# Benjamin-Lee/circkit

Measured on NVIDIA B200. Metric: canonicalize+uniq records/sec, higher is better.
Workload: dtype u8

## Files before the change

circkit_b200/_native.py:

```python
from __future__ import annotations

import ctypes as C
import os

HERE = os.path.dirname(os.path.abspath(__file__))
LIB_PATH = os.environ.get("CIRCKIT_B200_LIB") or os.path.join(HERE, "libcirckit_b200.so")

CK_OK = 0
CK_ERR_CUDA, CK_ERR_ARG, CK_ERR_STATE, CK_ERR_TOO_LONG, CK_ERR_TABLE_FULL = -1, -2, -3, -4, -5
CK_F_NORMALIZE, CK_F_NO_BYTES, CK_F_ALIGNED_OUT, CK_F_PACKED_IN, CK_F_SURVIVORS, CK_F_SINGLE_COPY = 1, 2, 4, 8, 16, 32
CK_PEER_HANDLE_BYTES = 64
CK_MONO_SENSITIVE, CK_MONO_FIRST_ONLY, CK_MONO_KEEP_ALL, CK_MONO_NONE = 1, 2, 4, 0xFFFFFFFF
CK_CMD_CANONICALIZE, CK_CMD_UNIQ, CK_CMD_MONOMERIZE = 1, 2, 3
CK_F_CANONICAL_BODY = 64
CK_DEFLATE_MAX_BYTES, CK_DEFLATE_DICT_BYTES = 64 << 20, 32768
CK_CLASS_2BIT_LE_512, CK_CLASS_2BIT_LE_2048, CK_CLASS_2BIT_LE_65536, CK_CLASS_2BIT_LE_425984 = 1, 2, 4, 8
CK_CLASS_2BIT_LE_4096, CK_CLASS_2BIT_LE_8192 = 1 << 10, 1 << 11


class CkConfig(C.Structure):
    _fields_ = [("device", C.c_int32), ("max_batch_bytes", C.c_uint64),
                ("max_batch_records", C.c_uint32), ("table_capacity", C.c_uint64)]


class CkPackedBatch(C.Structure):
    _fields_ = [("packed2", C.c_void_p), ("offsets", C.c_void_p), ("lens", C.c_void_p), ("lane", C.c_void_p),
                ("lane_bytes", C.c_void_p), ("lane_offsets", C.c_void_p), ("lane_bytes_total", C.c_uint64),
                ("n_records", C.c_uint32)]


class CkMonoOptions(C.Structure):
    _fields_ = [("seed_len", C.c_uint32), ("flags", C.c_uint32), ("overlap_dist", C.c_uint64),
                ("overlap_min_identity", C.c_double), ("min_length", C.c_uint64), ("max_length", C.c_uint64),
                ("min_overlap", C.c_uint64), ("min_overlap_percent", C.c_double)]


class NativeLibraryMissing(RuntimeError):
    pass


_vp, _u64, _u32, _i, _sz = C.c_void_p, C.c_uint64, C.c_uint32, C.c_int, C.c_size_t

SIGNATURES = {
    "ck_init": (_i, [C.POINTER(CkConfig), C.POINTER(_vp)]),
    "ck_destroy": (None, [_vp]),
    "ck_last_error": (C.c_char_p, [_vp]),
    "ck_alloc_pinned": (_vp, [_vp, _sz]),
    "ck_free_pinned": (None, [_vp, _vp]),
    "ck_canon_submit": (_i, [_vp, _i, _vp, _vp, _u32, _u32]),
    "ck_canon_wait": (_i, [_vp, _i, _vp, _vp, _vp, _vp, _vp]),
    "ck_uniq_submit": (_i, [_vp, _i, _vp, _vp, _u32, _u32, _u64]),
    "ck_uniq_wait": (_i, [_vp, _i, _vp, _vp, _vp, _vp]),
    "ck_uniq_wait_survivors": (_i, [_vp, _i, C.POINTER(_u32), _vp, _vp, _vp, _vp, _vp, _vp]),
    "ck_uniq_reset": (_i, [_vp]),
    "ck_uniq_grow": (_i, [_vp, _u64]),
    "ck_uniq_table_info": (_i, [_vp, C.POINTER(_u64), C.POINTER(_u64), C.POINTER(_u64)]),
    "ck_peer_export": (_i, [_vp, _u32, _u32, _u32, _vp]),
    "ck_peer_attach": (_i, [_vp, _vp]),
    "ck_dev_peer_first_index": (_i, [_vp, _vp, _vp, _u32, _u64, _vp, _u64, _vp]),
    "ck_pack2_words": (_u64, [_u64, _u32]),
    "ck_pack2_host": (_i, [_vp, _vp, _u32, _u32, _u32, _vp, _vp, _vp, _vp, _u64, _vp, C.POINTER(_u64)]),
    "ck_canon_submit_packed": (_i, [_vp, _i, C.POINTER(CkPackedBatch), _u32]),
    "ck_uniq_submit_packed": (_i, [_vp, _i, C.POINTER(CkPackedBatch), _u32, _u64]),
    "ck_lmsr_index": (_i, [_vp, _vp, _sz, C.POINTER(_sz)]),
    "ck_lmsr": (_i, [_vp, _vp, _sz, _vp]),
    "ck_canonicalize": (_i, [_vp, _vp, _sz, _vp]),
    "ck_lmsr_index_batch": (_i, [_vp, _vp, _vp, _u32, _vp]),
    "ck_dev_workspace_bytes": (_u64, [_u32, _u64]),
    "ck_out_arena_bytes": (_u64, [_u64, _u32]),
    "ck_dev_canon_packed2": (_i, [_vp, _vp, _vp, _vp, _u32, _u32, _u32, _vp, _vp, _vp, _vp, _vp, _u64]),
    "ck_dev_canon_bytes": (_i, [_vp, _vp, _vp, _vp, _u32, _u64, _u32, _u32, _vp, _vp, _vp, _vp, _vp, _vp, _u64]),
    "ck_dev_check": (_i, [_vp, _vp, _vp]),
    "ck_dev_table_bytes": (_u64, [_u64]),
    "ck_dev_table_clear": (_i, [_vp, _vp, _vp, _u64]),
    "ck_dev_table_insert": (_i, [_vp, _vp, _vp, _u64, _vp, _vp, _u64, _u32, _vp]),
    "ck_dev_table_first": (_i, [_vp, _vp, _vp, _u64, _vp, _u32, _vp]),
    "ck_dev_owner_partition": (_i, [_vp, _vp, _vp, _u32, _u64, _u32, _vp, _vp, _vp, _vp]),
    "ck_dev_table_insert_pairs": (_i, [_vp, _vp, _vp, _u64, _vp, _u32, _vp]),
    "ck_dev_owner_partition_padded": (_i, [_vp, _vp, _vp, _u32, _u64, _u32, _u32, _vp, _vp, _vp]),
    "ck_dev_owner_scatter_peers": (_i, [_vp, _vp, _vp, _u32, _u64, _u32, _u32, _u32, _vp, _vp, _vp]),
    "ck_dev_table_first_peers": (_i, [_vp, _vp, _vp, _u64, _vp, _u32, _u32, _u32, _vp]),
    "ck_dev_gather_first": (_i, [_vp, _vp, _vp, _vp, _u32, _vp]),
    "ck_dev_monomerize": (_i, [_vp, _vp, _vp, _vp, _vp, _u32, _u32, _u64, C.c_double, _u32, _vp]),
    "ck_dev_normalize": (_i, [_vp, _vp, _vp, _vp, _u32, _vp, _vp]),
    "ck_mono_submit": (_i, [_vp, _i, _vp, _vp, _u32, _u32, C.POINTER(CkMonoOptions)]),
    "ck_mono_wait": (_i, [_vp, _i, C.POINTER(_u32), _vp, _vp, _vp, _vp, _vp, _vp]),
    "ck_fasta_out_bytes": (_u64, [_u64, _u32]),
    "ck_fasta_submit": (_i, [_vp, _i, _vp, _u64, _u32, _u32, _u64, C.POINTER(CkMonoOptions), C.POINTER(_u32)]),
    "ck_fasta_wait": (_i, [_vp, _i, _vp, C.POINTER(_u64), C.POINTER(_u32), _vp, _vp, _vp, _vp, _vp]),
    "ck_deflate_bound": (_u64, [_u64]),
    "ck_deflate_submit": (_i, [_vp, _i, _vp, _u64, _vp, _u32, _u32]),
    "ck_deflate_wait": (_i, [_vp, _i, _vp, C.POINTER(_u64), C.POINTER(_u32)]),
    "ck_launch_count": (_u64, [_vp]),
    "ck_kernel_timing": (_i, [_vp, _i]),
    "ck_kernel_times": (_i, [_vp, _vp, _vp, _u32]),
    "ck_synth_offsets": (_i, [_vp, _vp, _u64, _u64, _u32, _u32, _u32, _u32, _u32, _vp, C.POINTER(_u64)]),
    "ck_synth_packed2": (_i, [_vp, _vp, _u64, _u64, _u32, _vp, _u32, _u32, _vp, _u32]),
    "ck_dev_unpack2": (_i, [_vp, _vp, _vp, _vp, _u32, _vp, _u32]),
    "ck_packed2_words": (_u64, [_u64, _u32, _u32]),
}

_lib = None


def lib() -> C.CDLL:
    global _lib
    if _lib is None:
        if not os.path.exists(LIB_PATH):
            raise NativeLibraryMissing(
                f"{LIB_PATH} not found: build it with `python -m circkit_b200.build` "
                "(nvcc, sm_100a).  circkit_b200 has no CPU fallback.")
        L = C.CDLL(LIB_PATH)
        for name, (res, args) in SIGNATURES.items():
            f = getattr(L, name)
            f.restype, f.argtypes = res, args
        _lib = L
    return _lib
```

circkit_b200/csrc/ck_kernels.cuh:

```cuda
#pragma once
#include "ck_hash.cuh"

namespace ck {

enum : int {
    CLS_W2S = 0,
    CLS_W2M = 1,
    CLS_C2A = 2,
    CLS_C2B = 3,
    CLS_W4 = 4,
    CLS_C4 = 5,
    CLS_W8 = 6,
    CLS_C8 = 7,
    CLS_HUGE = 8,
    CLS_EMPTY = 9,
    CLS_W2L = 10,
    CLS_W2X = 11,
    CLS_COUNT = 12
};
__host__ __device__ constexpr u32 cls_max_n(int c)
{
    return c == CLS_W2S ? 512u : c == CLS_W2M ? 2048u : c == CLS_W2L ? 4096u : c == CLS_W2X ? 8192u : c == CLS_C2A ? 65536u
         : c == CLS_C2B ? 425984u : c == CLS_W4 ? 2048u : c == CLS_C4 ? 212992u : c == CLS_W8 ? 1024u : c == CLS_C8 ? 106496u
         : c == CLS_EMPTY ? 0u : 0xffffffffu;
}
__host__ __device__ constexpr u32 cls_min_n(int c)
{
    return c == CLS_W2M ? cls_max_n(CLS_W2S) + 1 : c == CLS_W2L ? cls_max_n(CLS_W2M) + 1 : c == CLS_W2X ? cls_max_n(CLS_W2L) + 1
         : c == CLS_C2A ? cls_max_n(CLS_W2X) + 1 : c == CLS_C2B ? cls_max_n(CLS_C2A) + 1 : c == CLS_C4 ? cls_max_n(CLS_W4) + 1
         : c == CLS_C8 ? cls_max_n(CLS_W8) + 1 : c == CLS_EMPTY ? 0u : 1u;
}

__host__ __device__ constexpr u32 cls_rank(int c)
{
    return c == CLS_W2S ? 0u : c == CLS_W2M ? 1u : c == CLS_W2L ? 2u : c == CLS_W2X ? 3u : c == CLS_C2A ? 4u : c == CLS_C2B ? 5u
         : c == CLS_W4 ? 6u : c == CLS_C4 ? 7u : c == CLS_W8 ? 8u : c == CLS_C8 ? 9u : c == CLS_HUGE ? 10u : 11u;
}
__host__ __device__ constexpr int cls_of_rank(u32 r)
{
    return r == 0 ? CLS_W2S : r == 1 ? CLS_W2M : r == 2 ? CLS_W2L : r == 3 ? CLS_W2X : r == 4 ? CLS_C2A : r == 5 ? CLS_C2B
         : r == 6 ? CLS_W4 : r == 7 ? CLS_C4 : r == 8 ? CLS_W8 : r == 9 ? CLS_C8 : r == 10 ? CLS_HUGE : CLS_EMPTY;
}

struct TableSlot { u64 key; u64 first; };
#define CK_EMPTY_KEY 0xffffffffffffffffULL
__device__ __forceinline__ u64 table_home(u64 key, u64 nslots) { return __umul64hi((key ^ (key >> 29)) * 0x9E3779B97F4A7C15ULL, nslots); }
__device__ __forceinline__ u64 table_insert_one(TableSlot *slots, u64 nslots, u64 *side_first, u32 *overflow, u64 key, u64 idx)
{
    if (key == CK_EMPTY_KEY) { atomicMin(side_first, idx); return ~0ULL; }
    u64 s = table_home(key, nslots);
    for (u64 probes = 0; probes < nslots; probes++) {
        const u64 prev = atomicCAS(&slots[s].key, CK_EMPTY_KEY, key);
        if (prev == CK_EMPTY_KEY || prev == key) { atomicMin(&slots[s].first, idx); return s; }
        s = s + 1 == nslots ? 0 : s + 1;
    }
    *overflow = 1;
    return ~0ULL - 1;
}

struct CanonArgs {
    const u64 *packed2;
    u32 p2_dbl;
    const u8 *bytes;
    const u64 *offsets;
    const u32 *lens;
    const u32 *list;
    const u32 *count;
    u32 n_direct;
    u8 *out;
    u32 *out_start;
    u8 *out_strand;
    u64 *out_hash;
    u32 *scratch;
    u64 scratch_stride;
    u32 smem_units;
    u32 *xglobal;
    u32 mode;
    u32 min_n, max_n;
    u32 *retry;
    u32 *retry_counts;
    const u8 *lane_bits;
};

__device__ __forceinline__ void store_chunk(u8 *dst, int t0, u32 n, u64 lo, u64 hi)
{
    if (t0 >= 0 && (u32)t0 + 16u <= n) {
        *reinterpret_cast<uint4 *>(dst + t0) = make_uint4((u32)lo, (u32)(lo >> 32), (u32)hi, (u32)(hi >> 32));
        return;
    }
    const u32 kb = t0 < 0 ? (u32)(-t0) : 0u;
    const u32 ke = t0 < 0 ? min(16u, n + kb) : min(16u, n - (u32)t0);
    u8 *p = dst + t0;
#define CK_PIECE(k) (((k) & 8u ? hi : lo) >> (8u * ((k) & 7u)))
    u32 k = kb;
    if ((k & 1u) && k + 1 <= ke) { p[k] = (u8)CK_PIECE(k); k += 1; }
    if ((k & 2u) && k + 2 <= ke) { *reinterpret_cast<u16 *>(p + k) = (u16)CK_PIECE(k); k += 2; }
    if ((k & 4u) && k + 4 <= ke) { *reinterpret_cast<u32 *>(p + k) = (u32)CK_PIECE(k); k += 4; }
    if ((k & 8u) && k + 8 <= ke) { *reinterpret_cast<u64 *>(p + k) = hi; k += 8; }
    if (k + 8 <= ke) { *reinterpret_cast<u64 *>(p + k) = CK_PIECE(k); k += 8; }
    if (k + 4 <= ke) { *reinterpret_cast<u32 *>(p + k) = (u32)CK_PIECE(k); k += 4; }
    if (k + 2 <= ke) { *reinterpret_cast<u16 *>(p + k) = (u16)CK_PIECE(k); k += 2; }
    if (k + 1 <= ke) { p[k] = (u8)CK_PIECE(k); }
#undef CK_PIECE
}

template <int BITS, typename G>
__device__ __forceinline__ void emit_ascii(const u32 *X, u32 n, u32 start, u8 *dst)
{
    const u32 rank = G::rank(), gs = G::size();
    const u32 a = (u32)(reinterpret_cast<uintptr_t>(dst) & 15u);
    const u32 nchunks = (n + a + 15u) >> 4;
    for (u32 c = rank; c < nchunks; c += gs) {
        const int t0 = (int)(16u * c) - (int)a;
        int ti = t0;
        if (ti < 0) { ti += (int)n; if (ti < 0) { ti %= (int)n; if (ti < 0) ti += (int)n; } }
        const u32 tt = (u32)ti;
        u32 t8 = tt + 8; if (t8 >= n) { t8 -= n; if (t8 >= n) t8 %= n; }
        const u64 lo = ascii8<BITS>(X, n, start, tt), hi = ascii8<BITS>(X, n, start, t8);
        store_chunk(dst, t0, n, lo, hi);
    }
}

template <int BITS, typename G>
__device__ __forceinline__ void do_record(const CanonArgs &a, u32 rec, u32 *Xf, u32 *Xr, u32 *scr, u64 *hbuf, u32 *red)
{
    const u64 off = a.offsets[rec];
    const u32 n = a.lens ? a.lens[rec] : (u32)(a.offsets[rec + 1] - off);
    if (a.list == nullptr && (n < a.min_n || n > a.max_n)) return;
    if (a.lane_bits) { const u32 lb = a.lane_bits[rec]; if ((lb == 3u ? 4u : lb) != (u32)BITS) return; }
    RecordIn in;
    in.packed2 = a.packed2 ? a.packed2 + p2_word(off, rec, a.p2_dbl) : nullptr;
    in.bytes = a.bytes ? a.bytes + off : nullptr;
    in.n = n;
    stage_record<BITS, G>(in, Xf, Xr);
    RecordOut o = canonical_start<BITS, G>(Xf, Xr, n, scr, red, (a.mode & 1u) != 0);
    const u32 *X = o.strand ? Xr : Xf;
    if (a.out) emit_ascii<BITS, G>(X, n, o.start, a.out + ((a.mode & 2u) ? out_byte(off, rec) : off));
    u64 h = 0;
    if (a.out_hash) h = xxh3_canonical<BITS, G>(X, n, o.start, hbuf, red);
    if (G::rank() == 0) {
        if (a.out_start) a.out_start[rec] = o.strand ? (n - 1 - o.start) : o.start;
        if (a.out_strand) a.out_strand[rec] = (u8)o.strand;
        if (a.out_hash) a.out_hash[rec] = h;
    }
    G::sync();
}

template <int BITS>
__global__ void __launch_bounds__(256) k_canon_warp(CanonArgs a)
{
    extern __shared__ u32 smem[];
    typedef Grp<false> G;
    if (BITS != 2) stab_load();
    const u32 wid = threadIdx.x >> 5, wpb = blockDim.x >> 5;
    u32 *Xf = smem + (size_t)wid * 2 * a.smem_units, *Xr = Xf + a.smem_units;
    const u32 gw = blockIdx.x * wpb + wid, nw = gridDim.x * wpb;
    u32 *scr = a.scratch + (size_t)gw * a.scratch_stride;
    const u32 count = a.list ? *a.count : a.n_direct;
    if (a.list) a.list += a.count[16];
    for (u32 e = gw; e < count; e += nw) {
        const u32 rec = a.list ? a.list[e] : e;
        do_record<BITS, G>(a, rec, Xf, Xr, scr, nullptr, nullptr);
    }
}

template <int BITS, bool XGLOBAL>
__global__ void __launch_bounds__(1024) k_canon_cta(CanonArgs a)
{
    extern __shared__ u32 smem[];
    __shared__ u32 red[40];
    __shared__ u64 hbuf[32 * 8];
    typedef Grp<true> G;
    if (BITS != 2) stab_load();
    u32 *Xf = XGLOBAL ? a.xglobal + (size_t)blockIdx.x * 2 * a.smem_units : smem;
    u32 *Xr = Xf + a.smem_units;
    u32 *scr = a.scratch + (size_t)blockIdx.x * a.scratch_stride;
    const u32 count = a.list ? *a.count : a.n_direct;
    if (a.list) a.list += a.count[16];
    for (u32 e = blockIdx.x; e < count; e += gridDim.x) {
        const u32 rec = a.list ? a.list[e] : e;
        do_record<BITS, G>(a, rec, Xf, Xr, scr, hbuf, red);
    }
}

__global__ void k_canon_empty(CanonArgs a)
{
    const u32 count = a.list ? *a.count : a.n_direct;
    if (a.list) a.list += a.count[16];
    for (u32 e = blockIdx.x * blockDim.x + threadIdx.x; e < count; e += gridDim.x * blockDim.x) {
        const u32 rec = a.list ? a.list[e] : e;
        if (a.list == nullptr && a.offsets[rec + 1] != a.offsets[rec]) continue;
        if (a.out_start) a.out_start[rec] = 0;
        if (a.out_strand) a.out_strand[rec] = 1;
        if (a.out_hash) a.out_hash[rec] = xxh64_avalanche(sec64(56) ^ sec64(64));
    }
}

struct PrepareArgs {
    const u8 *raw; const u64 *offsets; u32 n_records; u32 flags;
    u64 *packed2; u8 *bytes; u32 *lens; u8 *lane;
};
__device__ __forceinline__ u32 code2_of(u32 b) { return ((b >> 1) & 3u) ^ ((b >> 2) & 1u); }

__device__ __forceinline__ uint4 prep_load16(const uint4 *w, u32 sh, bool second, bool first = true)
{
    uint4 a = make_uint4(0, 0, 0, 0), b = make_uint4(0, 0, 0, 0);
    if (first) a = __ldg(w);
    if (second) b = __ldg(w + 1);
    const u32 bs = 8u * (sh & 3u);
// ... 52 lines not shown
#pragma unroll
        for (int i = 0; i < 4; i++) {
            const u32 t = ((mm[i] & 0x7f7f7f7fu) + 0x7f7f7f7fu) | mm[i];
            nz |= ((((t >> 7) & 0x01010101u) * 0x01020408u) >> 24) << (4 * i);
        }
        keep = valid & nz;
    }
}

template <int K> __device__ __forceinline__ void prep_store_byte(u8 *g, u32 w, u32 mask)
{
    asm volatile("{ .reg .pred q; .reg .b32 t; and.b32 t, %2, %3; setp.ne.u32 q, t, 0; @q st.global.u8 [%0+%4], %1; }"
                 :: "l"(g), "r"(w >> (8 * (K & 3))), "r"(mask), "n"(1 << K), "n"(K) : "memory");
}
__device__ __forceinline__ void prep_store_bytes(u8 *g, const u32 (&w)[4], u32 mask)
{
    prep_store_byte<0>(g, w[0], mask); prep_store_byte<1>(g, w[0], mask); prep_store_byte<2>(g, w[0], mask); prep_store_byte<3>(g, w[0], mask);
    prep_store_byte<4>(g, w[1], mask); prep_store_byte<5>(g, w[1], mask); prep_store_byte<6>(g, w[1], mask); prep_store_byte<7>(g, w[1], mask);
    prep_store_byte<8>(g, w[2], mask); prep_store_byte<9>(g, w[2], mask); prep_store_byte<10>(g, w[2], mask); prep_store_byte<11>(g, w[2], mask);
    prep_store_byte<12>(g, w[3], mask); prep_store_byte<13>(g, w[3], mask); prep_store_byte<14>(g, w[3], mask); prep_store_byte<15>(g, w[3], mask);
}

#define CK_PREP_STAGE 560u

__global__ void __launch_bounds__(256) k_prepare(PrepareArgs a)
{
    __shared__ u16 tab[256];
    __shared__ __align__(16) u8 stage_all[8][CK_PREP_STAGE];
    const bool norm = a.flags & 1u;
    for (u32 b = threadIdx.x; b < 256; b += blockDim.x) {
        const u32 m = norm ? (u32)c_tab.norm[b] : b;
        const bool keep = norm ? m != 0 : true;
        const bool acgt = (m == 'A') | (m == 'C') | (m == 'G') | (m == 'T');
        u32 e = 0;
        if (keep) e = m | 0x100u | (acgt ? 0u : 0x200u) | ((!acgt && c_tab.code4[m] == 0xffu) ? 0x400u : 0u);
        tab[b] = (u16)e;
    }
    __syncthreads();
    const u32 lane = lane_id();
    u8 *stage = stage_all[threadIdx.x >> 5];
    const u32 gw = (blockIdx.x * blockDim.x + threadIdx.x) >> 5, nw = (gridDim.x * blockDim.x) >> 5;
    for (u32 rec = gw; rec < a.n_records; rec += nw) {
        const u64 off = a.offsets[rec];
        const u32 rawlen = (u32)(a.offsets[rec + 1] - off);
        const u8 *src = a.raw + off;
        u8 *dstb = a.bytes + off;
        const u32 A = (u32)((size_t)dstb & 15u);
        u8 *gbase = dstb - A;
        const u8 *srcA = src - A;
        const u32 shA = (u32)((size_t)srcA & 15u);
        const uint4 *srcA16 = reinterpret_cast<const uint4 *>(srcA - shA);
        const u32 spanA = A + rawlen;
        u32 fl = 0, cnt = 0;
        uint4 m1 = make_uint4(0, 0, 0, 0);
        for (u32 base = 0; base < spanA && rawlen; base += 512) {
            const u32 p = base + 16 * lane;
            if (p < spanA) {
                const u32 lo = p < A ? A - p : 0u, hi = min(16u, spanA - p);
                const uint4 *w0 = srcA16 + (p >> 4);
                const uint4 q = prep_load16(w0, shA, p + 16 < spanA + shA, p + 16 > A + shA);
                u32 f, keep;
                prep_lookup(tab, q, lo, hi, m1, f, keep);
                fl |= f; cnt += __popc(keep);
            }
        }
        cnt = __reduce_add_sync(CK_FULL, cnt);
        fl = __reduce_or_sync(CK_FULL, fl);
        const u32 lanebits = (fl & 0x400u) ? 8u : (fl & 0x200u) ? 4u : 2u;
        if (lane == 0) { a.lens[rec] = cnt; if (a.lane) a.lane[rec] = (u8)lanebits; }
        const bool pack2 = lanebits == 2 && !(a.flags & 2u);
        if (rawlen == 0) continue;
        const u32 sh = (u32)((size_t)src & 15u);
        const uint4 *src16 = reinterpret_cast<const uint4 *>(src - sh);
        const u32 span = sh + rawlen;
        u32 *dst32 = reinterpret_cast<u32 *>(a.packed2 + p2_word(off, rec, (a.flags >> 2) & 1u));
        if (cnt == rawlen && pack2) {
            for (u32 base = 0; base < rawlen; base += 512) {
                const u32 p = base + 16 * lane;
                if (p < rawlen) {
                    const u32 v = min(16u, rawlen - p);
                    u32 unit = prep_pack16(prep_load16(src16 + (p >> 4), sh, p + 16 < span));
                    if (v < 16) unit &= ~(0xffffffffu >> (2 * v));
                    dst32[p >> 4] = unit;
                }
            }
            continue;
        }
        if (cnt == rawlen && spanA <= 512) {
            const u32 p = 16 * lane;
            if (p < spanA) {
                const u32 lo = p < A ? A - p : 0u, hi = min(16u, spanA - p);
                if (hi - lo == 16) *reinterpret_cast<uint4 *>(gbase + p) = m1;
                else {
                    const u32 valid = (hi >= 16 ? 0xffffu : ((1u << hi) - 1u)) & ~((1u << lo) - 1u);
                    const u32 w[4] = {m1.x, m1.y, m1.z, m1.w};
                    u8 *g = gbase + p;
                    u32 vb = valid;
#pragma unroll
                    for (int i = 0; i < 4; i++)
                        if (((valid >> (4 * i)) & 15u) == 15u) { *reinterpret_cast<u32 *>(g + 4 * i) = w[i]; vb &= ~(15u << (4 * i)); }
                    prep_store_bytes(g, w, vb);
                }
            }
            continue;
        }
        u32 S = pack2 ? 0u : A;
        u32 done = 0;
        for (u32 base = 0; base < rawlen; base += 512) {
            const u32 p = base + 16 * lane;
            uint4 m = make_uint4(0, 0, 0, 0);
            u32 mask = 0;
            if (p < rawlen) {
                u32 f;
                prep_lookup(tab, prep_load16(src16 + (p >> 4), sh, p + 16 < span), 0u, min(16u, rawlen - p), m, f, mask);
            }
            const u32 kc = __popc(mask);
            u32 incl = kc;
#pragma unroll
            for (int d = 1; d < 32; d <<= 1) { const u32 t = __shfl_up_sync(CK_FULL, incl, d); if (lane >= (u32)d) incl += t; }
            const u32 T = __shfl_sync(CK_FULL, incl, 31);
            u32 idx = S + incl - kc;
            __syncwarp();
#pragma unroll
            for (int k = 0; k < 16; k++)
                if ((mask >> k) & 1u) stage[idx++] = (u8)prep_byte(m, k);
            __syncwarp();
            const u32 fill = S + T;
            if (pack2) {
                const u32 U = fill >> 4;
                for (u32 j = lane; j < U; j += 32) dst32[done + j] = prep_pack16(*reinterpret_cast<const uint4 *>(stage + 16 * j));
                const u32 r = fill & 15u;
                u8 c = 0;
                if (lane < r) c = stage[16 * U + lane];
                __syncwarp();
                if (lane < r) stage[lane] = c;
                done += U; S = r;
            } else {
                u8 *g = dstb + done - S;
                for (u32 w = lane; 16 * w < fill; w += 32) {
                    const u32 lo = max(16 * w, S), hi = min(16 * w + 16, fill);
                    if (hi - lo == 16) *reinterpret_cast<uint4 *>(g + 16 * w) = *reinterpret_cast<const uint4 *>(stage + 16 * w);
                    else for (u32 i = lo; i < hi; i++) g[i] = stage[i];
                }
                done += T; S = (u32)((size_t)(dstb + done) & 15u);
            }
        }
        __syncwarp();
        if (pack2 && S && lane == 0)
            dst32[done] = prep_pack16(*reinterpret_cast<const uint4 *>(stage)) & ~(0xffffffffu >> (2 * S));
        __syncwarp();
    }
}

struct ClassifyArgs {
    const u64 *offsets; const u32 *lens; const u8 *lane;
    u32 n_records;
    u32 *keys, *vals;
    u32 *counts;
    u32 direct_mask;
    u32 window_shift;
    u32 top_bit;
};
__global__ void __launch_bounds__(256) k_classify(ClassifyArgs a)
{
    __shared__ u32 cnt[16];
    if (threadIdx.x < 16) cnt[threadIdx.x] = 0;
    __syncthreads();
    const u32 nthreads = gridDim.x * blockDim.x;
    const u32 rounds = (a.n_records + nthreads - 1) / nthreads;
    for (u32 r = 0; r < rounds; r++) {
        const u32 i = r * nthreads + blockIdx.x * blockDim.x + threadIdx.x;
        int cls = -1;
        u32 n = 0;
        if (i < a.n_records) {
            n = a.lens ? a.lens[i] : (u32)(a.offsets[i + 1] - a.offsets[i]);
            const u32 bits = a.lane ? a.lane[i] : 2u;
            if (n == 0) cls = CLS_EMPTY;
            else if (bits == 2) cls = n <= cls_max_n(CLS_W2S) ? CLS_W2S : n <= cls_max_n(CLS_W2M) ? CLS_W2M
                                    : n <= cls_max_n(CLS_W2L) ? CLS_W2L : n <= cls_max_n(CLS_W2X) ? CLS_W2X
                                    : n <= cls_max_n(CLS_C2A) ? CLS_C2A : n <= cls_max_n(CLS_C2B) ? CLS_C2B : CLS_HUGE;
            else if (bits == 4 || bits == 3) cls = n <= cls_max_n(CLS_W4) ? CLS_W4 : n <= cls_max_n(CLS_C4) ? CLS_C4 : CLS_HUGE;
            else cls = n <= cls_max_n(CLS_W8) ? CLS_W8 : n <= cls_max_n(CLS_C8) ? CLS_C8 : CLS_HUGE;
        }
        if (a.direct_mask) {
            const u32 m = __ballot_sync(CK_FULL, cls >= 0 && !((a.direct_mask >> cls) & 1u));
            if (m && lane_id() == (u32)(__ffs(m) - 1)) atomicAdd(cnt + CLS_HUGE, __popc(m));
            continue;
        }
        if (cls >= 0) {
            const u32 msb = 31u - __clz(n | 1u);
            const u32 bin = (msb << 5) | ((((n << (31u - msb)) >> 29) & 3u) << 3);
            u32 key = (cls_rank(cls) << 10) | bin;
            if (a.window_shift < 32u) {
                const bool lane_cls = cls == CLS_W2S || cls == CLS_W2M || cls == CLS_W2L || cls == CLS_W2X;
                const u32 q = (msb << 2) | (((n << (31u - msb)) >> 29) & 3u);
                key = lane_cls ? (((i >> a.window_shift) << 5) | (q > 28u ? q - 28u : 0u)) : (key | (1u << a.top_bit));
            }
            a.keys[i] = key; a.vals[i] = i;
        }
        u32 todo = __ballot_sync(CK_FULL, cls >= 0);
        while (todo) {
            const int c = __shfl_sync(CK_FULL, cls, __ffs(todo) - 1);
            const u32 m = __ballot_sync(CK_FULL, cls == c);
            if (lane_id() == (u32)(__ffs(m) - 1)) atomicAdd(cnt + c, __popc(m));
            todo &= ~m;
        }
    }
    __syncthreads();
    if (threadIdx.x < 16 && cnt[threadIdx.x]) atomicAdd(a.counts + threadIdx.x, cnt[threadIdx.x]);
}
__global__ void k_list_starts(u32 *counts)
{
    if (threadIdx.x == 0) {
        u32 s = 0;
        for (u32 r = 0; r < (u32)CLS_COUNT; r++) {
            const int c = cls_of_rank(r);
            counts[16 + c] = s; counts[48 + c] = s;
            s += counts[c];
        }
        counts[12] = counts[CLS_W2S] + counts[CLS_W2M] + counts[CLS_W2L] + counts[CLS_W2X];
        counts[28] = counts[16 + CLS_W2S];
        counts[13] = counts[CLS_C2A] + counts[CLS_C2B];
        counts[29] = counts[16 + CLS_C2A];
    }
}

__device__ __forceinline__ u32 p2_last_unit(u32 n) { return max((2u * n + 143u) >> 4, (n >> 4) + 5u); }
__device__ __forceinline__ void extend_one(u64 *packed2, const u64 *offsets, const u32 *lens, u32 i, const u64 *dense, u32 dbl, u32 lane)
{
    const u64 off = offsets[i];
    const u32 n = lens ? lens[i] : (u32)(offsets[i + 1] - off);
    if (n == 0) return;
    u32 *U = reinterpret_cast<u32 *>(packed2 + p2_word(off, i, dbl));
    const u32 *S = dense ? reinterpret_cast<const u32 *>(dense + (off >> 5) + i) : U;
    const u32 jn = n >> 4, last = dbl ? p2_last_unit(n) : jn + 4;
    if (n >= 80) {
        for (u32 j = (dense ? 0u : jn) + lane; j <= last; j += 32) {
            const u32 r = (16u * j) % n;
            const u32 q = r >> 4, sh = 2u * (r & 15u);
            u32 w = __funnelshift_l(__ldcg(S + q + 1), __ldcg(S + q), sh);
            if (r + 16u > n) {
                const u32 k = n - r;
                w = (w & ~(0xffffffffu >> (2u * k))) | (__ldcg(S) >> (2u * k));
            }
            U[j] = w;
        }
    } else {
        for (u32 j = (dense ? 0u : jn) + lane; j <= last; j += 32) {
            u32 v = 0;
            for (u32 b = 0; b < 16; b++) {
                const u32 t = (16 * j + b) % n;
                v = (v << 2) | ((__ldcg(S + (t >> 4)) >> (30 - 2 * (t & 15))) & 3u);
            }
            __syncwarp(__activemask());
            U[j] = v;
        }
    }
    __syncwarp();
}
__global__ void __launch_bounds__(256) k_extend_packed2(u64 *packed2, const u64 *offsets, const u32 *lens, const u8 *lane_bits, u32 n_records,
                                                        const u64 *dense, u32 dbl)
{
    const u32 lane = lane_id();
    const u32 gw = (blockIdx.x * blockDim.x + threadIdx.x) >> 5, nw = (gridDim.x * blockDim.x) >> 5;
    if (n_records < 65536u) {
        for (u32 i = gw; i < n_records; i += nw) {
            if (lane_bits && lane_bits[i] != 2) continue;
            extend_one(packed2, offsets, lens, i, dense, dbl, lane);
        }
        return;
    }
    for (u32 i0 = 32u * gw; i0 < n_records; i0 += 32u * nw) {
        const u32 ii = i0 + lane;
        u32 m = __ballot_sync(CK_FULL, ii < n_records && (!lane_bits || lane_bits[ii] == 2));
        while (m) {
            const u32 i = i0 + (u32)__ffs(m) - 1u;
            m &= m - 1u;
            extend_one(packed2, offsets, lens, i, dense, dbl, lane);
        }
    }
}

__global__ void __launch_bounds__(256) k_scatter_lane_bytes(const u8 *lane_bytes, const u64 *lane_offsets, const u64 *offsets, const u32 *lens,
                                                            const u8 *lane_bits, u32 n_records, u8 *bytes)
{
    const u32 lane = lane_id();
    const u32 gw = (blockIdx.x * blockDim.x + threadIdx.x) >> 5, nw = (gridDim.x * blockDim.x) >> 5;
    for (u32 i = gw; i < n_records; i += nw) {
        if (lane_bits[i] == 2) continue;
        const u8 *src = lane_bytes + lane_offsets[i];
        u8 *dst = bytes + offsets[i];
        const u32 n = lens[i];
        for (u32 k = lane; k < n; k += 32) dst[k] = src[k];
    }
}

struct TableArgs {
    TableSlot *slots; u64 nslots;
    u64 *side_first;
    const u64 *hash; const u64 *index;
    u32 stride;
    u64 base_index; u32 n;
    u64 *slot_of;
    u64 *first_out;
    u32 *overflow;
    u64 *keys;
};
__global__ void __launch_bounds__(256) k_table_insert(TableArgs a)
{
    const u32 i = blockIdx.x * blockDim.x + threadIdx.x;
    if (i >= a.n) return;
    const u64 key = a.hash[(size_t)i * a.stride];
    const u64 idx = a.index ? a.index[(size_t)i * a.stride] : a.base_index + i;
    if (idx == ~0ULL) { a.slot_of[i] = ~0ULL - 1; return; }
    if (key == CK_EMPTY_KEY) { atomicMin(a.side_first, idx); a.slot_of[i] = ~0ULL; return; }
    u64 s = table_home(key, a.nslots);
    for (u64 probes = 0; probes < a.nslots; probes++) {
        u64 prev = atomicCAS(&a.slots[s].key, CK_EMPTY_KEY, key);
        if (prev == CK_EMPTY_KEY || prev == key) {
            atomicMin(&a.slots[s].first, idx);
            a.slot_of[i] = s;
            if (a.keys && prev == CK_EMPTY_KEY) {
                const u32 m = __activemask();
                if ((threadIdx.x & 31) == (u32)(__ffs(m) - 1)) atomicAdd(a.keys, (u64)__popc(m));
            }
            return;
        }
        s = s + 1 == a.nslots ? 0 : s + 1;
    }
    *a.overflow = 1; a.slot_of[i] = ~0ULL - 1;
}
__global__ void __launch_bounds__(256) k_table_first(TableArgs a)
{
    const u32 i = blockIdx.x * blockDim.x + threadIdx.x;
    if (i >= a.n) return;
    const u64 s = a.slot_of[i];
    a.first_out[i] = s == ~0ULL ? *a.side_first : (s == ~0ULL - 1 ? ~0ULL : a.slots[s].first);
}
__global__ void k_table_clear(TableSlot *slots, u64 n, u64 *side_first)
{
    for (u64 i = blockIdx.x * (u64)blockDim.x + threadIdx.x; i < n; i += (u64)gridDim.x * blockDim.x) {
        slots[i].key = CK_EMPTY_KEY; slots[i].first = ~0ULL;
    }
    if (blockIdx.x == 0 && threadIdx.x == 0) *side_first = ~0ULL;
}
__global__ void __launch_bounds__(256) k_table_rehash(const TableSlot *old, u64 old_slots, TableSlot *slots, u64 nslots)
{
    for (u64 i = blockIdx.x * (u64)blockDim.x + threadIdx.x; i < old_slots; i += (u64)gridDim.x * blockDim.x) {
        const TableSlot e = old[i];
        if (e.key == CK_EMPTY_KEY) continue;
        u64 s = table_home(e.key, nslots);
        while (atomicCAS(&slots[s].key, CK_EMPTY_KEY, e.key) != CK_EMPTY_KEY) s = s + 1 == nslots ? 0 : s + 1;
        slots[s].first = e.first;
    }
}

__global__ void __launch_bounds__(256) k_survivor_flags(const u64 *first, u64 base_index, u32 n, u8 *flags)
{
    const u32 i = blockIdx.x * blockDim.x + threadIdx.x;
    if (i < n) flags[i] = first[i] == base_index + i;
}
__global__ void __launch_bounds__(256) k_survivor_lens(const u32 *sel, const u32 *n_sel, const u32 *lens, u32 n, u64 *len16)
{
    const u32 k = blockIdx.x * blockDim.x + threadIdx.x;
    if (k > n) return;
    len16[k] = k < *n_sel ? (u64)((lens[sel[k]] + 15u) & ~15u) : 0ull;
}
__global__ void __launch_bounds__(256) k_gather_survivors(const u32 *sel, const u32 *n_sel, const u32 *lens, const u64 *offsets, const u8 *out,
                                                          u32 aligned, const u64 *compact_off, u8 *compact)
{
    const u32 lane = lane_id();
    const u32 gw = (blockIdx.x * blockDim.x + threadIdx.x) >> 5, nw = (gridDim.x * blockDim.x) >> 5;
    const u32 ns = *n_sel;
    for (u32 k = gw; k < ns; k += nw) {
        const u32 rec = sel[k], n = lens[rec];
        const u64 off = offsets[rec];
        const u8 *src = out + (aligned ? out_byte(off, rec) : off);
        u8 *dst = compact + compact_off[k];
        if (aligned) {
            for (u32 c = lane; 16u * c < n; c += 32) reinterpret_cast<uint4 *>(dst)[c] = reinterpret_cast<const uint4 *>(src)[c];
        } else {
            for (u32 b = lane; b < n; b += 32) dst[b] = src[b];
        }
    }
}

struct OwnerArgs {
    const u64 *hash; u32 n; u32 world; u64 base_index;
    u32 *counts;
    u64 *send_pairs; u32 *pos;
};
__device__ __forceinline__ u32 owner_of_hash(u64 h, u32 world) { return __umulhi((u32)(h >> 32), world); }
__global__ void __launch_bounds__(256) k_owner_count(OwnerArgs a)
{
    __shared__ u32 cnt[32];
    if (threadIdx.x < 32) cnt[threadIdx.x] = 0;
    __syncthreads();
    for (u32 i = blockIdx.x * blockDim.x + threadIdx.x; i < a.n; i += gridDim.x * blockDim.x)
        atomicAdd(cnt + owner_of_hash(a.hash[i], a.world), 1u);
    __syncthreads();
    if (threadIdx.x < a.world && cnt[threadIdx.x]) atomicAdd(a.counts + threadIdx.x, cnt[threadIdx.x]);
}
__global__ void __launch_bounds__(256) k_owner_scatter(OwnerArgs a)
{
    __shared__ u32 cnt[32], basep[32];
    const u32 per = (a.n + gridDim.x - 1) / gridDim.x;
    const u32 lo = min(a.n, blockIdx.x * per), hi = min(a.n, lo + per);
    if (threadIdx.x < 32) cnt[threadIdx.x] = 0;
    __syncthreads();
    for (u32 i = lo + threadIdx.x; i < hi; i += blockDim.x) atomicAdd(cnt + owner_of_hash(a.hash[i], a.world), 1u);
    __syncthreads();
    if (threadIdx.x < a.world) {
        u32 start = 0;
        for (u32 o = 0; o < threadIdx.x; o++) start += a.counts[o];
        basep[threadIdx.x] = start + atomicAdd(a.counts + a.world + threadIdx.x, cnt[threadIdx.x]);
        cnt[threadIdx.x] = 0;
    }
    __syncthreads();
    for (u32 i = lo + threadIdx.x; i < hi; i += blockDim.x) {
        const u64 h = a.hash[i];
        const u32 o = owner_of_hash(h, a.world);
        const u32 p = basep[o] + atomicAdd(cnt + o, 1u);
        reinterpret_cast<ulonglong2 *>(a.send_pairs)[p] = make_ulonglong2(h, a.base_index + i);
        a.pos[i] = p;
    }
}


struct OwnerPadArgs {
    const u64 *hash; u32 n; u32 world; u64 base_index; u32 cap;
    u32 *cursors;
    u64 *send_pairs; u32 *pos;
};
__global__ void __launch_bounds__(256) k_owner_scatter_padded(OwnerPadArgs a)
{
    __shared__ u32 cnt[32], basep[32];
    const u32 per = (a.n + gridDim.x - 1) / gridDim.x;
    const u32 lo = min(a.n, blockIdx.x * per), hi = min(a.n, lo + per);
    if (threadIdx.x < 32) cnt[threadIdx.x] = 0;
    __syncthreads();
    for (u32 i = lo + threadIdx.x; i < hi; i += blockDim.x) atomicAdd(cnt + owner_of_hash(a.hash[i], a.world), 1u);
    __syncthreads();
    if (threadIdx.x < a.world) {
        basep[threadIdx.x] = cnt[threadIdx.x] ? atomicAdd(a.cursors + threadIdx.x, cnt[threadIdx.x]) : 0u;
        if (basep[threadIdx.x] + cnt[threadIdx.x] > a.cap) a.cursors[a.world] = 1u;
        cnt[threadIdx.x] = 0;
    }
    __syncthreads();
    for (u32 i = lo + threadIdx.x; i < hi; i += blockDim.x) {
        const u64 h = a.hash[i];
        const u32 o = owner_of_hash(h, a.world);
        const u32 k = basep[o] + atomicAdd(cnt + o, 1u);
        u32 p = 0xffffffffu;
        if (k < a.cap) {
            p = o * a.cap + k;
            reinterpret_cast<ulonglong2 *>(a.send_pairs)[p] = make_ulonglong2(h, a.base_index + i);
        }
        a.pos[i] = p;
    }
}
__global__ void __launch_bounds__(256) k_owner_pad(OwnerPadArgs a)
{
    const u32 o = blockIdx.y;
    const u32 used = min(a.cursors[o], a.cap);
    for (u32 k = used + blockIdx.x * blockDim.x + threadIdx.x; k < a.cap; k += gridDim.x * blockDim.x)
        reinterpret_cast<ulonglong2 *>(a.send_pairs)[(size_t)o * a.cap + k] = make_ulonglong2(0ULL, ~0ULL);
}

struct PeerPtrs { u64 *p[32]; };
struct OwnerPeerArgs {
    const u64 *hash; u32 n; u32 world; u32 rank; u64 base_index; u32 cap;
    u32 *cursors;
    u32 *pos;
    PeerPtrs recv;
};
#define CK_SCAT_TILE 2048u
__global__ void __launch_bounds__(256) k_owner_scatter_peers(OwnerPeerArgs a)
{
    __shared__ ulonglong2 stage[CK_SCAT_TILE];
    __shared__ u8 own[CK_SCAT_TILE];
    __shared__ u32 cnt[32], start[33], basep[32], fill[32];
    const u32 per = (a.n + gridDim.x - 1) / gridDim.x;
    const u32 lo = min(a.n, blockIdx.x * per), hi = min(a.n, lo + per);
    for (u32 tile = lo; tile < hi; tile += CK_SCAT_TILE) {
        const u32 tn = min(hi - tile, CK_SCAT_TILE);
        if (threadIdx.x < 32) { cnt[threadIdx.x] = 0; fill[threadIdx.x] = 0; }
        __syncthreads();
        u64 hreg[CK_SCAT_TILE / 256];
        u32 oreg[CK_SCAT_TILE / 256];
#pragma unroll
        for (u32 k = 0; k < CK_SCAT_TILE / 256; k++) {
            const u32 j = threadIdx.x + 256u * k;
            if (j < tn) {
                hreg[k] = a.hash[tile + j];
                oreg[k] = owner_of_hash(hreg[k], a.world);
                atomicAdd(cnt + oreg[k], 1u);
            }
        }
        __syncthreads();
        if (threadIdx.x == 0) {
            u32 acc = 0;
            for (u32 o = 0; o < a.world; o++) { start[o] = acc; acc += cnt[o]; }
            start[a.world] = acc;
        }
        if (threadIdx.x < a.world) {
            const u32 c = cnt[threadIdx.x];
            basep[threadIdx.x] = c ? atomicAdd(a.cursors + threadIdx.x, c) : 0u;
            if (basep[threadIdx.x] + c > a.cap) a.cursors[a.world] = 1u;
        }
        __syncthreads();
#pragma unroll
        for (u32 k = 0; k < CK_SCAT_TILE / 256; k++) {
            const u32 j = threadIdx.x + 256u * k;
            if (j < tn) {
                const u32 o = oreg[k];
                const u32 r = atomicAdd(fill + o, 1u);
                const u32 slot = start[o] + r;
                stage[slot] = make_ulonglong2(hreg[k], a.base_index + tile + j);
                own[slot] = (u8)o;
                const u32 g = basep[o] + r;
                a.pos[tile + j] = g < a.cap ? o * a.cap + g : 0xffffffffu;
            }
        }
        __syncthreads();
        for (u32 sl = threadIdx.x; sl < tn; sl += 256) {
            const u32 o = own[sl];
            const u32 g = basep[o] + (sl - start[o]);
            if (g < a.cap) reinterpret_cast<ulonglong2 *>(a.recv.p[o])[(size_t)a.rank * a.cap + g] = stage[sl];
        }
        __syncthreads();
    }
}
__global__ void __launch_bounds__(256) k_owner_pad_peers(OwnerPeerArgs a)
{
    const u32 o = blockIdx.y;
    const u32 used = min(a.cursors[o], a.cap);
    ulonglong2 *dst = reinterpret_cast<ulonglong2 *>(a.recv.p[o]) + (size_t)a.rank * a.cap;
    for (u32 k = used + blockIdx.x * blockDim.x + threadIdx.x; k < a.cap; k += gridDim.x * blockDim.x)
        dst[k] = make_ulonglong2(0ULL, ~0ULL);
}
struct FirstPeerArgs {
    const TableSlot *slots; const u64 *side_first; const u64 *slot_of;
    u32 world; u32 rank; u32 cap;
    PeerPtrs ret;
};
__global__ void __launch_bounds__(256) k_table_first_peers(FirstPeerArgs a)
{
    const u32 s = blockIdx.y;
    u64 *dst = a.ret.p[s] + (size_t)a.rank * a.cap;
    const u64 *slot_of = a.slot_of + (size_t)s * a.cap;
    for (u32 k = blockIdx.x * blockDim.x + threadIdx.x; k < a.cap; k += gridDim.x * blockDim.x) {
        const u64 sl = slot_of[k];
        dst[k] = sl == ~0ULL ? *a.side_first : (sl == ~0ULL - 1 ? ~0ULL : a.slots[sl].first);
    }
}
struct PeerBlockPtrs { u64 *p[32]; };
#define CK_PEER_FLAG_WORDS 128u
#define CK_PEER_HEADER_BYTES 4096u
__global__ void k_peer_barrier(PeerBlockPtrs blocks, u32 world, u32 rank, u32 barrier_id, u64 epoch, const u32 *send_counts, u32 count_slot)
{
    const u32 t = threadIdx.x;
    if (t >= world) return;
    if (send_counts) blocks.p[t][CK_PEER_FLAG_WORDS + 32u * count_slot + rank] = send_counts[t];
    __threadfence_system();
    u64 *theirs = blocks.p[t] + barrier_id * 32u + rank;
    asm volatile("st.release.sys.global.u64 [%0], %1;" ::"l"(theirs), "l"(epoch) : "memory");
    const u64 *mine = blocks.p[rank] + barrier_id * 32u + t;
    u64 seen;
    do {
        asm volatile("ld.acquire.sys.global.u64 %0, [%1];" : "=l"(seen) : "l"(mine) : "memory");
    } while (seen < epoch);
}
struct RegionArgs {
    TableSlot *slots; u64 nslots; u64 *side_first; u32 *overflow;
    const u64 *recv;
    const u64 *counts;
    u64 *slot_of;
    u32 world, rank, cap;
    PeerBlockPtrs ret;
};
__global__ void __launch_bounds__(256) k_table_insert_regions(RegionArgs a)
{
    const u32 s = blockIdx.y;
    const u32 cnt = (u32)a.counts[s];
    const ulonglong2 *pairs = reinterpret_cast<const ulonglong2 *>(a.recv) + (size_t)s * a.cap;
    u64 *slot_of = a.slot_of + (size_t)s * a.cap;
    for (u32 k = blockIdx.x * blockDim.x + threadIdx.x; k < cnt; k += gridDim.x * blockDim.x) {
        const ulonglong2 pr = pairs[k];
        const u64 key = pr.x, idx = pr.y;
        if (key == CK_EMPTY_KEY) { atomicMin(a.side_first, idx); slot_of[k] = ~0ULL; continue; }
        u64 sl = table_home(key, a.nslots);
        u64 found = ~0ULL - 1;
        for (u64 probes = 0; probes < a.nslots; probes++) {
            const u64 prev = atomicCAS(&a.slots[sl].key, CK_EMPTY_KEY, key);
            if (prev == CK_EMPTY_KEY || prev == key) { atomicMin(&a.slots[sl].first, idx); found = sl; break; }
            sl = sl + 1 == a.nslots ? 0 : sl + 1;
        }
        if (found == ~0ULL - 1) *a.overflow = 1;
        slot_of[k] = found;
    }
}
__global__ void __launch_bounds__(256) k_table_first_regions(RegionArgs a)
{
    const u32 s = blockIdx.y;
    const u32 cnt = (u32)a.counts[s];
    u64 *dst = a.ret.p[s] + (size_t)a.rank * a.cap;
    const u64 *slot_of = a.slot_of + (size_t)s * a.cap;
    for (u32 k = blockIdx.x * blockDim.x + threadIdx.x; k < cnt; k += gridDim.x * blockDim.x) {
        const u64 sl = slot_of[k];
        dst[k] = sl == ~0ULL ? *a.side_first : (sl == ~0ULL - 1 ? ~0ULL : a.slots[sl].first);
    }
}

__global__ void __launch_bounds__(256) k_gather_first(const u64 *ret, const u32 *pos, u32 n, u64 *out)
{
    for (u32 i = blockIdx.x * blockDim.x + threadIdx.x; i < n; i += gridDim.x * blockDim.x) {
        const u32 p = pos[i];
        out[i] = p == 0xffffffffu ? ~0ULL : ret[p];
    }
}

}
```

circkit_b200/csrc/ck_lib.cu:

```cuda
#include <algorithm>
#include <cstdio>
#include <cstdlib>
#include <cstring>
#include <mutex>
#include <new>
#include <string>
#include <vector>

#include <cub/device/device_radix_sort.cuh>
#include <cub/device/device_scan.cuh>
#include <cub/device/device_select.cuh>
#include <cub/iterator/counting_input_iterator.cuh>

#include "../../include/circkit_b200.h"
#include "ck_kernels.cuh"
#include "ck_warp2.cuh"
#include "ck_lane2.cuh"
#include "ck_stream2.cuh"
#include "ck_stream3.cuh"
#include "ck_seg2.cuh"
#include "ck_lane4.cuh"
#include "ck_synth.cuh"
#include "ck_monomerize.cuh"
#include "ck_fasta.cuh"
#include "ck_deflate.cuh"

using namespace ck;

namespace {

thread_local std::string g_init_error;

inline const u64 *U(const uint64_t *p) { return reinterpret_cast<const u64 *>(p); }
inline u64 *U(uint64_t *p) { return reinterpret_cast<u64 *>(p); }

struct ClsCfg { int bits; bool cta; u32 threads; u32 ctas_per_sm; };
const ClsCfg kCls[CLS_COUNT] = {
    {2, false, 256, 8},
    {2, false, 256, 6},
    {2, true, 512, 4},
    {2, true, 1024, 1},
    {4, false, 256, 32},
    {4, true, 1024, 1},
    {8, false, 256, 32},
    {8, true, 1024, 1},
    {0, true, 0, 0},
    {0, false, 256, 1},
    {2, false, 256, 6},
    {2, false, 256, 6},
};

u32 cls_units(int c)
{
    const u32 n = cls_max_n(c);
    switch (kCls[c].bits) {
    case 2: return strand_units<2>(n);
    case 4: return strand_units<4>(n);
    default: return strand_units<8>(n);
    }
}
u64 cls_tie_words(int c)
{
    const u64 n = cls_max_n(c);
    switch (kCls[c].bits) {
    case 2: return tie_scratch_words<2>(n);
    case 4: return tie_scratch_words<4>(n);
    default: return tie_scratch_words<8>(n);
    }
}
u32 cls_smem_bytes(int c)
{
    const u32 per = 2u * cls_units(c) * 4u;
    if (c == CLS_W2S || c == CLS_W2M || c == CLS_W2L || c == CLS_W2X) return (u32)sizeof(W2Const) + per * (kCls[c].threads / 32u);
    return kCls[c].cta ? per : per * (kCls[c].threads / 32u);
}

struct ExecScratch {
    u32 *tie[CLS_COUNT] = {};
    u64 *seg = nullptr;
    u32 *huge_x = nullptr, *huge_tie = nullptr;
    u64 huge_x_words = 0, huge_tie_words = 0;
    cudaStream_t side_stream[CLS_COUNT] = {};
    cudaEvent_t ev_fork = nullptr, ev_join[CLS_COUNT] = {};
};

struct Slot {
    cudaStream_t stream = nullptr;
    cudaEvent_t inserted = nullptr;
    u8 *d_raw = nullptr; u64 *d_off = nullptr; u64 *d_p2 = nullptr; u8 *d_norm = nullptr; u8 *d_p4 = nullptr;
    u32 *d_len = nullptr; u8 *d_lane = nullptr; u8 *d_out = nullptr; u32 *d_start = nullptr;
    u8 *d_strand = nullptr; u64 *d_hash = nullptr; u64 *d_first = nullptr; u64 *d_slotof = nullptr;
    u32 *d_lists = nullptr; u32 *d_counts = nullptr;
    u64 *d_dense = nullptr; u64 *d_laneoff = nullptr;
    u32 *h_counts = nullptr;
    ExecScratch scr;
    bool busy = false, uniq = false, mono = false;
    bool text = false;
    u32 cmd = 0;
    u8 *d_text = nullptr, *d_frame = nullptr;
    u64 *d_rstart = nullptr, *d_head = nullptr, *d_seq = nullptr, *d_len64 = nullptr, *d_fofs = nullptr, *d_meta = nullptr;
    u32 *d_tiles = nullptr;
    u32 dbl = 1;
    u64 longest = 0;
    u32 *sel = nullptr; u64 *coff = nullptr;
    u32 n = 0, flags = 0; u64 total = 0;
    u64 rec_mark = 0;
    bool defl = false;
    struct Deflate {
        cudaStream_t stream = nullptr;
        u64 cap = 0;
        u8 *buf = nullptr;
        u32 *kA = nullptr, *kB = nullptr, *vA = nullptr, *vB = nullptr;
        u32 *prev8 = nullptr, *prev4 = nullptr;
        u32 *seg = nullptr;
        u32 *out = nullptr, *result = nullptr;
        u32 *h_result = nullptr;
        void *tmp = nullptr; size_t tmp_bytes = 0;
        u64 n = 0;
    } z;
};

struct PeerGroup {
    u32 world = 1, rank = 0, cap = 0;
    u8 *block = nullptr; u64 block_bytes = 0, recv_bytes = 0, ret_bytes = 0;
    void *mapped[32] = {};
    bool exported = false, attached = false;
    u64 epoch[4] = {};
    u32 *pos[2] = {}; u32 *cursors[2] = {}; u64 *slot_of[2] = {};
    u64 *recv(u32 r, u32 slot) const { return reinterpret_cast<u64 *>((u8 *)mapped[r] + CK_PEER_HEADER_BYTES + (u64)slot * recv_bytes); }
    u64 *ret(u32 r, u32 slot) const { return reinterpret_cast<u64 *>((u8 *)mapped[r] + CK_PEER_HEADER_BYTES + 2 * recv_bytes + (u64)slot * ret_bytes); }
    u64 *counts(u32 r, u32 slot) const { return reinterpret_cast<u64 *>(mapped[r]) + CK_PEER_FLAG_WORDS + 32u * slot; }
};

}

struct ck_ctx {
    int device = 0;
    int num_sms = 148;
    ck_config cfg{};
    std::string err;
    Slot slot[2];
    ExecScratch dev_scr;
    cudaEvent_t last_insert = nullptr;
    bool have_last_insert = false;
    TableSlot *table = nullptr; u64 table_slots = 0; u64 *side = nullptr; u32 *d_overflow = nullptr;
    u64 *d_keys = nullptr;
    u64 grow_max = 0, grows = 0;
    u64 known_keys = 0, known_rec = 0, submitted_rec = 0;
    PeerGroup peer;
    std::mutex lib_mu;
    cudaStream_t lib_stream = nullptr;
    u8 *lib_h = nullptr, *lib_d = nullptr; size_t lib_h_bytes = 0, lib_d_bytes = 0;
    ExecScratch lib_scr;
    u64 launches = 0;
    bool attrs_set = false;
    u32 s3_debug = 0;
    bool l4_kernel = true;
    bool seg_kernel = true;
    int lane_kernel = 3;
    bool timing = false;
    std::vector<cudaEvent_t> ev_pairs[CLS_COUNT + 7];
};

namespace {

int fail(ck_ctx *ctx, int code, const char *what, cudaError_t e = cudaSuccess)
{
    std::string m = what;
    if (e != cudaSuccess) { m += ": "; m += cudaGetErrorString(e); }
    if (ctx) ctx->err = m; else g_init_error = m;
    return code;
}
#define CK_CUDA(ctx, call)                                                     \
    do {                                                                       \
        cudaError_t e__ = (call);                                              \
        if (e__ != cudaSuccess) return fail((ctx), CK_ERR_CUDA, #call, e__);   \
    } while (0)

void fill_tables(Tables &t, u8 secret[200])
{
    for (int c = 0; c < 256; c++) t.norm[c] = 'N';
    for (const char *p = "ACGTN-"; *p; p++) t.norm[(u8)*p] = (u8)*p;
    t.norm['a'] = 'A'; t.norm['c'] = 'C'; t.norm['g'] = 'G';
    t.norm['t'] = 'T'; t.norm['u'] = 'T'; t.norm['U'] = 'T';
    t.norm['.'] = '-'; t.norm['~'] = '-';
    t.norm[' '] = 0; t.norm['\t'] = 0; t.norm['\r'] = 0; t.norm['\n'] = 0;
    for (int c = 0; c < 256; c++) t.comp[c] = (u8)c;
    const char *a = "AGCTYRWSKMDVHBN", *b = "TCGARYWSMKHBDVN";
    for (int i = 0; a[i]; i++) { t.comp[(u8)a[i]] = (u8)b[i]; t.comp[(u8)a[i] + 32] = (u8)(b[i] + 32); }
    const char *alpha = "-ABCDGHKMNRSTVWY";
    for (int c = 0; c < 256; c++) t.code4[c] = 0xff;
    for (int i = 0; i < 16; i++) { t.sym4[i] = (u8)alpha[i]; t.code4[(u8)alpha[i]] = (u8)i; }
    for (int i = 0; i < 16; i++) t.comp4[i] = t.code4[t.comp[t.sym4[i]]];
    static const u8 sec[192] = {
        0xb8, 0xfe, 0x6c, 0x39, 0x23, 0xa4, 0x4b, 0xbe, 0x7c, 0x01, 0x81, 0x2c, 0xf7, 0x21, 0xad, 0x1c,
        0xde, 0xd4, 0x6d, 0xe9, 0x83, 0x90, 0x97, 0xdb, 0x72, 0x40, 0xa4, 0xa4, 0xb7, 0xb3, 0x67, 0x1f,
        0xcb, 0x79, 0xe6, 0x4e, 0xcc, 0xc0, 0xe5, 0x78, 0x82, 0x5a, 0xd0, 0x7d, 0xcc, 0xff, 0x72, 0x21,
        0xb8, 0x08, 0x46, 0x74, 0xf7, 0x43, 0x24, 0x8e, 0xe0, 0x35, 0x90, 0xe6, 0x81, 0x3a, 0x26, 0x4c,
        0x3c, 0x28, 0x52, 0xbb, 0x91, 0xc3, 0x00, 0xcb, 0x88, 0xd0, 0x65, 0x8b, 0x1b, 0x53, 0x2e, 0xa3,
        0x71, 0x64, 0x48, 0x97, 0xa2, 0x0d, 0xf9, 0x4e, 0x38, 0x19, 0xef, 0x46, 0xa9, 0xde, 0xac, 0xd8,
        0xa8, 0xfa, 0x76, 0x3f, 0xe3, 0x9c, 0x34, 0x3f, 0xf9, 0xdc, 0xbb, 0xc7, 0xc7, 0x0b, 0x4f, 0x1d,
        0x8a, 0x51, 0xe0, 0x4b, 0xcd, 0xb4, 0x59, 0x31, 0xc8, 0x9f, 0x7e, 0xc9, 0xd9, 0x78, 0x73, 0x64,
        0xea, 0xc5, 0xac, 0x83, 0x34, 0xd3, 0xeb, 0xc3, 0xc5, 0x81, 0xa0, 0xff, 0xfa, 0x13, 0x63, 0xeb,
        0x17, 0x0d, 0xdd, 0x51, 0xb7, 0xf0, 0xda, 0x49, 0xd3, 0x16, 0x55, 0x26, 0x29, 0xd4, 0x68, 0x9e,
        0x2b, 0x16, 0xbe, 0x58, 0x7d, 0x47, 0xa1, 0xfc, 0x8f, 0xf8, 0xb8, 0xd1, 0x7a, 0xd0, 0x31, 0xce,
        0x45, 0xcb, 0x3a, 0x8f, 0x95, 0x16, 0x04, 0x28, 0xaf, 0xd7, 0xfb, 0xca, 0xbb, 0x4b, 0x40, 0x7e,
    };
    memset(secret, 0, 200);
    memcpy(secret, sec, 192);
}

int alloc_scratch(ck_ctx *ctx, ExecScratch &s)
{
    CK_CUDA(ctx, cudaEventCreateWithFlags(&s.ev_fork, cudaEventDisableTiming));
    for (int c = 0; c < CLS_COUNT; c++) {
        CK_CUDA(ctx, cudaStreamCreateWithFlags(&s.side_stream[c], cudaStreamNonBlocking));
        CK_CUDA(ctx, cudaEventCreateWithFlags(&s.ev_join[c], cudaEventDisableTiming));
    }
    CK_CUDA(ctx, cudaMalloc(&s.seg, (size_t)2 * ctx->num_sms * CK_SEG_WARPS * CK_SEG_SCRATCH_U64 * 8));
    for (int c = 0; c < CLS_COUNT; c++) {
        if (kCls[c].bits == 0) continue;
        const u64 groups = (u64)kCls[c].ctas_per_sm * ctx->num_sms * (kCls[c].cta ? 1u : kCls[c].threads / 32u);
        CK_CUDA(ctx, cudaMalloc(&s.tie[c], groups * cls_tie_words(c) * 4));
    }
    return CK_OK;
}
void free_scratch(ExecScratch &s)
{
    for (int c = 0; c < CLS_COUNT; c++) {
        if (s.tie[c]) cudaFree(s.tie[c]);
        if (s.side_stream[c]) cudaStreamDestroy(s.side_stream[c]);
        if (s.ev_join[c]) cudaEventDestroy(s.ev_join[c]);
        s.tie[c] = nullptr; s.side_stream[c] = nullptr; s.ev_join[c] = nullptr;
    }
    if (s.ev_fork) cudaEventDestroy(s.ev_fork);
    if (s.seg) cudaFree(s.seg);
    if (s.huge_x) cudaFree(s.huge_x);
    if (s.huge_tie) cudaFree(s.huge_tie);
    s.huge_x = s.huge_tie = nullptr; s.huge_x_words = s.huge_tie_words = 0;
    s.ev_fork = nullptr; s.seg = nullptr;
}

template <typename K> int set_smem(ck_ctx *ctx, K kernel, u32 bytes)
{
    if (bytes > 48 * 1024) CK_CUDA(ctx, cudaFuncSetAttribute(kernel, cudaFuncAttributeMaxDynamicSharedMemorySize, (int)bytes));
    return CK_OK;
}
void s2_launch(ck_ctx *ctx, cudaStream_t st, const CanonArgs &a, int v)
{
    if (ctx->lane_kernel != 2 && a.p2_dbl) {
        const u32 g3 = 2u * (u32)ctx->num_sms, th3 = 32u * CK_S3_WARPS, sm3 = CK_S3_WARPS * CK_S3_WARP_BYTES;
#define CK_S3(V) k_canon_s3<V><<<g3, th3, sm3, st>>>(a)
        switch (v) {
        case 0: CK_S3(0); break; case 1: CK_S3(1); break; case 2: CK_S3(2); break; case 3: CK_S3(3); break;
        case 4: CK_S3(4); break; case 5: CK_S3(5); break; case 6: CK_S3(6); break; default: CK_S3(7);
        }
#undef CK_S3
        return;
    }
    const u32 g = 2u * (u32)ctx->num_sms, th = 32u * CK_S2_WARPS, sm = CK_S2_WARPS * CK_S2_WARP_BYTES;
#define CK_S2(V) k_canon_s2<V><<<g, th, sm, st>>>(a)
    switch (v) {
    case 0: CK_S2(0); break; case 1: CK_S2(1); break; case 2: CK_S2(2); break; case 3: CK_S2(3); break;
    case 4: CK_S2(4); break; case 5: CK_S2(5); break; case 6: CK_S2(6); break; default: CK_S2(7);
    }
#undef CK_S2
}

int set_attrs(ck_ctx *ctx)
{
    if (ctx->attrs_set) return CK_OK;
    int rc;
    if ((rc = set_smem(ctx, k_canon_cta<2, false>, cls_smem_bytes(CLS_C2B)))) return rc;
    if ((rc = set_smem(ctx, k_canon_cta<4, false>, cls_smem_bytes(CLS_C4)))) return rc;
    if ((rc = set_smem(ctx, k_canon_cta<8, false>, cls_smem_bytes(CLS_C8)))) return rc;
    const u32 s2 = CK_S2_WARPS * CK_S2_WARP_BYTES;
    if ((rc = set_smem(ctx, k_canon_s2<0>, s2)) || (rc = set_smem(ctx, k_canon_s2<1>, s2)) || (rc = set_smem(ctx, k_canon_s2<2>, s2)) ||
        (rc = set_smem(ctx, k_canon_s2<3>, s2)) || (rc = set_smem(ctx, k_canon_s2<4>, s2)) || (rc = set_smem(ctx, k_canon_s2<5>, s2)) ||
        (rc = set_smem(ctx, k_canon_s2<6>, s2)) || (rc = set_smem(ctx, k_canon_s2<7>, s2))) return rc;
    const u32 s3 = CK_S3_WARPS * CK_S3_WARP_BYTES;
    if ((rc = set_smem(ctx, k_canon_s3<0>, s3)) || (rc = set_smem(ctx, k_canon_s3<1>, s3)) || (rc = set_smem(ctx, k_canon_s3<2>, s3)) ||
        (rc = set_smem(ctx, k_canon_s3<3>, s3)) || (rc = set_smem(ctx, k_canon_s3<4>, s3)) || (rc = set_smem(ctx, k_canon_s3<5>, s3)) ||
        (rc = set_smem(ctx, k_canon_s3<6>, s3)) || (rc = set_smem(ctx, k_canon_s3<7>, s3))) return rc;
    const u32 l4 = CK_L4_WARPS * CK_L4_WARP_BYTES;
    if ((rc = set_smem(ctx, k_canon_l4<0>, l4)) || (rc = set_smem(ctx, k_canon_l4<1>, l4)) || (rc = set_smem(ctx, k_canon_l4<2>, l4)) ||
        (rc = set_smem(ctx, k_canon_l4<3>, l4))) return rc;
    ctx->attrs_set = true;
    return CK_OK;
}

struct CanonIO {
    const u64 *packed2; const u8 *bytes; const u64 *offsets; const u32 *lens; const u8 *lane;
    u32 n; u32 mode;
    u32 dbl = 1;
    u64 longest = 0;
    u8 *p4 = nullptr;
    u8 *out; u32 *out_start; u8 *out_strand; u64 *out_hash;
    u32 *lists; u64 lists_bytes;
    u32 *counts;
};

u64 lists_bytes_for(u64 n) { return ((16 * (n + 4) + 24 * (n + 4) + 255) & ~255ull) + (1ull << 20); }

int run_canon(ck_ctx *ctx, cudaStream_t st, ExecScratch &scr, const CanonIO &io, u32 class_mask)
{
    if (io.n == 0) return CK_OK;
    int rc = set_attrs(ctx);
    if (rc) return rc;
    CK_CUDA(ctx, cudaMemsetAsync(io.counts, 0, 64 * sizeof(u32), st));
    int only = -1;
    if (class_mask && (class_mask & (class_mask - 1)) == 0)
        for (int c = 0; c < CLS_COUNT; c++) if (class_mask == (1u << c)) only = c;
    const u64 stride = ((u64)io.n + 4) & ~3ull;
    u32 *k0 = io.lists, *k1 = k0 + stride, *v0 = k1 + stride, *v1 = v0 + stride;
    if (io.lists_bytes < 16 * stride) return fail(ctx, CK_ERR_ARG, "sort workspace too small");
    const bool fastv = io.packed2 && !(io.mode & 1u) && (!io.out || (io.mode & 2u)) && io.out_start && io.out_strand;
    u32 window_shift = 32, top_bit = 13;
    if (fastv && only < 0) {
        window_shift = 16;
        u32 wbits = 0;
        while ((((u64)io.n - 1) >> window_shift) >> wbits) wbits++;
        top_bit = std::max(14u, 5u + wbits);
    }
    const bool l4_run = fastv && only < 0 && ctx->l4_kernel && io.p4 && io.lane && io.bytes && (!class_mask || (class_mask & (1u << CLS_W4)));
    if (l4_run) {
        cudaEvent_t e0 = nullptr, e1 = nullptr;
        if (ctx->timing) { CK_CUDA(ctx, cudaEventCreate(&e0)); CK_CUDA(ctx, cudaEventCreate(&e1)); CK_CUDA(ctx, cudaEventRecord(e0, st)); }
        k_pack4<<<std::min<u32>((io.n + 15) / 16, 16u * (u32)ctx->num_sms), 256, 0, st>>>(io.bytes, io.offsets, io.lens, const_cast<u8 *>(io.lane), io.n, io.p4);
        if (ctx->timing) { CK_CUDA(ctx, cudaEventRecord(e1, st)); ctx->ev_pairs[CLS_COUNT + 5].push_back(e0); ctx->ev_pairs[CLS_COUNT + 5].push_back(e1); }
        ctx->launches++;
    }
    const int sort_bits = (int)top_bit + 1;
    const bool lane_checks = fastv && only >= 0 && io.lane == nullptr &&
                             (only == CLS_W2S || only == CLS_W2M || only == CLS_W2L || only == CLS_W2X);
    if (!lane_checks) {
        ClassifyArgs ca{io.offsets, io.lens, io.lane, io.n, k0, v0, io.counts, only >= 0 ? (1u << only) : 0u, window_shift, top_bit};
        k_classify<<<std::min<u32>((io.n + 255) / 256, 16u * (u32)ctx->num_sms), 256, 0, st>>>(ca);
        ctx->launches++;
    }
    const u32 *sorted = nullptr;
    u32 *retry = v0;
    if (only < 0) {
        cub::DoubleBuffer<u32> keys(k0, k1), vals(v0, v1);
        void *tmp = v1 + stride;
        size_t tmp_bytes = (size_t)(io.lists_bytes - 16 * stride), need = 0;
        cub::DeviceRadixSort::SortPairs(nullptr, need, keys, vals, (int)io.n, 0, sort_bits, st);
        if (need > tmp_bytes) return fail(ctx, CK_ERR_ARG, "sort workspace too small");
        CK_CUDA(ctx, cub::DeviceRadixSort::SortPairs(tmp, need, keys, vals, (int)io.n, 0, sort_bits, st));
        sorted = vals.Current();
        retry = vals.Alternate();
        k_list_starts<<<1, 32, 0, st>>>(io.counts);
        ctx->launches += 2;
    }
    const u32 lane_classes = (1u << CLS_W2S) | (1u << CLS_W2M) | (1u << CLS_W2L) | (1u << CLS_W2X);
    auto timed = [&](int slot, cudaEvent_t &e0, cudaEvent_t &e1, bool begin, cudaStream_t on) -> cudaError_t {
        if (!ctx->timing) return cudaSuccess;
        if (begin) {
            cudaError_t e = cudaEventCreate(&e0); if (e != cudaSuccess) return e;
            e = cudaEventCreate(&e1); if (e != cudaSuccess) return e;
            return cudaEventRecord(e0, on);
        }
        ctx->ev_pairs[slot].push_back(e0); ctx->ev_pairs[slot].push_back(e1);
        return cudaEventRecord(e1, on);
    };
    auto base_args = [&](int c) {
        CanonArgs a{};
        a.packed2 = io.packed2; a.p2_dbl = io.dbl; a.bytes = io.bytes; a.offsets = io.offsets; a.lens = io.lens;
        a.max_n = cls_max_n(c); a.min_n = cls_min_n(c);
        a.out = io.out; a.out_start = io.out_start; a.out_strand = io.out_strand; a.out_hash = io.out_hash;
        a.scratch = scr.tie[c]; a.scratch_stride = kCls[c].bits ? cls_tie_words(c) : 0;
        a.smem_units = kCls[c].bits ? cls_units(c) : 0; a.xglobal = nullptr; a.mode = io.mode;
        a.retry = retry; a.retry_counts = io.counts + 32;
        return a;
    };
    const bool lane_run = fastv && (only >= 0 ? ((lane_classes >> only) & 1u) != 0 : (!class_mask || (class_mask & lane_classes)));
    if (lane_run) {
        CanonArgs a = base_args(only >= 0 ? only : CLS_W2S);
        if (only >= 0) { a.list = nullptr; a.count = nullptr; a.n_direct = io.n; }
        else { a.list = sorted; a.count = io.counts + 12; a.n_direct = 0; a.min_n = 1; a.max_n = cls_max_n(CLS_W2X); }
        const int v = (a.out_hash ? CK_W2_HASH : 0) | (a.out ? CK_W2_OUT : 0) | (a.list ? CK_W2_LIST : 0);
        a.mode |= ctx->s3_debug;
        cudaEvent_t e0 = nullptr, e1 = nullptr;
        CK_CUDA(ctx, timed(CLS_COUNT, e0, e1, true, st));
        s2_launch(ctx, st, a, v);
        CK_CUDA(ctx, timed(CLS_COUNT, e0, e1, false, st));
        ctx->launches++;
    }
    const u32 seg_classes = (1u << CLS_C2A) | (1u << CLS_C2B);
    const bool seg_run = fastv && only < 0 && ctx->seg_kernel && io.dbl && (!class_mask || (class_mask & seg_classes));
    if (seg_run) {
        CanonArgs a = base_args(CLS_C2A);
        a.list = sorted; a.count = io.counts + 13; a.n_direct = 0;
        const u32 g = 2u * (u32)ctx->num_sms, th = 32u * CK_SEG_WARPS, sm = CK_SEG_WARPS * CK_SEG_WARP_BYTES;
        cudaEvent_t e0 = nullptr, e1 = nullptr;
        CK_CUDA(ctx, timed(CLS_COUNT + 3, e0, e1, true, st));
        switch ((a.out_hash ? CK_W2_HASH : 0) | (a.out ? CK_W2_OUT : 0)) {
        case 0: k_canon_seg<0><<<g, th, sm, st>>>(a, scr.seg); break;
        case 1: k_canon_seg<1><<<g, th, sm, st>>>(a, scr.seg); break;
        case 2: k_canon_seg<2><<<g, th, sm, st>>>(a, scr.seg); break;
        default: k_canon_seg<3><<<g, th, sm, st>>>(a, scr.seg); break;
        }
        CK_CUDA(ctx, timed(CLS_COUNT + 3, e0, e1, false, st));
        ctx->launches++;
    }
    if (l4_run) {
        CanonArgs a = base_args(CLS_W4);
        a.list = sorted; a.count = io.counts + CLS_W4; a.n_direct = 0;
        const u32 g = 2u * (u32)ctx->num_sms, th = 32u * CK_L4_WARPS, sm = CK_L4_WARPS * CK_L4_WARP_BYTES;
        cudaEvent_t e0 = nullptr, e1 = nullptr;
        CK_CUDA(ctx, timed(CLS_COUNT + 4, e0, e1, true, st));
        switch ((a.out_hash ? CK_W2_HASH : 0) | (a.out ? CK_W2_OUT : 0)) {
        case 0: k_canon_l4<0><<<g, th, sm, st>>>(a, io.p4, io.lane); break;
        case 1: k_canon_l4<1><<<g, th, sm, st>>>(a, io.p4, io.lane); break;
        case 2: k_canon_l4<2><<<g, th, sm, st>>>(a, io.p4, io.lane); break;
        default: k_canon_l4<3><<<g, th, sm, st>>>(a, io.p4, io.lane); break;
        }
        CK_CUDA(ctx, timed(CLS_COUNT + 4, e0, e1, false, st));
        ctx->launches++;
    }
    u32 to_launch = 0;
    for (int c = 0; c < CLS_COUNT; c++)
        if (c != CLS_HUGE && !(class_mask && !(class_mask & (1u << c)))) to_launch++;
    const bool fork = scr.ev_fork != nullptr && to_launch >= 2;
    if (fork) CK_CUDA(ctx, cudaEventRecord(scr.ev_fork, st));
    u32 joined = 0;
    for (int c = 0; c < CLS_COUNT; c++) {
        if (c == CLS_HUGE) continue;
        if (class_mask && !(class_mask & (1u << c))) continue;
        CanonArgs a = base_args(c);
        const bool is_lane_cls = ((lane_classes >> c) & 1u) != 0;
        if ((lane_run && is_lane_cls) || (seg_run && ((seg_classes >> c) & 1u)) || (l4_run && c == CLS_W4)) { a.list = retry; a.count = io.counts + 32 + c; a.n_direct = 0; }
        else if (only >= 0) { a.list = nullptr; a.count = nullptr; a.n_direct = io.n; }
        else { a.list = sorted; a.count = io.counts + c; a.n_direct = 0; }
        const u32 grid = kCls[c].ctas_per_sm * (u32)ctx->num_sms, thr = kCls[c].threads;
        const u32 smem = kCls[c].bits ? cls_smem_bytes(c) : 0;
        cudaEvent_t e0 = nullptr, e1 = nullptr;
        const bool side = fork && (!kCls[c].cta || (seg_run && ((seg_classes >> c) & 1u)));
        cudaStream_t sc = side ? scr.side_stream[c] : st;
        if (side) CK_CUDA(ctx, cudaStreamWaitEvent(sc, scr.ev_fork, 0));
        CK_CUDA(ctx, timed(c, e0, e1, true, sc));
        switch (c) {
        case CLS_W2S: k_canon_w2<true, -1><<<grid, thr, smem, sc>>>(a); break;
        case CLS_W2M: case CLS_W2L: case CLS_W2X: k_canon_w2<false, -1><<<grid, thr, smem, sc>>>(a); break;
        case CLS_C2A: case CLS_C2B: k_canon_cta<2, false><<<grid, thr, smem, sc>>>(a); break;
        case CLS_W4: k_canon_warp<4><<<grid, thr, smem, sc>>>(a); break;
        case CLS_C4: k_canon_cta<4, false><<<grid, thr, smem, sc>>>(a); break;
        case CLS_W8: k_canon_warp<8><<<grid, thr, smem, sc>>>(a); break;
        case CLS_C8: k_canon_cta<8, false><<<grid, thr, smem, sc>>>(a); break;
        case CLS_EMPTY: k_canon_empty<<<(u32)ctx->num_sms, 256, 0, sc>>>(a); break;
        }
        CK_CUDA(ctx, timed(c, e0, e1, false, sc));
        if (side) { CK_CUDA(ctx, cudaEventRecord(scr.ev_join[c], sc)); joined |= 1u << c; }
        ctx->launches++;
    }
    for (int c = 0; c < CLS_COUNT; c++)
        if ((joined >> c) & 1u) CK_CUDA(ctx, cudaStreamWaitEvent(st, scr.ev_join[c], 0));
    if (only < 0 && io.longest > cls_max_n(CLS_C8) && (!class_mask || (class_mask & (1u << CLS_HUGE)))) {
        const u64 nl = io.longest;
        const u32 G = (u32)std::max<u64>(1, std::min<u64>(32, (1ull << 30) / (2 * nl + 64)));
        const u64 xw = (u64)G * 2 * strand_units<8>((u32)nl), tw = (u64)G * tie_scratch_words<8>(nl);
        if (xw > scr.huge_x_words) {
            if (scr.huge_x) CK_CUDA(ctx, cudaFree(scr.huge_x));
            scr.huge_x = nullptr; scr.huge_x_words = 0;
            CK_CUDA(ctx, cudaMalloc(&scr.huge_x, xw * 4));
            scr.huge_x_words = xw;
        }
        if (tw > scr.huge_tie_words) {
            if (scr.huge_tie) CK_CUDA(ctx, cudaFree(scr.huge_tie));
            scr.huge_tie = nullptr; scr.huge_tie_words = 0;
            CK_CUDA(ctx, cudaMalloc(&scr.huge_tie, tw * 4));
            scr.huge_tie_words = tw;
        }
        CanonArgs a = base_args(CLS_HUGE);
        a.list = sorted; a.count = io.counts + CLS_HUGE; a.n_direct = 0; a.min_n = 1; a.max_n = 0xffffffffu;
        a.xglobal = scr.huge_x; a.scratch = scr.huge_tie; a.lane_bits = io.lane;
        a.smem_units = strand_units<2>((u32)nl); a.scratch_stride = tie_scratch_words<2>(nl);
        if (nl > cls_max_n(CLS_C2B)) { k_canon_cta<2, true><<<G, 1024, 0, st>>>(a); ctx->launches++; }
        if (io.lane && nl > cls_max_n(CLS_C4)) {
            a.smem_units = strand_units<4>((u32)nl); a.scratch_stride = tie_scratch_words<4>(nl);
            k_canon_cta<4, true><<<G, 1024, 0, st>>>(a);
            ctx->launches++;
        }
        if (io.lane) {
            a.smem_units = strand_units<8>((u32)nl); a.scratch_stride = tie_scratch_words<8>(nl);
            k_canon_cta<8, true><<<G, 1024, 0, st>>>(a);
            ctx->launches++;
        }
        CK_CUDA(ctx, cudaMemsetAsync(io.counts + CLS_HUGE, 0, 4, st));
    }
    CK_CUDA(ctx, cudaGetLastError());
    return CK_OK;
}

u32 extend_grid(const ck_ctx *ctx, u32 n_records) { return std::max(1u, std::min<u32>((n_records + 7) / 8, 32u * (u32)ctx->num_sms)); }

u64 table_slots_for(u64 keys) { return std::max<u64>(1024, keys + keys / 2 + 16); }

int table_insert(ck_ctx *ctx, cudaStream_t st, TableSlot *slots, u64 nslots, u64 *side, u32 *overflow,
                 const u64 *hash, const u64 *index, u64 base, u32 n, u64 *slot_of, u32 stride = 1, u64 *keys = nullptr)
{
    if (!n) return CK_OK;
    TableArgs t{slots, nslots, side, hash, index, stride, base, n, slot_of, nullptr, overflow, keys};
    k_table_insert<<<(n + 255) / 256, 256, 0, st>>>(t);
    ctx->launches++;
    CK_CUDA(ctx, cudaGetLastError());
    return CK_OK;
}
int table_first(ck_ctx *ctx, cudaStream_t st, TableSlot *slots, u64 nslots, u64 *side, const u64 *slot_of, u32 n, u64 *first)
{
    if (!n) return CK_OK;
    TableArgs t{slots, nslots, side, nullptr, nullptr, 1, 0, n, const_cast<u64 *>(slot_of), first, nullptr};
    k_table_first<<<(n + 255) / 256, 256, 0, st>>>(t);
    ctx->launches++;
    CK_CUDA(ctx, cudaGetLastError());
    return CK_OK;
}

u64 table_capacity_keys(u64 slots) { return slots * 2 / 3; }

int table_grow(ck_ctx *ctx, cudaStream_t st, u64 slots)
{
    TableSlot *t = nullptr;
    cudaError_t e = cudaMalloc(&t, slots * sizeof(TableSlot));
    if (e != cudaSuccess) {
        cudaGetLastError();
        return fail(ctx, CK_ERR_TABLE_FULL, "uniq table cannot grow: its new size cannot be allocated", e);
    }
    e = cudaMemsetAsync(t, 0xff, slots * sizeof(TableSlot), st);
    if (e == cudaSuccess) {
        const u64 grid = std::min<u64>((ctx->table_slots + 255) / 256, 32ull * (u64)ctx->num_sms);
        k_table_rehash<<<(u32)grid, 256, 0, st>>>(ctx->table, ctx->table_slots, t, slots);
        ctx->launches++;
        e = cudaGetLastError();
    }
    if (e == cudaSuccess) e = cudaStreamSynchronize(st);
    if (e != cudaSuccess) { cudaFree(t); return fail(ctx, CK_ERR_CUDA, "uniq table growth", e); }
    cudaFree(ctx->table);
    ctx->table = t; ctx->table_slots = slots; ctx->grows++;
    return CK_OK;
}

int table_reserve(ck_ctx *ctx, Slot &s, u64 n)
{
    const u64 cap = table_capacity_keys(ctx->table_slots);
    if (ctx->grow_max && ctx->known_keys + (ctx->submitted_rec - ctx->known_rec) + n > cap) {
        for (Slot &o : ctx->slot) if (o.stream) CK_CUDA(ctx, cudaStreamSynchronize(o.stream));
        u64 exact = 0;
        CK_CUDA(ctx, cudaMemcpy(&exact, ctx->d_keys, 8, cudaMemcpyDeviceToHost));
        ctx->known_keys = exact; ctx->known_rec = ctx->submitted_rec;
        const u64 need = exact + n;
        if (need > cap) {
            if (need > ctx->grow_max) return fail(ctx, CK_ERR_TABLE_FULL, "uniq batch would take the table past max_keys");
            const int rc = table_grow(ctx, s.stream, table_slots_for(std::min(ctx->grow_max, 2 * need + 2 * n)));
            if (rc) return rc;
        }
    }
    ctx->submitted_rec += n;
    s.rec_mark = ctx->submitted_rec;
    return CK_OK;
}

void note_keys(ck_ctx *ctx, const Slot &s)
{
    if (s.rec_mark <= ctx->known_rec) return;
    memcpy(&ctx->known_keys, s.h_counts + 18, 8);
    ctx->known_rec = s.rec_mark;
}

int peer_first_index(ck_ctx *ctx, cudaStream_t st, u32 slot, const u64 *hash, u32 n, u64 base_index, TableSlot *table, u64 nslots,
                     u64 *side, u32 *overflow, u64 *out_first, cudaEvent_t insert_done, cudaEvent_t wait_before_query)
{
    PeerGroup &P = ctx->peer;
    if (!P.attached) return fail(ctx, CK_ERR_STATE, "peer group not attached");
    if (n > P.cap) return fail(ctx, CK_ERR_ARG, "batch larger than the peer group's max_records");
    CK_CUDA(ctx, cudaMemsetAsync(P.cursors[slot], 0, (P.world + 1) * sizeof(u32), st));
    OwnerPeerArgs oa{};
    oa.hash = hash; oa.n = n; oa.world = P.world; oa.rank = P.rank; oa.base_index = base_index; oa.cap = P.cap;
    oa.cursors = P.cursors[slot]; oa.pos = P.pos[slot];
    PeerBlockPtrs blocks{};
    RegionArgs ra{};
    for (u32 r = 0; r < P.world; r++) {
        oa.recv.p[r] = P.recv(r, slot);
        blocks.p[r] = reinterpret_cast<u64 *>(P.mapped[r]);
        ra.ret.p[r] = P.ret(r, slot);
    }
    if (n) {
        k_owner_scatter_peers<<<std::min<u32>((n + 255) / 256, 8u * (u32)ctx->num_sms), 256, 0, st>>>(oa);
        ctx->launches++;
    }
    k_peer_barrier<<<1, 32, 0, st>>>(blocks, P.world, P.rank, 2 * slot, ++P.epoch[2 * slot], P.cursors[slot], slot);
    ra.slots = table; ra.nslots = nslots; ra.side_first = side; ra.overflow = overflow;
    ra.recv = P.recv(P.rank, slot); ra.counts = P.counts(P.rank, slot); ra.slot_of = P.slot_of[slot];
    ra.world = P.world; ra.rank = P.rank; ra.cap = P.cap;
    const u32 gx = std::max<u32>(1u, std::min<u32>((P.cap + 255) / 256, (8u * (u32)ctx->num_sms + P.world - 1) / P.world));
    k_table_insert_regions<<<dim3(gx, P.world), 256, 0, st>>>(ra);
    if (insert_done) CK_CUDA(ctx, cudaEventRecord(insert_done, st));
    if (wait_before_query) CK_CUDA(ctx, cudaStreamWaitEvent(st, wait_before_query, 0));
    k_table_first_regions<<<dim3(gx, P.world), 256, 0, st>>>(ra);
    k_peer_barrier<<<1, 32, 0, st>>>(blocks, P.world, P.rank, 2 * slot + 1, ++P.epoch[2 * slot + 1], nullptr, 0);
    if (n) k_gather_first<<<std::min<u32>((n + 255) / 256, 16u * (u32)ctx->num_sms), 256, 0, st>>>(P.ret(P.rank, slot), P.pos[slot], n, out_first);
    ctx->launches += 5;
    CK_CUDA(ctx, cudaGetLastError());
    return CK_OK;
}

constexpr u64 kMonoMaxRecord = (1ull << 32) - 1024;

int mono_options_check(ck_ctx *ctx, const ck_mono_options *opt)
{
    if (!opt) return fail(ctx, CK_ERR_ARG, "null options");
    if (opt->seed_len < 1 || opt->seed_len > 63) return fail(ctx, CK_ERR_ARG, "Seed length must be at least 1 and at most 63");
    if (opt->overlap_min_identity >= 0.0 && opt->overlap_dist)
        return fail(ctx, CK_ERR_ARG, "Both overlap_dist and overlap_min_identity are set. They are mutually exclusive");
    if (opt->flags & ~(CK_MONO_SENSITIVE | CK_MONO_FIRST_ONLY | CK_MONO_KEEP_ALL)) return fail(ctx, CK_ERR_ARG, "unknown option flags");
    return CK_OK;
}

int submit_check(ck_ctx *ctx, int slot, const uint64_t *offsets, uint32_t n_records, uint32_t flags, bool uniq, bool have_bytes,
                 bool mono = false)
{
    if (!ctx) return CK_ERR_ARG;
    if (slot < 0 || slot > 1) return fail(ctx, CK_ERR_ARG, "slot must be 0 or 1");
    Slot &s = ctx->slot[slot];
    if (s.busy) return fail(ctx, CK_ERR_STATE, "slot already holds a batch; call the matching wait first");
    if (n_records > ctx->cfg.max_batch_records) return fail(ctx, CK_ERR_ARG, "n_records exceeds max_batch_records");
    if (n_records && (!offsets || (!have_bytes && offsets[n_records] != offsets[0])))
        return fail(ctx, CK_ERR_ARG, "null batch pointers");
    if (uniq && !ctx->table) return fail(ctx, CK_ERR_STATE, "context was created with table_capacity 0");
    s.n = n_records; s.flags = flags; s.uniq = uniq; s.mono = false; s.text = false; s.defl = false; s.total = 0; s.rec_mark = 0;
    if (n_records == 0) return CK_OK;
    if (offsets[0] != 0) return fail(ctx, CK_ERR_ARG, "offsets[0] must be 0");
    const u64 total = offsets[n_records];
    if (total > ctx->cfg.max_batch_bytes) return fail(ctx, CK_ERR_ARG, "batch exceeds max_batch_bytes");
    u64 longest = 0;
    for (u32 i = 0; i < n_records; i++) {
        if (offsets[i + 1] < offsets[i]) return fail(ctx, CK_ERR_ARG, "offsets must be non-decreasing");
        longest = std::max<u64>(longest, offsets[i + 1] - offsets[i]);
    }
    if (mono && longest > kMonoMaxRecord) return fail(ctx, CK_ERR_TOO_LONG, "record longer than 2^32 - 1024 bytes");
    if (!mono && longest > (1ull << 30)) return fail(ctx, CK_ERR_TOO_LONG, "record longer than 2^30 symbols");
    s.total = total;
    s.longest = longest;
    s.dbl = longest > 512 ? 1u : 0u;
    return CK_OK;
}

struct Compaction {
    u32 *sel; u64 *len16; u64 *coff; u8 *flags; u32 *n_sel; void *tmp; size_t tmp_bytes;
};
int compaction_carve(ck_ctx *ctx, Slot &s, Compaction &c)
{
    const u32 n = s.n;
    u8 *w = reinterpret_cast<u8 *>(s.d_lists);
    c.sel = reinterpret_cast<u32 *>(w); w += ((size_t)n * 4 + 255) & ~(size_t)255;
    c.len16 = reinterpret_cast<u64 *>(w); w += ((size_t)(n + 1) * 8 + 255) & ~(size_t)255;
    c.coff = reinterpret_cast<u64 *>(w); w += ((size_t)(n + 1) * 8 + 255) & ~(size_t)255;
    c.flags = w; w += ((size_t)n + 255) & ~(size_t)255;
    c.n_sel = reinterpret_cast<u32 *>(w); w += 256;
    c.tmp = w;
    const size_t used = (size_t)(w - reinterpret_cast<u8 *>(s.d_lists));
    const size_t have = lists_bytes_for(ctx->cfg.max_batch_records);
    size_t need_a = 0, need_b = 0;
    cub::CountingInputIterator<u32> ids(0);
    cub::DeviceSelect::Flagged(nullptr, need_a, ids, c.flags, c.sel, c.n_sel, (int)n, s.stream);
    cub::DeviceScan::ExclusiveSum(nullptr, need_b, c.len16, c.coff, (int)n + 1, s.stream);
    if (used + std::max(need_a, need_b) > have) return fail(ctx, CK_ERR_ARG, "sort workspace too small for the compaction");
    c.tmp_bytes = have - used;
    return CK_OK;
}
int compaction_select_scan(ck_ctx *ctx, Slot &s, const Compaction &c, const u32 *lens)
{
    cudaStream_t st = s.stream;
    const u32 n = s.n;
    size_t tb = c.tmp_bytes;
    cub::CountingInputIterator<u32> ids(0);
    CK_CUDA(ctx, cub::DeviceSelect::Flagged(c.tmp, tb, ids, c.flags, c.sel, c.n_sel, (int)n, st));
    k_survivor_lens<<<(n + 256) / 256, 256, 0, st>>>(c.sel, c.n_sel, lens, n, c.len16);
    tb = c.tmp_bytes;
    CK_CUDA(ctx, cub::DeviceScan::ExclusiveSum(c.tmp, tb, c.len16, c.coff, (int)n + 1, st));
    ctx->launches += 3;
    CK_CUDA(ctx, cudaMemcpyAsync(s.h_counts + 20, c.n_sel, 4, cudaMemcpyDeviceToHost, st));
    s.sel = c.sel; s.coff = c.coff;
    return CK_OK;
}

int enqueue_compaction(ck_ctx *ctx, Slot &s, uint64_t base_index)
{
    cudaStream_t st = s.stream;
    const u32 n = s.n;
    Compaction c;
    int rc = compaction_carve(ctx, s, c);
    if (rc) return rc;
    k_survivor_flags<<<(n + 255) / 256, 256, 0, st>>>(s.d_first, base_index, n, c.flags);
    rc = compaction_select_scan(ctx, s, c, s.d_len);
    if (rc) return rc;
    if (!(s.flags & CK_F_NO_BYTES))
        k_gather_survivors<<<std::min<u32>((n + 7) / 8, 32u * (u32)ctx->num_sms), 256, 0, st>>>(c.sel, c.n_sel, s.d_len, s.d_off, s.d_out,
                                                                                               (s.flags & CK_F_ALIGNED_OUT) ? 1u : 0u, c.coff, s.d_norm);
    ctx->launches += 2;
    CK_CUDA(ctx, cudaGetLastError());
    return CK_OK;
}

int enqueue_mono(ck_ctx *ctx, Slot &s, const Compaction &c, const ck_mono_options &o)
{
    cudaStream_t st = s.stream;
    const u32 n = s.n;
    const bool norm = s.flags & CK_F_NORMALIZE;
    u32 *end = s.d_start, *full_len = reinterpret_cast<u32 *>(s.d_slotof), *mono_len = reinterpret_cast<u32 *>(s.d_hash);
    int rc;
    if (norm) {
        PrepareArgs pa{s.d_raw, s.d_off, n, 1u | 2u | 4u, nullptr, s.d_norm, s.d_len, nullptr};
        k_prepare<<<ctx->num_sms * 32, 256, 0, st>>>(pa);
        ctx->launches++;
    }
    MonoArgs ma{};
    ma.bytes = norm ? s.d_norm : s.d_raw; ma.offsets = s.d_off; ma.lens = norm ? s.d_len : nullptr; ma.n_records = n;
    ma.seed_len = o.seed_len; ma.use_identity = o.overlap_min_identity >= 0.0 ? 1u : 0u; ma.overlap_dist = o.overlap_dist;
    ma.identity = o.overlap_min_identity; ma.flags = o.flags & (CK_MONO_SENSITIVE | CK_MONO_FIRST_ONLY); ma.out_end = end;
    k_monomerize<<<std::min<u32>((n + 7) / 8, 16u * (u32)ctx->num_sms), 256, 0, st>>>(ma);
    MonoSelectArgs sa{};
    sa.raw = s.d_raw; sa.offsets = s.d_off; sa.lens = norm ? s.d_len : nullptr; sa.n_records = n; sa.normalize = norm ? 1u : 0u;
    sa.keep_all = (o.flags & CK_MONO_KEEP_ALL) ? 1u : 0u; sa.seed_len = o.seed_len; sa.min_length = o.min_length;
    sa.max_length = o.max_length; sa.min_overlap = o.min_overlap; sa.min_overlap_percent = o.min_overlap_percent;
    sa.end = end; sa.full_len = full_len; sa.monomer_len = mono_len; sa.written = c.flags;
    const u32 grid = std::min<u32>((n + 7) / 8, 32u * (u32)ctx->num_sms);
    k_mono_select<<<grid, 256, 0, st>>>(sa);
    ctx->launches += 2;
    rc = compaction_select_scan(ctx, s, c, mono_len);
    if (rc) return rc;
    if (!(s.flags & CK_F_NO_BYTES)) {
        k_mono_gather<<<grid, 256, 0, st>>>(s.d_raw, s.d_off, c.sel, c.n_sel, mono_len, c.coff, norm ? 1u : 0u, s.d_out);
        ctx->launches++;
    }
    CK_CUDA(ctx, cudaGetLastError());
    return CK_OK;
}

int submit_tail(ck_ctx *ctx, Slot &s, bool lens_given, uint64_t base_index)
{
    cudaStream_t st = s.stream;
    const u32 n_records = s.n, flags = s.flags;
    CanonIO io{};
    io.packed2 = s.d_p2; io.bytes = s.d_norm; io.offsets = s.d_off; io.lens = lens_given ? s.d_len : nullptr; io.lane = s.d_lane;
    io.n = n_records; io.mode = (flags & CK_F_ALIGNED_OUT) ? 2u : 0u; io.dbl = s.dbl; io.p4 = s.d_p4; io.longest = s.longest;
    io.out = (flags & CK_F_NO_BYTES) ? nullptr : s.d_out;
    io.out_start = s.d_start; io.out_strand = s.d_strand; io.out_hash = s.d_hash;
    io.lists = s.d_lists; io.lists_bytes = lists_bytes_for(ctx->cfg.max_batch_records); io.counts = s.d_counts;
// ... 3 lines not shown
    if (peer_mode) {
        const u32 slot = (u32)(&s - ctx->slot);
        cudaEvent_t prev = (ctx->have_last_insert && ctx->last_insert != s.inserted) ? ctx->last_insert : nullptr;
        rc = peer_first_index(ctx, st, slot, s.d_hash, n_records, base_index, ctx->table, ctx->table_slots, ctx->side, ctx->d_overflow,
                              s.d_first, s.inserted, prev);
        if (rc) return rc;
        ctx->last_insert = s.inserted; ctx->have_last_insert = true;
        CK_CUDA(ctx, cudaMemcpyAsync(s.h_counts + 16, ctx->d_overflow, 4, cudaMemcpyDeviceToHost, st));
    } else if (s.uniq) {
        rc = table_insert(ctx, st, ctx->table, ctx->table_slots, ctx->side, ctx->d_overflow, s.d_hash, nullptr,
                          base_index, n_records, s.d_slotof, 1, ctx->d_keys);
        if (rc) return rc;
        CK_CUDA(ctx, cudaEventRecord(s.inserted, st));
        if (ctx->have_last_insert && ctx->last_insert != s.inserted) CK_CUDA(ctx, cudaStreamWaitEvent(st, ctx->last_insert, 0));
        ctx->last_insert = s.inserted; ctx->have_last_insert = true;
        rc = table_first(ctx, st, ctx->table, ctx->table_slots, ctx->side, s.d_slotof, n_records, s.d_first);
        if (rc) return rc;
        CK_CUDA(ctx, cudaMemcpyAsync(s.h_counts + 16, ctx->d_overflow, 16, cudaMemcpyDeviceToHost, st));
    }
    CK_CUDA(ctx, cudaMemcpyAsync(s.h_counts, s.d_counts, 16 * 4, cudaMemcpyDeviceToHost, st));
    if (s.uniq && (flags & CK_F_SURVIVORS)) {
        rc = enqueue_compaction(ctx, s, base_index);
        if (rc) return rc;
    }
    s.busy = true;
    return CK_OK;
}

int submit_empty(ck_ctx *ctx, Slot &s, uint64_t base_index)
{
    s.busy = true;
    if (!(s.uniq && ctx->peer.attached && ctx->peer.world > 1)) return CK_OK;
    CK_CUDA(ctx, cudaSetDevice(ctx->device));
    const u32 slot = (u32)(&s - ctx->slot);
    cudaEvent_t prev = (ctx->have_last_insert && ctx->last_insert != s.inserted) ? ctx->last_insert : nullptr;
    int rc = peer_first_index(ctx, s.stream, slot, s.d_hash, 0, base_index, ctx->table, ctx->table_slots, ctx->side, ctx->d_overflow,
                              s.d_first, s.inserted, prev);
    if (rc) { s.busy = false; return rc; }
    ctx->last_insert = s.inserted; ctx->have_last_insert = true;
    return CK_OK;
}

int enqueue_canon(ck_ctx *ctx, Slot &s, uint64_t base_index)
{
    cudaStream_t st = s.stream;
    const u32 n_records = s.n, flags = s.flags;
    PrepareArgs pa{s.d_raw, s.d_off, n_records, (flags & CK_F_NORMALIZE) | (s.dbl << 2), s.d_p2, s.d_norm, s.d_len, s.d_lane};
    k_prepare<<<ctx->num_sms * 32, 256, 0, st>>>(pa);
    k_extend_packed2<<<extend_grid(ctx, n_records), 256, 0, st>>>(s.d_p2, s.d_off, s.d_len, s.d_lane, n_records, nullptr, s.dbl);
    ctx->launches += 2;
    return submit_tail(ctx, s, (flags & CK_F_NORMALIZE) != 0, base_index);
}

int submit_common(ck_ctx *ctx, int slot, const uint8_t *bytes, const uint64_t *offsets, uint32_t n_records,
                  uint32_t flags, bool uniq, uint64_t base_index)
{
    int rc = submit_check(ctx, slot, offsets, n_records, flags, uniq, bytes != nullptr);
    if (rc) return rc;
    Slot &s = ctx->slot[slot];
    if (n_records == 0) return submit_empty(ctx, s, base_index);
    const u64 total = s.total;
    cudaStream_t st = s.stream;
    CK_CUDA(ctx, cudaSetDevice(ctx->device));
    if (uniq && !ctx->peer.attached && (rc = table_reserve(ctx, s, n_records))) return rc;
    CK_CUDA(ctx, cudaMemcpyAsync(s.d_off, offsets, (size_t)(n_records + 1) * 8, cudaMemcpyHostToDevice, st));
    if (total) CK_CUDA(ctx, cudaMemcpyAsync(s.d_raw, bytes, total, cudaMemcpyHostToDevice, st));
    return enqueue_canon(ctx, s, base_index);
}

int submit_packed(ck_ctx *ctx, int slot, const ck_packed_batch *b, uint32_t flags, bool uniq, uint64_t base_index)
{
    if (!ctx) return CK_ERR_ARG;
    if (!b) return fail(ctx, CK_ERR_ARG, "null batch");
    const u32 n_records = b->n_records;
    int rc = submit_check(ctx, slot, b->offsets, n_records, flags | CK_F_PACKED_IN, uniq, true);
    if (rc) return rc;
    Slot &s = ctx->slot[slot];
    if (n_records == 0) return submit_empty(ctx, s, base_index);
    if (!b->packed2 || !b->lens || !b->lane) return fail(ctx, CK_ERR_ARG, "null batch pointers");
    if (b->lane_bytes_total && (!b->lane_bytes || !b->lane_offsets)) return fail(ctx, CK_ERR_ARG, "byte-lane records without lane_bytes / lane_offsets");
    if (b->lane_bytes_total > ctx->cfg.max_batch_bytes) return fail(ctx, CK_ERR_ARG, "lane_bytes exceed max_batch_bytes");
    cudaStream_t st = s.stream;
    CK_CUDA(ctx, cudaSetDevice(ctx->device));
    if (uniq && !ctx->peer.attached && (rc = table_reserve(ctx, s, n_records))) return rc;
    CK_CUDA(ctx, cudaMemcpyAsync(s.d_off, b->offsets, (size_t)(n_records + 1) * 8, cudaMemcpyHostToDevice, st));
    CK_CUDA(ctx, cudaMemcpyAsync(s.d_len, b->lens, (size_t)n_records * 4, cudaMemcpyHostToDevice, st));
    CK_CUDA(ctx, cudaMemcpyAsync(s.d_lane, b->lane, (size_t)n_records, cudaMemcpyHostToDevice, st));
    CK_CUDA(ctx, cudaMemcpyAsync(s.d_dense, b->packed2, (size_t)ck_pack2_words(s.total, n_records) * 8, cudaMemcpyHostToDevice, st));
    k_extend_packed2<<<extend_grid(ctx, n_records), 256, 0, st>>>(s.d_p2, s.d_off, s.d_len, s.d_lane, n_records, s.d_dense, s.dbl);
    ctx->launches++;
    if (b->lane_bytes_total) {
        CK_CUDA(ctx, cudaMemcpyAsync(s.d_laneoff, b->lane_offsets, (size_t)(n_records + 1) * 8, cudaMemcpyHostToDevice, st));
        CK_CUDA(ctx, cudaMemcpyAsync(s.d_raw, b->lane_bytes, (size_t)b->lane_bytes_total, cudaMemcpyHostToDevice, st));
        k_scatter_lane_bytes<<<extend_grid(ctx, n_records), 256, 0, st>>>(s.d_raw, s.d_laneoff, s.d_off, s.d_len, s.d_lane, n_records, s.d_norm);
        ctx->launches++;
    }
    return submit_tail(ctx, s, true, base_index);
}

int wait_common(ck_ctx *ctx, int slot, bool uniq, uint8_t *out_bytes, uint32_t *out_len, uint32_t *out_start,
                uint8_t *out_strand, uint64_t *out_hash, uint64_t *out_first)
{
    if (!ctx) return CK_ERR_ARG;
    if (slot < 0 || slot > 1) return fail(ctx, CK_ERR_ARG, "slot must be 0 or 1");
    Slot &s = ctx->slot[slot];
    if (!s.busy || s.uniq != uniq || s.mono || s.text || s.defl) return fail(ctx, CK_ERR_STATE, "no matching submit on this slot");
    s.busy = false;
    if (s.n == 0) {
        if (uniq && ctx->peer.attached && ctx->peer.world > 1) CK_CUDA(ctx, cudaStreamSynchronize(s.stream));
        return CK_OK;
    }
    cudaStream_t st = s.stream;
    const size_t n = s.n;
    if (out_bytes && !(s.flags & CK_F_NO_BYTES) && s.total)
        CK_CUDA(ctx, cudaMemcpyAsync(out_bytes, s.d_out, (s.flags & CK_F_ALIGNED_OUT) ? ck_out_arena_bytes(s.total, s.n) : s.total,
                                     cudaMemcpyDeviceToHost, st));
    if (out_len) CK_CUDA(ctx, cudaMemcpyAsync(out_len, s.d_len, n * 4, cudaMemcpyDeviceToHost, st));
    if (out_start) CK_CUDA(ctx, cudaMemcpyAsync(out_start, s.d_start, n * 4, cudaMemcpyDeviceToHost, st));
    if (out_strand) CK_CUDA(ctx, cudaMemcpyAsync(out_strand, s.d_strand, n, cudaMemcpyDeviceToHost, st));
    if (out_hash) CK_CUDA(ctx, cudaMemcpyAsync(out_hash, s.d_hash, n * 8, cudaMemcpyDeviceToHost, st));
    if (out_first && uniq) CK_CUDA(ctx, cudaMemcpyAsync(out_first, s.d_first, n * 8, cudaMemcpyDeviceToHost, st));
    CK_CUDA(ctx, cudaStreamSynchronize(st));
    if (uniq) note_keys(ctx, s);
    if (s.h_counts[CLS_HUGE]) return fail(ctx, CK_ERR_TOO_LONG, "batch holds a record beyond the staged-length classes");
    if (uniq && s.h_counts[16]) return fail(ctx, CK_ERR_TABLE_FULL, "uniq table is full; raise table_capacity");
    return CK_OK;
}

}

static bool table_view(void *table, u64 bytes, TableSlot *&slots, u64 &nslots, u64 *&side, u32 *&overflow)
{
    if (!table || bytes < 64 + sizeof(TableSlot) * 16) return false;
    nslots = (bytes - 64) / sizeof(TableSlot);
    side = (u64 *)table; overflow = (u32 *)((u8 *)table + 8);
    slots = (TableSlot *)((u8 *)table + 64);
    return true;
}

extern "C" {

int ck_init(const ck_config *cfg, ck_ctx **out)
{
    if (!cfg || !out) return fail(nullptr, CK_ERR_ARG, "null argument");
    *out = nullptr;
    ck_ctx *ctx = new (std::nothrow) ck_ctx();
    if (!ctx) return fail(nullptr, CK_ERR_ARG, "out of host memory");
    ctx->cfg = *cfg;
    ctx->device = cfg->device;
    if (const char *dbg = getenv("CK_S3_DEBUG")) ctx->s3_debug = (u32)strtoul(dbg, nullptr, 0) & 0xff00u;
    if (const char *sk = getenv("CK_SEG_KERNEL")) ctx->seg_kernel = atoi(sk) != 0;
    if (const char *lk = getenv("CK_L4_KERNEL")) ctx->l4_kernel = atoi(lk) != 0;
    if (const char *lk = getenv("CK_LANE_KERNEL")) ctx->lane_kernel = atoi(lk) == 2 ? 2 : 3;
#define CK_INIT(call)                                                                          \
    do {                                                                                       \
        cudaError_t e__ = (call);                                                              \
        if (e__ != cudaSuccess) { fail(nullptr, CK_ERR_CUDA, #call, e__); ck_destroy(ctx); return CK_ERR_CUDA; } \
    } while (0)
    CK_INIT(cudaSetDevice(ctx->device));
    cudaDeviceProp prop;
    CK_INIT(cudaGetDeviceProperties(&prop, ctx->device));
    ctx->num_sms = prop.multiProcessorCount;
    Tables t; u8 secret[200];
    fill_tables(t, secret);
    CK_INIT(cudaMemcpyToSymbol(c_tab, &t, sizeof(t)));
    CK_INIT(cudaMemcpyToSymbol(c_secret, secret, sizeof(secret)));
    {
        u64 last[8], merge[8], mid[16];
        for (int i = 0; i < 8; i++) { memcpy(&last[i], secret + 121 + 8 * i, 8); memcpy(&merge[i], secret + 11 + 8 * i, 8); }
        for (int i = 0; i < 14; i++) memcpy(&mid[i], secret + 3 + 8 * i, 8);
        memcpy(&mid[14], secret + 119, 8); memcpy(&mid[15], secret + 127, 8);
        CK_INIT(cudaMemcpyToSymbol(c_lastsec, last, sizeof(last)));
        CK_INIT(cudaMemcpyToSymbol(c_mergesec, merge, sizeof(merge)));
        CK_INIT(cudaMemcpyToSymbol(c_midsec, mid, sizeof(mid)));
    }
    if (alloc_scratch(ctx, ctx->dev_scr)) { g_init_error = ctx->err; ck_destroy(ctx); return CK_ERR_CUDA; }
    if (alloc_scratch(ctx, ctx->lib_scr)) { g_init_error = ctx->err; ck_destroy(ctx); return CK_ERR_CUDA; }
    CK_INIT(cudaStreamCreateWithFlags(&ctx->lib_stream, cudaStreamNonBlocking));
    const u64 B = cfg->max_batch_bytes, R = cfg->max_batch_records;
    if (B || R) {
        for (int k = 0; k < 2; k++) {
            Slot &s = ctx->slot[k];
            CK_INIT(cudaStreamCreateWithFlags(&s.stream, cudaStreamNonBlocking));
            CK_INIT(cudaEventCreateWithFlags(&s.inserted, cudaEventDisableTiming));
            CK_INIT(cudaMalloc(&s.d_raw, B + 16));
            CK_INIT(cudaMalloc(&s.d_norm, B + 16));
            CK_INIT(cudaMalloc(&s.d_out, out_bytes_total(B, R) + 64));
            CK_INIT(cudaMalloc(&s.d_p2, p2_words(B, R) * 8));
            CK_INIT(cudaMalloc(&s.d_p4, p4_bytes_total(B, R)));
            CK_INIT(cudaMalloc(&s.d_off, (R + 1) * 8));
            CK_INIT(cudaMalloc(&s.d_len, (R + 1) * 4));
            CK_INIT(cudaMalloc(&s.d_lane, R + 1));
            CK_INIT(cudaMalloc(&s.d_start, (R + 1) * 4));
            CK_INIT(cudaMalloc(&s.d_strand, R + 1));
            CK_INIT(cudaMalloc(&s.d_hash, (R + 1) * 8));
            CK_INIT(cudaMalloc(&s.d_first, (R + 1) * 8));
            CK_INIT(cudaMalloc(&s.d_slotof, (R + 1) * 8));
            CK_INIT(cudaMalloc(&s.d_lists, lists_bytes_for(R)));
            CK_INIT(cudaMalloc(&s.d_counts, 64 * 4));
            CK_INIT(cudaMalloc(&s.d_dense, ((B >> 5) + R + 2) * 8));
            CK_INIT(cudaMalloc(&s.d_laneoff, (R + 1) * 8));
            CK_INIT(cudaMallocHost(&s.h_counts, 32 * 4));
            memset(s.h_counts, 0, 32 * 4);
            if (alloc_scratch(ctx, s.scr)) { g_init_error = ctx->err; ck_destroy(ctx); return CK_ERR_CUDA; }
        }
    }
    CK_INIT(cudaMalloc(&ctx->side, 8));
    CK_INIT(cudaMalloc(&ctx->d_overflow, 16));
    CK_INIT(cudaMemset(ctx->d_overflow, 0, 16));
    ctx->d_keys = reinterpret_cast<u64 *>(ctx->d_overflow + 2);
    if (cfg->table_capacity) {
        ctx->table_slots = table_slots_for(cfg->table_capacity);
        CK_INIT(cudaMalloc(&ctx->table, ctx->table_slots * sizeof(TableSlot)));
        k_table_clear<<<ctx->num_sms * 4, 256>>>(ctx->table, ctx->table_slots, ctx->side);
        CK_INIT(cudaGetLastError());
    }
    CK_INIT(cudaDeviceSynchronize());
#undef CK_INIT
    *out = ctx;
    return CK_OK;
}

void ck_destroy(ck_ctx *ctx)
{
    if (!ctx) return;
    cudaSetDevice(ctx->device);
    cudaDeviceSynchronize();
    for (int k = 0; k < 2; k++) {
        Slot &s = ctx->slot[k];
        void *ptrs[] = {s.d_raw, s.d_off, s.d_p2, s.d_norm, s.d_len, s.d_lane, s.d_out, s.d_start, s.d_strand,
                        s.d_hash, s.d_first, s.d_slotof, s.d_lists, s.d_counts, s.d_dense, s.d_laneoff, s.d_p4,
                        s.d_text, s.d_frame, s.d_rstart, s.d_head, s.d_seq, s.d_len64, s.d_fofs, s.d_meta, s.d_tiles};
        for (void *p : ptrs) if (p) cudaFree(p);
        if (s.h_counts) cudaFreeHost(s.h_counts);
        if (s.stream) cudaStreamDestroy(s.stream);
        {
            Slot::Deflate &z = s.z;
            void *zp[] = {z.buf, z.kA, z.kB, z.vA, z.vB, z.prev8, z.prev4, z.seg, z.out, z.result, z.tmp};
            for (void *p : zp) if (p) cudaFree(p);
            if (z.h_result) cudaFreeHost(z.h_result);
            if (z.stream) cudaStreamDestroy(z.stream);
        }
        if (s.inserted) cudaEventDestroy(s.inserted);
        free_scratch(s.scr);
    }
    free_scratch(ctx->dev_scr);
    free_scratch(ctx->lib_scr);
    if (ctx->lib_stream) cudaStreamDestroy(ctx->lib_stream);
    if (ctx->lib_h) cudaFreeHost(ctx->lib_h);
    if (ctx->lib_d) cudaFree(ctx->lib_d);
    {
        PeerGroup &P = ctx->peer;
        for (u32 r = 0; r < P.world && P.attached; r++) if (r != P.rank && P.mapped[r]) cudaIpcCloseMemHandle(P.mapped[r]);
        for (int k = 0; k < 2; k++) { if (P.pos[k]) cudaFree(P.pos[k]); if (P.cursors[k]) cudaFree(P.cursors[k]); if (P.slot_of[k]) cudaFree(P.slot_of[k]); }
        if (P.block) cudaFree(P.block);
    }
    if (ctx->table) cudaFree(ctx->table);
    if (ctx->side) cudaFree(ctx->side);
    if (ctx->d_overflow) cudaFree(ctx->d_overflow);
    delete ctx;
}

const char *ck_last_error(const ck_ctx *ctx) { return ctx ? ctx->err.c_str() : g_init_error.c_str(); }

void *ck_alloc_pinned(ck_ctx *ctx, size_t bytes)
{
    void *p = nullptr;
    if (ctx) cudaSetDevice(ctx->device);
    if (cudaMallocHost(&p, bytes ? bytes : 1) != cudaSuccess) { if (ctx) ctx->err = "cudaMallocHost failed"; return nullptr; }
    return p;
}
void ck_free_pinned(ck_ctx *, void *p) { if (p) cudaFreeHost(p); }

int ck_canon_submit(ck_ctx *ctx, int slot, const uint8_t *bytes, const uint64_t *offsets, uint32_t n_records, uint32_t flags)
{
    return submit_common(ctx, slot, bytes, offsets, n_records, flags, false, 0);
}
int ck_canon_wait(ck_ctx *ctx, int slot, uint8_t *out_bytes, uint32_t *out_len, uint32_t *out_start,
                  uint8_t *out_strand, uint64_t *out_hash64)
{
    return wait_common(ctx, slot, false, out_bytes, out_len, out_start, out_strand, out_hash64, nullptr);
}
int ck_uniq_submit(ck_ctx *ctx, int slot, const uint8_t *bytes, const uint64_t *offsets, uint32_t n_records,
                   uint32_t flags, uint64_t base_index)
{
    return submit_common(ctx, slot, bytes, offsets, n_records, flags, true, base_index);
}
int ck_uniq_wait(ck_ctx *ctx, int slot, uint8_t *out_bytes, uint32_t *out_len, uint64_t *out_hash64, uint64_t *out_first_index)
{
    return wait_common(ctx, slot, true, out_bytes, out_len, nullptr, nullptr, out_hash64, out_first_index);
}
int ck_canon_submit_packed(ck_ctx *ctx, int slot, const ck_packed_batch *batch, uint32_t flags)
{
    return submit_packed(ctx, slot, batch, flags, false, 0);
}
int ck_uniq_submit_packed(ck_ctx *ctx, int slot, const ck_packed_batch *batch, uint32_t flags, uint64_t base_index)
{
    return submit_packed(ctx, slot, batch, flags, true, base_index);
}
int ck_peer_export(ck_ctx *ctx, uint32_t world, uint32_t rank, uint32_t max_records, void *handle_out)
{
    if (!ctx || !handle_out || world < 1 || world > 32 || rank >= world || !max_records || (u64)world * max_records > 0xffffffffull)
        return ctx ? fail(ctx, CK_ERR_ARG, "bad peer group arguments") : CK_ERR_ARG;
    PeerGroup &P = ctx->peer;
    if (P.exported) return fail(ctx, CK_ERR_STATE, "peer block already exported");
    if (ctx->grow_max) return fail(ctx, CK_ERR_STATE, "a context whose uniq table grows (ck_uniq_grow) cannot join a peer group");
// ... 475 lines not shown
    if (rc) return rc;
    cudaStream_t st = ctx->lib_stream;
    const size_t R = n_records;
    const size_t off_bytes = (R + 1) * 8, in_bytes = off_bytes + ((total + 15) & ~15ull);
    const size_t res_bytes = R * 4 + ((R + 15) & ~15ull) + total;
    const bool small = n_records <= 256 && longest <= cls_max_n(CLS_C8);
    if (small) {
        if ((rc = lib_reserve(ctx, in_bytes + res_bytes + 64, in_bytes + res_bytes + 64))) return rc;
        u8 *h_in = ctx->lib_h, *h_res = ctx->lib_h + in_bytes;
        u8 *d_in = ctx->lib_d, *d_res = ctx->lib_d + in_bytes;
        memcpy(h_in, offsets, off_bytes);
        if (total) memcpy(h_in + off_bytes, bytes, total);
        CK_CUDA(ctx, cudaMemcpyAsync(d_in, h_in, off_bytes + total, cudaMemcpyHostToDevice, st));
        CanonArgs a{};
        a.bytes = d_in + off_bytes; a.offsets = reinterpret_cast<const u64 *>(d_in); a.n_direct = n_records;
        a.out_start = reinterpret_cast<u32 *>(d_res); a.out_strand = d_res + R * 4;
        a.out = out_bytes ? d_res + R * 4 + ((R + 15) & ~15ull) : nullptr;
        a.scratch = ctx->lib_scr.tie[CLS_C8]; a.scratch_stride = cls_tie_words(CLS_C8); a.smem_units = cls_units(CLS_C8);
        a.mode = mode; a.min_n = 1; a.max_n = cls_max_n(CLS_C8);
        const u32 grid = std::min<u32>(n_records, kCls[CLS_C8].ctas_per_sm * (u32)ctx->num_sms);
        k_canon_cta<8, false><<<grid, kCls[CLS_C8].threads, cls_smem_bytes(CLS_C8), st>>>(a);
        ctx->launches++;
        if (longest != offsets[n_records] / std::max<u32>(n_records, 1) || total == 0 || n_records > 1) {
            bool any_empty = false;
            for (u32 i = 0; i < n_records && !any_empty; i++) any_empty = offsets[i + 1] == offsets[i];
            if (any_empty) { k_canon_empty<<<1, 256, 0, st>>>(a); ctx->launches++; }
        }
        CK_CUDA(ctx, cudaGetLastError());
        CK_CUDA(ctx, cudaMemcpyAsync(h_res, d_res, out_bytes ? res_bytes : R * 4 + R, cudaMemcpyDeviceToHost, st));
        CK_CUDA(ctx, cudaStreamSynchronize(st));
        if (out_start) memcpy(out_start, h_res, R * 4);
        if (out_strand) memcpy(out_strand, h_res + R * 4, R);
        if (out_bytes && total) memcpy(out_bytes, h_res + R * 4 + ((R + 15) & ~15ull), total);
        return CK_OK;
    }
    size_t o = 0;
    auto take = [&](size_t bytes_) { const size_t at = o; o += (bytes_ + 255) & ~(size_t)255; return at; };
    const size_t o_raw = take(total + 16), o_norm = take(total + 16), o_out = take(total + 16), o_p2 = take(p2_words(total, R) * 8);
    const size_t o_off = take((R + 1) * 8), o_len = take(R * 4), o_lane = take(R), o_start = take(R * 4), o_strand = take(R);
    const size_t o_lists = take(lists_bytes_for(R)), o_counts = take(256);
    if ((rc = lib_reserve(ctx, 64, o))) return rc;
    u8 *d = ctx->lib_d;
    u32 h_counts[16] = {};
    CK_CUDA(ctx, cudaMemcpyAsync(d + o_off, offsets, (R + 1) * 8, cudaMemcpyHostToDevice, st));
    if (total) CK_CUDA(ctx, cudaMemcpyAsync(d + o_raw, bytes, total, cudaMemcpyHostToDevice, st));
    PrepareArgs pa{d + o_raw, (u64 *)(d + o_off), n_records, 1u << 2, (u64 *)(d + o_p2), d + o_norm, (u32 *)(d + o_len), d + o_lane};
    k_prepare<<<ctx->num_sms * 32, 256, 0, st>>>(pa);
    k_extend_packed2<<<extend_grid(ctx, n_records), 256, 0, st>>>((u64 *)(d + o_p2), (u64 *)(d + o_off), (u32 *)(d + o_len), d + o_lane, n_records, nullptr, 1u);
    ctx->launches += 2;
    CanonIO io{};
    io.packed2 = (u64 *)(d + o_p2); io.bytes = d + o_norm; io.offsets = (u64 *)(d + o_off); io.lens = (u32 *)(d + o_len); io.lane = d + o_lane;
    io.n = n_records; io.mode = mode; io.out = out_bytes ? d + o_out : nullptr; io.out_start = (u32 *)(d + o_start); io.out_strand = d + o_strand;
    io.out_hash = nullptr; io.lists = (u32 *)(d + o_lists); io.lists_bytes = lists_bytes_for(R); io.counts = (u32 *)(d + o_counts);
    io.longest = longest;
    rc = run_canon(ctx, st, ctx->lib_scr, io, 0);
    if (rc) return rc;
    CK_CUDA(ctx, cudaMemcpyAsync(h_counts, d + o_counts, 64, cudaMemcpyDeviceToHost, st));
    if (out_bytes && total) CK_CUDA(ctx, cudaMemcpyAsync(out_bytes, d + o_out, total, cudaMemcpyDeviceToHost, st));
    if (out_start) CK_CUDA(ctx, cudaMemcpyAsync(out_start, d + o_start, R * 4, cudaMemcpyDeviceToHost, st));
    if (out_strand) CK_CUDA(ctx, cudaMemcpyAsync(out_strand, d + o_strand, R, cudaMemcpyDeviceToHost, st));
    CK_CUDA(ctx, cudaStreamSynchronize(st));
    if (h_counts[CLS_HUGE]) return fail(ctx, CK_ERR_TOO_LONG, "record beyond the staged-length classes");
    return CK_OK;
}

int ck_lmsr_index_batch(ck_ctx *ctx, const uint8_t *bytes, const uint64_t *offsets, uint32_t n_records, uint32_t *out_index)
{
    return lib_batch(ctx, bytes, offsets, n_records, 1u, nullptr, out_index, nullptr);
}
int ck_lmsr_index(ck_ctx *ctx, const uint8_t *s, size_t n, size_t *out_index)
{
    if (!out_index) return ctx ? fail(ctx, CK_ERR_ARG, "null argument") : CK_ERR_ARG;
    if (n > (1ull << 30)) return fail(ctx, CK_ERR_TOO_LONG, "record longer than 2^30 symbols");
    uint64_t off[2] = {0, (uint64_t)n};
    uint32_t idx = 0;
    int rc = lib_batch(ctx, s, off, 1, 1u, nullptr, &idx, nullptr);
    *out_index = idx;
    return rc;
}
int ck_lmsr(ck_ctx *ctx, const uint8_t *s, size_t n, uint8_t *out)
{
    if (n > (1ull << 30)) return fail(ctx, CK_ERR_TOO_LONG, "record longer than 2^30 symbols");
    uint64_t off[2] = {0, (uint64_t)n};
    return lib_batch(ctx, s, off, 1, 1u, out, nullptr, nullptr);
}
int ck_canonicalize(ck_ctx *ctx, const uint8_t *s, size_t n, uint8_t *out)
{
    if (n > (1ull << 30)) return fail(ctx, CK_ERR_TOO_LONG, "record longer than 2^30 symbols");
    uint64_t off[2] = {0, (uint64_t)n};
    return lib_batch(ctx, s, off, 1, 0u, out, nullptr, nullptr);
}

uint64_t ck_dev_workspace_bytes(uint32_t n_records, uint64_t total_bytes)
{
    u64 b = 256 + lists_bytes_for(n_records);
    if (total_bytes) b += p2_words(total_bytes, n_records) * 8 + total_bytes + 64 + ((5ull * (n_records + 16) + 63) & ~63ull) + p4_bytes_total(total_bytes, n_records);
    return (b + 255) & ~255ull;
}
uint64_t ck_out_arena_bytes(uint64_t total_bytes, uint32_t n_records) { return out_bytes_total(total_bytes, n_records); }

int ck_dev_canon_packed2(ck_ctx *ctx, void *stream, const uint64_t *packed2, const uint64_t *offsets, uint32_t n_records,
                         uint32_t flags, uint32_t class_mask, uint8_t *out_bytes, uint32_t *out_start, uint8_t *out_strand,
                         uint64_t *out_hash64, void *workspace, uint64_t workspace_bytes)
{
    if (!ctx) return CK_ERR_ARG;
    if (workspace_bytes < ck_dev_workspace_bytes(n_records, 0)) return fail(ctx, CK_ERR_ARG, "workspace too small");
    CanonIO io{};
    io.packed2 = U(packed2); io.offsets = U(offsets); io.n = n_records; io.dbl = (flags & CK_F_SINGLE_COPY) ? 0u : 1u;
    io.mode = (flags & CK_F_ALIGNED_OUT) ? 2u : 0u;
    io.out = (flags & CK_F_NO_BYTES) ? nullptr : out_bytes; io.out_start = out_start; io.out_strand = out_strand; io.out_hash = U(out_hash64);
    io.counts = (u32 *)workspace; io.lists = (u32 *)((u8 *)workspace + 256); io.lists_bytes = lists_bytes_for(n_records);
    return run_canon(ctx, (cudaStream_t)stream, ctx->dev_scr, io, class_mask);
}
int ck_dev_canon_bytes(ck_ctx *ctx, void *stream, const uint8_t *bytes, const uint64_t *offsets, uint32_t n_records,
                       uint64_t total_bytes, uint32_t flags, uint32_t class_mask, uint8_t *out_bytes, uint32_t *out_len,
                       uint32_t *out_start, uint8_t *out_strand, uint64_t *out_hash64, void *workspace,
                       uint64_t workspace_bytes)
{
    if (!ctx) return CK_ERR_ARG;
    if (!n_records) return CK_OK;
    if (!out_len) return fail(ctx, CK_ERR_ARG, "out_len is required");
    if (workspace_bytes < ck_dev_workspace_bytes(n_records, total_bytes)) return fail(ctx, CK_ERR_ARG, "workspace too small");
    if (!total_bytes) {
        cudaStream_t st0 = (cudaStream_t)stream;
        CK_CUDA(ctx, cudaMemsetAsync(out_len, 0, (size_t)n_records * 4, st0));
        CanonIO io0{};
        io0.offsets = U(offsets); io0.lens = out_len; io0.n = n_records; io0.mode = (flags & CK_F_ALIGNED_OUT) ? 2u : 0u;
        io0.out_start = out_start; io0.out_strand = out_strand; io0.out_hash = U(out_hash64);
        io0.counts = (u32 *)workspace; io0.lists = (u32 *)((u8 *)workspace + 256); io0.lists_bytes = lists_bytes_for(n_records);
        return run_canon(ctx, st0, ctx->dev_scr, io0, class_mask);
    }
    u8 *w = (u8 *)workspace;
    u32 *counts = (u32 *)w; w += 256;
    u32 *lists = (u32 *)w; w += lists_bytes_for(n_records);
    u64 *p2 = (u64 *)w; w += p2_words(total_bytes, n_records) * 8;
    u8 *norm = w; w += (total_bytes + 63) & ~63ull;
    u8 *lane = w; w += ((size_t)n_records + 63) & ~63ull;
    u8 *p4 = w;
    cudaStream_t st = (cudaStream_t)stream;
    PrepareArgs pa{bytes, U(offsets), n_records, (flags & CK_F_NORMALIZE) | (1u << 2), p2, norm, out_len, lane};
    cudaEvent_t pe0 = nullptr, pe1 = nullptr;
    if (ctx->timing) { CK_CUDA(ctx, cudaEventCreate(&pe0)); CK_CUDA(ctx, cudaEventCreate(&pe1)); CK_CUDA(ctx, cudaEventRecord(pe0, st)); }
    k_prepare<<<ctx->num_sms * 32, 256, 0, st>>>(pa);
    k_extend_packed2<<<extend_grid(ctx, n_records), 256, 0, st>>>(p2, U(offsets), out_len, lane, n_records, nullptr, 1u);
    if (ctx->timing) { CK_CUDA(ctx, cudaEventRecord(pe1, st)); ctx->ev_pairs[CLS_COUNT + 6].push_back(pe0); ctx->ev_pairs[CLS_COUNT + 6].push_back(pe1); }
    ctx->launches += 2;
    CanonIO io{};
    io.packed2 = p2; io.bytes = norm; io.offsets = U(offsets); io.lens = out_len; io.lane = lane; io.n = n_records; io.p4 = p4;
    io.mode = (flags & CK_F_ALIGNED_OUT) ? 2u : 0u;
    io.out = (flags & CK_F_NO_BYTES) ? nullptr : out_bytes; io.out_start = out_start; io.out_strand = out_strand;
    io.out_hash = U(out_hash64); io.counts = counts; io.lists = lists; io.lists_bytes = lists_bytes_for(n_records);
    return run_canon(ctx, st, ctx->dev_scr, io, class_mask);
}
int ck_dev_check(ck_ctx *ctx, void *stream, const void *workspace)
{
    if (!ctx) return CK_ERR_ARG;
    u32 h[16];
    CK_CUDA(ctx, cudaMemcpyAsync(h, workspace, sizeof(h), cudaMemcpyDeviceToHost, (cudaStream_t)stream));
    CK_CUDA(ctx, cudaStreamSynchronize((cudaStream_t)stream));
    if (h[CLS_HUGE]) return fail(ctx, CK_ERR_TOO_LONG, "batch holds a record beyond the staged-length classes");
    return CK_OK;
}

uint64_t ck_dev_table_bytes(uint64_t capacity_keys) { return table_slots_for(capacity_keys) * sizeof(TableSlot) + 64; }
int ck_dev_table_clear(ck_ctx *ctx, void *stream, void *table, uint64_t table_bytes)
{
    TableSlot *slots; u64 nslots; u64 *side; u32 *ov;
    if (!ctx || !table_view(table, table_bytes, slots, nslots, side, ov)) return ctx ? fail(ctx, CK_ERR_ARG, "bad table") : CK_ERR_ARG;
    CK_CUDA(ctx, cudaMemsetAsync(table, 0, 64, (cudaStream_t)stream));
    k_table_clear<<<ctx->num_sms * 4, 256, 0, (cudaStream_t)stream>>>(slots, nslots, side);
    ctx->launches++;
    CK_CUDA(ctx, cudaGetLastError());
    return CK_OK;
}
int ck_dev_table_insert(ck_ctx *ctx, void *stream, void *table, uint64_t table_bytes, const uint64_t *hash64,
                        const uint64_t *index, uint64_t base_index, uint32_t n, uint64_t *slot_scratch)
{
    TableSlot *slots; u64 nslots; u64 *side; u32 *ov;
    if (!ctx || !table_view(table, table_bytes, slots, nslots, side, ov)) return ctx ? fail(ctx, CK_ERR_ARG, "bad table") : CK_ERR_ARG;
    return table_insert(ctx, (cudaStream_t)stream, slots, nslots, side, ov, U(hash64), U(index), base_index, n, U(slot_scratch));
}
int ck_dev_table_first(ck_ctx *ctx, void *stream, void *table, uint64_t table_bytes, const uint64_t *slot_scratch,
                       uint32_t n, uint64_t *out_first_index)
{
    TableSlot *slots; u64 nslots; u64 *side; u32 *ov;
    if (!ctx || !table_view(table, table_bytes, slots, nslots, side, ov)) return ctx ? fail(ctx, CK_ERR_ARG, "bad table") : CK_ERR_ARG;
    return table_first(ctx, (cudaStream_t)stream, slots, nslots, side, U(slot_scratch), n, U(out_first_index));
}
int ck_dev_table_insert_pairs(ck_ctx *ctx, void *stream, void *table, uint64_t table_bytes, const uint64_t *pairs, uint32_t n,
                              uint64_t *slot_scratch)
{
    TableSlot *slots; u64 nslots; u64 *side; u32 *ov;
    if (!ctx || !pairs || !table_view(table, table_bytes, slots, nslots, side, ov)) return ctx ? fail(ctx, CK_ERR_ARG, "bad table") : CK_ERR_ARG;
    return table_insert(ctx, (cudaStream_t)stream, slots, nslots, side, ov, U(pairs), U(pairs) + 1, 0, n, U(slot_scratch), 2);
}
int ck_dev_owner_partition(ck_ctx *ctx, void *stream, const uint64_t *hash64, uint32_t n, uint64_t base_index, uint32_t world,
                           uint64_t *send_pairs, uint32_t *pos, uint32_t *counts_dev, uint32_t *counts_host)
{
    if (!ctx || !hash64 || !send_pairs || !pos || !counts_dev || !counts_host || world < 1 || world > 32)
        return ctx ? fail(ctx, CK_ERR_ARG, "bad partition arguments") : CK_ERR_ARG;
    cudaStream_t st = (cudaStream_t)stream;
    CK_CUDA(ctx, cudaMemsetAsync(counts_dev, 0, 2 * world * sizeof(u32), st));
    OwnerArgs a{U(hash64), n, world, base_index, counts_dev, U(send_pairs), pos};
    if (n) {
        const u32 grid = std::min<u32>((n + 255) / 256, 8u * (u32)ctx->num_sms);
        k_owner_count<<<grid, 256, 0, st>>>(a);
        k_owner_scatter<<<grid, 256, 0, st>>>(a);
        ctx->launches += 2;
    }
    CK_CUDA(ctx, cudaMemcpyAsync(counts_host, counts_dev, world * sizeof(u32), cudaMemcpyDeviceToHost, st));
    CK_CUDA(ctx, cudaStreamSynchronize(st));
    return CK_OK;
}
int ck_dev_owner_partition_padded(ck_ctx *ctx, void *stream, const uint64_t *hash64, uint32_t n, uint64_t base_index,
                                  uint32_t world, uint32_t bucket_capacity, uint64_t *send_pairs, uint32_t *pos, uint32_t *cursors_dev)
{
    if (!ctx || !hash64 || !send_pairs || !pos || !cursors_dev || world < 1 || world > 32 || !bucket_capacity ||
        (u64)world * bucket_capacity > 0xffffffffull)
        return ctx ? fail(ctx, CK_ERR_ARG, "bad partition arguments") : CK_ERR_ARG;
    cudaStream_t st = (cudaStream_t)stream;
    CK_CUDA(ctx, cudaMemsetAsync(cursors_dev, 0, (world + 1) * sizeof(u32), st));
    OwnerPadArgs a{U(hash64), n, world, base_index, bucket_capacity, cursors_dev, U(send_pairs), pos};
    if (n) {
        k_owner_scatter_padded<<<std::min<u32>((n + 255) / 256, 8u * (u32)ctx->num_sms), 256, 0, st>>>(a);
        ctx->launches++;
    }
    k_owner_pad<<<dim3(16, world), 256, 0, st>>>(a);
    ctx->launches++;
    CK_CUDA(ctx, cudaGetLastError());
    return CK_OK;
}
int ck_dev_owner_scatter_peers(ck_ctx *ctx, void *stream, const uint64_t *hash64, uint32_t n, uint64_t base_index,
                               uint32_t world, uint32_t rank, uint32_t bucket_capacity, const uint64_t *peer_recv_ptrs,
                               uint32_t *pos, uint32_t *cursors_dev)
{
    if (!ctx || !hash64 || !peer_recv_ptrs || !pos || !cursors_dev || world < 1 || world > 32 || rank >= world || !bucket_capacity ||
        (u64)world * bucket_capacity > 0xffffffffull)
        return ctx ? fail(ctx, CK_ERR_ARG, "bad partition arguments") : CK_ERR_ARG;
    cudaStream_t st = (cudaStream_t)stream;
    CK_CUDA(ctx, cudaMemsetAsync(cursors_dev, 0, (world + 1) * sizeof(u32), st));
    OwnerPeerArgs a{};
    a.hash = U(hash64); a.n = n; a.world = world; a.rank = rank; a.base_index = base_index; a.cap = bucket_capacity;
    a.cursors = cursors_dev; a.pos = pos;
    for (u32 o = 0; o < world; o++) {
        if (!peer_recv_ptrs[o]) return fail(ctx, CK_ERR_ARG, "null peer pointer");
        a.recv.p[o] = reinterpret_cast<u64 *>(peer_recv_ptrs[o]);
    }
    if (n) {
        k_owner_scatter_peers<<<std::min<u32>((n + 255) / 256, 8u * (u32)ctx->num_sms), 256, 0, st>>>(a);
        ctx->launches++;
    }
    k_owner_pad_peers<<<dim3(16, world), 256, 0, st>>>(a);
    ctx->launches++;
    CK_CUDA(ctx, cudaGetLastError());
    return CK_OK;
}
int ck_dev_table_first_peers(ck_ctx *ctx, void *stream, void *table, uint64_t table_bytes, const uint64_t *slot_scratch,
                             uint32_t world, uint32_t rank, uint32_t bucket_capacity, const uint64_t *peer_ret_ptrs)
{
    TableSlot *slots; u64 nslots; u64 *side; u32 *ov;
    if (!ctx || !slot_scratch || !peer_ret_ptrs || world < 1 || world > 32 || rank >= world || !bucket_capacity ||
        !table_view(table, table_bytes, slots, nslots, side, ov))
        return ctx ? fail(ctx, CK_ERR_ARG, "bad table or peer arguments") : CK_ERR_ARG;
    FirstPeerArgs a{};
    a.slots = slots; a.side_first = side; a.slot_of = U(slot_scratch); a.world = world; a.rank = rank; a.cap = bucket_capacity;
    for (u32 s = 0; s < world; s++) {
        if (!peer_ret_ptrs[s]) return fail(ctx, CK_ERR_ARG, "null peer pointer");
        a.ret.p[s] = reinterpret_cast<u64 *>(peer_ret_ptrs[s]);
    }
    const u32 gx = std::max<u32>(1u, std::min<u32>((bucket_capacity + 255) / 256, (8u * (u32)ctx->num_sms + world - 1) / world));
    k_table_first_peers<<<dim3(gx, world), 256, 0, (cudaStream_t)stream>>>(a);
    ctx->launches++;
    CK_CUDA(ctx, cudaGetLastError());
    return CK_OK;
}
int ck_dev_gather_first(ck_ctx *ctx, void *stream, const uint64_t *ret, const uint32_t *pos, uint32_t n, uint64_t *out_first_index)
{
    if (!ctx || !ret || !pos || !out_first_index) return ctx ? fail(ctx, CK_ERR_ARG, "null argument") : CK_ERR_ARG;
    if (!n) return CK_OK;
    k_gather_first<<<std::min<u32>((n + 255) / 256, 16u * (u32)ctx->num_sms), 256, 0, (cudaStream_t)stream>>>(U(ret), pos, n, U(out_first_index));
    ctx->launches++;
    CK_CUDA(ctx, cudaGetLastError());
    return CK_OK;
}
int ck_dev_normalize(ck_ctx *ctx, void *stream, const uint8_t *bytes, const uint64_t *offsets, uint32_t n_records,
                     uint8_t *out_bytes, uint32_t *out_len)
{
    if (!ctx) return CK_ERR_ARG;
    if (!n_records) return CK_OK;
    if (!offsets || !out_bytes || !out_len) return fail(ctx, CK_ERR_ARG, "null argument");
    PrepareArgs pa{bytes, U(offsets), n_records, 1u | 2u | 4u, nullptr, out_bytes, out_len, nullptr};
    k_prepare<<<ctx->num_sms * 32, 256, 0, (cudaStream_t)stream>>>(pa);
    ctx->launches++;
    CK_CUDA(ctx, cudaGetLastError());
    return CK_OK;
}
int ck_dev_monomerize(ck_ctx *ctx, void *stream, const uint8_t *bytes, const uint64_t *offsets, const uint32_t *lens, uint32_t n_records,
                      uint32_t seed_len, uint64_t overlap_dist, double overlap_min_identity, uint32_t flags, uint32_t *out_end_index)
{
    if (!ctx) return CK_ERR_ARG;
    if (seed_len < 1 || seed_len > 63) return fail(ctx, CK_ERR_ARG, "Seed length must be at least 1 and at most 63");
    if (overlap_min_identity >= 0.0 && overlap_dist)
        return fail(ctx, CK_ERR_ARG, "Both overlap_dist and overlap_min_identity are set. They are mutually exclusive");
    if (!n_records) return CK_OK;
    if (!offsets || !out_end_index) return fail(ctx, CK_ERR_ARG, "null argument");
    MonoArgs a{};
    a.bytes = bytes; a.offsets = U(offsets); a.lens = lens; a.n_records = n_records; a.seed_len = seed_len;
    a.use_identity = overlap_min_identity >= 0.0 ? 1u : 0u; a.overlap_dist = overlap_dist;
    a.identity = overlap_min_identity; a.flags = flags; a.out_end = out_end_index;
    const u32 grid = std::min<u32>((n_records + 7) / 8, 16u * (u32)ctx->num_sms);
    k_monomerize<<<grid, 256, 0, (cudaStream_t)stream>>>(a);
    ctx->launches++;
    CK_CUDA(ctx, cudaGetLastError());
    return CK_OK;
}
uint64_t ck_launch_count(const ck_ctx *ctx) { return ctx ? ctx->launches : 0; }

int ck_kernel_timing(ck_ctx *ctx, int enable)
{
    if (!ctx) return CK_ERR_ARG;
    ctx->timing = enable != 0;
    return CK_OK;
}
int ck_kernel_times(ck_ctx *ctx, double *out_ms, uint32_t *out_launches, uint32_t n_classes)
{
    if (!ctx || !out_ms || !out_launches) return ctx ? fail(ctx, CK_ERR_ARG, "null argument") : CK_ERR_ARG;
    CK_CUDA(ctx, cudaDeviceSynchronize());
    for (u32 c = 0; c < n_classes; c++) { out_ms[c] = 0; out_launches[c] = 0; }
    for (u32 c = 0; c < (u32)CLS_COUNT + 7; c++) {
        std::vector<cudaEvent_t> &v = ctx->ev_pairs[c];
        for (size_t k = 0; k + 1 < v.size(); k += 2) {
            float ms = 0;
            cudaEventElapsedTime(&ms, v[k], v[k + 1]);
            if (c < n_classes) { out_ms[c] += ms; out_launches[c]++; }
            cudaEventDestroy(v[k]); cudaEventDestroy(v[k + 1]);
        }
        v.clear();
    }
    return CK_OK;
}

int ck_synth_offsets(ck_ctx *ctx, void *stream, uint64_t seed, uint64_t first_index, uint32_t n_records, uint32_t kind,
                     uint32_t lo, uint32_t hi, uint32_t dup_permille, uint64_t *offsets_dev, uint64_t *total_out_host)
{
    if (!ctx || !offsets_dev || lo < 1 || hi < lo) return ctx ? fail(ctx, CK_ERR_ARG, "bad synth arguments") : CK_ERR_ARG;
    cudaStream_t st = (cudaStream_t)stream;
    u64 *lens = nullptr; void *tmp = nullptr; size_t tmp_bytes = 0;
    CK_CUDA(ctx, cudaMalloc(&lens, ((size_t)n_records + 1) * 8));
    CK_CUDA(ctx, cudaMemsetAsync(lens, 0, ((size_t)n_records + 1) * 8, st));
    SynthArgs a{seed, n_records, kind, lo, hi, dup_permille, 0, first_index};
    if (n_records) k_synth_lens<<<(n_records + 255) / 256, 256, 0, st>>>(a, lens);
    ctx->launches++;
    cub::DeviceScan::ExclusiveSum(nullptr, tmp_bytes, lens, U(offsets_dev), (int)n_records + 1, st);
    CK_CUDA(ctx, cudaMalloc(&tmp, tmp_bytes ? tmp_bytes : 8));
    cub::DeviceScan::ExclusiveSum(tmp, tmp_bytes, lens, U(offsets_dev), (int)n_records + 1, st);
    ctx->launches++;
    u64 total = 0;
    CK_CUDA(ctx, cudaMemcpyAsync(&total, offsets_dev + n_records, 8, cudaMemcpyDeviceToHost, st));
    CK_CUDA(ctx, cudaStreamSynchronize(st));
    cudaFree(lens); cudaFree(tmp);
    if (total_out_host) *total_out_host = total;
    return CK_OK;
}
uint64_t ck_packed2_words(uint64_t total_bytes, uint32_t n_records, uint32_t flags)
{
    return p2_words(total_bytes, n_records, (flags & CK_F_SINGLE_COPY) ? 0u : 1u);
}
int ck_synth_packed2(ck_ctx *ctx, void *stream, uint64_t seed, uint64_t first_index, uint32_t n_records,
                     const uint64_t *offsets_dev, uint32_t dup_permille, uint32_t adversarial_permille, uint64_t *packed2_dev,
                     uint32_t flags)
{
    const u32 dbl = (flags & CK_F_SINGLE_COPY) ? 0u : 1u;
    if (!ctx || !offsets_dev || !packed2_dev) return ctx ? fail(ctx, CK_ERR_ARG, "bad synth arguments") : CK_ERR_ARG;
    SynthArgs a{seed, n_records, 0, 0, 0, dup_permille, adversarial_permille, first_index};
    if (n_records) {
        k_synth_packed2<<<ctx->num_sms * 8, 256, 0, (cudaStream_t)stream>>>(a, U(offsets_dev), U(packed2_dev), dbl);
        k_extend_packed2<<<extend_grid(ctx, n_records), 256, 0, (cudaStream_t)stream>>>(U(packed2_dev), U(offsets_dev), nullptr, nullptr, n_records, nullptr, dbl);
    }
    ctx->launches += 2;
    CK_CUDA(ctx, cudaGetLastError());
    return CK_OK;
}
int ck_dev_unpack2(ck_ctx *ctx, void *stream, const uint64_t *packed2, const uint64_t *offsets, uint32_t n_records, uint8_t *ascii_out,
                   uint32_t flags)
{
    if (!ctx) return CK_ERR_ARG;
    if (n_records) k_unpack2<<<ctx->num_sms * 8, 256, 0, (cudaStream_t)stream>>>(U(packed2), U(offsets), n_records, ascii_out,
                                                                                 (flags & CK_F_SINGLE_COPY) ? 0u : 1u);
    ctx->launches++;
    CK_CUDA(ctx, cudaGetLastError());
    return CK_OK;
}

}
```

circkit_b200/device.py:

```python
from __future__ import annotations

import ctypes as C

import torch

from . import _native as N
from .core import Context

CLASS_NAMES = ["2bit_le_512", "2bit_le_2048", "2bit_le_65536", "2bit_le_425984", "4bit_le_2048", "4bit_le_212992",
               "byte_le_1024", "byte_le_106496", "huge", "empty", "2bit_le_4096", "2bit_le_8192", "2bit_lane_128_8192",
               "table_insert", "table_first", "2bit_seg_8193_425984", "4bit_lane_129_2048", "pack4", "prepare"]
BYTE_CLASSES = ("4bit_le_2048", "4bit_le_212992", "byte_le_1024", "byte_le_106496")
CLASS_RANGE = {"2bit_le_512": (1, 512), "2bit_le_2048": (513, 2048), "2bit_le_4096": (2049, 4096), "2bit_le_8192": (4097, 8192),
               "2bit_le_65536": (8193, 65536), "2bit_le_425984": (65537, 425984), "2bit_lane_128_8192": (1, 8192), "2bit_seg_8193_425984": (8193, 425984)}


def class_mask_for(lo: int, hi: int) -> int:
    m = 0
    for name, (a, b) in CLASS_RANGE.items():
        if "lane" not in name and "seg" not in name and lo <= b and hi >= a:
            m |= 1 << CLASS_NAMES.index(name)
    return m


def _stream() -> int:
    return torch.cuda.current_stream().cuda_stream


def _p(t):
    return None if t is None else t.data_ptr()


class DeviceBatch:

    def __init__(self, offsets: torch.Tensor, packed2: torch.Tensor, n_records: int, total: int, single: bool = False):
        self.offsets, self.packed2, self.n, self.total = offsets, packed2, n_records, total
        self.single = single

    @property
    def layout_flag(self) -> int:
        return N.CK_F_SINGLE_COPY if self.single else 0

    @property
    def lens(self) -> torch.Tensor:
        return self.offsets[1:] - self.offsets[:-1]


def synth_batch(ctx: Context, *, seed: int, first_index: int, n_records: int, kind: int, lo: int, hi: int,
                dup_permille: int = 0, adversarial_permille: int = 0, device=None, single: bool | None = None) -> DeviceBatch:
    if single is None:
        single = hi <= 512
    lf = N.CK_F_SINGLE_COPY if single else 0
    dev = device or torch.device("cuda", ctx.device)
    offsets = torch.empty(n_records + 1, dtype=torch.int64, device=dev)
    total = C.c_uint64(0)
    ctx._check(ctx._lib.ck_synth_offsets(ctx.handle, _stream(), seed, first_index, n_records, kind, lo, hi,
                                         dup_permille, _p(offsets), C.byref(total)))
    words = int(ctx._lib.ck_packed2_words(total.value, n_records, lf))
    packed2 = torch.empty(words, dtype=torch.int64, device=dev)
    ctx._check(ctx._lib.ck_synth_packed2(ctx.handle, _stream(), seed, first_index, n_records, _p(offsets),
                                         dup_permille, adversarial_permille, _p(packed2), lf))
    return DeviceBatch(offsets, packed2, n_records, total.value, single)


def unpack_ascii(ctx: Context, b: DeviceBatch, n_records: int | None = None) -> torch.Tensor:
    n = b.n if n_records is None else n_records
    total = int(b.offsets[n].item())
    out = torch.empty(max(total, 1), dtype=torch.uint8, device=b.offsets.device)
    ctx._check(ctx._lib.ck_dev_unpack2(ctx.handle, _stream(), _p(b.packed2), _p(b.offsets), n, _p(out), b.layout_flag))
    return out[:total]


class CanonOutputs:
    def __init__(self, n: int, total: int, dev, want_bytes=True, want_hash=True, aligned=False):
        self.aligned = aligned
        nbytes = 32 * ((total >> 5) + n) + 32 if aligned else max(total, 1) + 16
        self.out = torch.empty(nbytes, dtype=torch.uint8, device=dev) if want_bytes else None
        self.start = torch.empty(max(n, 1), dtype=torch.int32, device=dev)
        self.strand = torch.empty(max(n, 1), dtype=torch.uint8, device=dev)
        self.hash = torch.empty(max(n, 1), dtype=torch.int64, device=dev) if want_hash else None


class Workspace:
    def __init__(self, ctx: Context, n_records: int, total_bytes: int = 0, dev=None):
        self.bytes = int(ctx._lib.ck_dev_workspace_bytes(n_records, total_bytes))
        self.buf = torch.empty(self.bytes, dtype=torch.uint8, device=dev or torch.device("cuda", ctx.device))


def canon_packed2(ctx: Context, b: DeviceBatch, outs: CanonOutputs, ws: Workspace, class_mask: int = 0):
    flags = (N.CK_F_ALIGNED_OUT if outs.aligned else 0) | (0 if outs.out is not None else N.CK_F_NO_BYTES) | b.layout_flag
    ctx._check(ctx._lib.ck_dev_canon_packed2(ctx.handle, _stream(), _p(b.packed2), _p(b.offsets), b.n, flags, class_mask,
                                             _p(outs.out), _p(outs.start), _p(outs.strand), _p(outs.hash),
                                             _p(ws.buf), ws.bytes))


def canon_bytes(ctx: Context, raw: torch.Tensor, offsets: torch.Tensor, n: int, total: int, outs: CanonOutputs,
                lens_out: torch.Tensor, ws: Workspace, normalize: bool, class_mask: int = 0):
    flags = ((N.CK_F_NORMALIZE if normalize else 0) | (N.CK_F_ALIGNED_OUT if outs.aligned else 0)
             | (0 if outs.out is not None else N.CK_F_NO_BYTES))
    ctx._check(ctx._lib.ck_dev_canon_bytes(ctx.handle, _stream(), _p(raw), _p(offsets), n, total, flags, class_mask,
                                           _p(outs.out), _p(lens_out), _p(outs.start), _p(outs.strand), _p(outs.hash),
                                           _p(ws.buf), ws.bytes))


def check(ctx: Context, ws: Workspace):
    ctx._check(ctx._lib.ck_dev_check(ctx.handle, _stream(), _p(ws.buf)))


class DeviceTable:

    def __init__(self, ctx: Context, capacity_keys: int, dev=None):
        self.ctx = ctx
        self.bytes = int(ctx._lib.ck_dev_table_bytes(capacity_keys))
        self.buf = torch.empty(self.bytes, dtype=torch.uint8, device=dev or torch.device("cuda", ctx.device))
        self.clear()

    def clear(self):
        self.ctx._check(self.ctx._lib.ck_dev_table_clear(self.ctx.handle, _stream(), _p(self.buf), self.bytes))

    def insert(self, hash64: torch.Tensor, n: int, slot_scratch: torch.Tensor, index: torch.Tensor | None = None,
               base_index: int = 0):
        self.ctx._check(self.ctx._lib.ck_dev_table_insert(self.ctx.handle, _stream(), _p(self.buf), self.bytes,
                                                          _p(hash64), _p(index), base_index, n, _p(slot_scratch)))

    def insert_pairs(self, pairs: torch.Tensor, n: int, slot_scratch: torch.Tensor):
        self.ctx._check(self.ctx._lib.ck_dev_table_insert_pairs(self.ctx.handle, _stream(), _p(self.buf), self.bytes,
                                                                _p(pairs), n, _p(slot_scratch)))

    def first(self, slot_scratch: torch.Tensor, n: int, out_first: torch.Tensor):
        self.ctx._check(self.ctx._lib.ck_dev_table_first(self.ctx.handle, _stream(), _p(self.buf), self.bytes,
                                                         _p(slot_scratch), n, _p(out_first)))


class OwnerPartitioner:

    def __init__(self, ctx: Context, n: int, world: int, dev=None):
        dev = dev or torch.device("cuda", ctx.device)
        self.ctx, self.world = ctx, world
        self.pairs = torch.empty((max(n, 1), 2), dtype=torch.int64, device=dev)
        self.pos = torch.empty(max(n, 1), dtype=torch.int32, device=dev)
        self.counts_dev = torch.zeros(2 * world, dtype=torch.int32, device=dev)
        self.counts_host = (C.c_uint32 * world)()
        self._padded, self._state = None, None

    def __call__(self, hash64: torch.Tensor, base_index: int, world: int):
        n = hash64.numel()
        assert world == self.world and n <= self.pairs.shape[0]
        self.ctx._check(self.ctx._lib.ck_dev_owner_partition(self.ctx.handle, _stream(), _p(hash64), n, base_index, world,
                                                             _p(self.pairs), _p(self.pos), _p(self.counts_dev),
                                                             self.counts_host))
        return self.pairs[:n], self.pos[:n], [int(c) for c in self.counts_host]

    def bucket_capacity(self, n: int) -> int:
        return exchange_bucket_capacity(n, self.world)

    def padded(self, hash64: torch.Tensor, base_index: int, world: int):
        n = hash64.numel()
        cap = self.bucket_capacity(n)
        assert world == self.world and n <= self.pos.shape[0]
        if self._padded is None or self._padded.shape[0] != world * cap:
            self._padded = torch.empty((world * cap, 2), dtype=torch.int64, device=self.pos.device)
            self._state = torch.zeros(world + 1, dtype=torch.int32, device=self.pos.device)
        self.ctx._check(self.ctx._lib.ck_dev_owner_partition_padded(self.ctx.handle, _stream(), _p(hash64), n, base_index, world,
                                                                    cap, _p(self._padded), _p(self.pos), _p(self._state)))
        return self._padded, self.pos[:n], self._state


class PeerExchange:

    def __init__(self, ctx: Context, n_max: int, world: int, rank: int, dev=None, group=None):
        import torch.distributed as dist
        import torch.distributed._symmetric_memory as symm_mem
        dev = dev or torch.device("cuda", ctx.device)
        self.ctx, self.world, self.rank = ctx, world, rank
        self.cap = exchange_bucket_capacity(n_max, world)
        m = world * self.cap
        self.m = m
        self.recv = symm_mem.empty((m, 2), dtype=torch.int64, device=dev)
        self.ret = symm_mem.empty(m, dtype=torch.int64, device=dev)
        group = group or dist.group.WORLD
        self.h_recv = symm_mem.rendezvous(self.recv, group)
        self.h_ret = symm_mem.rendezvous(self.ret, group)
        self.recv_ptrs = (C.c_uint64 * world)(*[int(p) for p in self.h_recv.buffer_ptrs])
        self.ret_ptrs = (C.c_uint64 * world)(*[int(p) for p in self.h_ret.buffer_ptrs])
        self.pos = torch.empty(max(n_max, 1), dtype=torch.int32, device=dev)
        self.state = torch.zeros(world + 1, dtype=torch.int32, device=dev)
        self.slots = torch.empty(m, dtype=torch.int64, device=dev)

    def first_index(self, hash64: torch.Tensor, base_index: int, table: "DeviceTable", out: torch.Tensor) -> torch.Tensor:
        n = hash64.numel()
        assert n <= self.pos.shape[0] and out.numel() >= n
        lib, h = self.ctx._lib, self.ctx.handle
        self.ctx._check(lib.ck_dev_owner_scatter_peers(h, _stream(), _p(hash64), n, base_index, self.world, self.rank, self.cap,
                                                       self.recv_ptrs, _p(self.pos), _p(self.state)))
        self.h_recv.barrier()
        table.insert_pairs(self.recv, self.m, self.slots)
        self.ctx._check(lib.ck_dev_table_first_peers(h, _stream(), _p(table.buf), table.bytes, _p(self.slots), self.world,
                                                     self.rank, self.cap, self.ret_ptrs))
        self.h_ret.barrier()
        self.ctx._check(lib.ck_dev_gather_first(h, _stream(), _p(self.ret), _p(self.pos), n, _p(out)))
        return self.state


class PeerGroup:

    def __init__(self, ctx: Context, n_max: int, world: int, rank: int, group=None):
        import torch.distributed as dist
        self.ctx, self.world, self.rank = ctx, world, rank
        mine = ctx.peer_export(world, rank, n_max)
        handles = [None] * world
        dist.all_gather_object(handles, mine, group=group)
        ctx.peer_attach(handles)

    def first_index(self, hash64: torch.Tensor, base_index: int, table: "DeviceTable", out: torch.Tensor):
        n = hash64.numel()
        self.ctx._check(self.ctx._lib.ck_dev_peer_first_index(self.ctx.handle, _stream(), _p(hash64), n, base_index, _p(table.buf),
                                                              table.bytes, _p(out)))


def exchange_bucket_capacity(n: int, world: int) -> int:
    mean = n / world
    return int(mean + 8.0 * (mean ** 0.5) + 64) + 1


def kernel_times(ctx: Context):
    n = len(CLASS_NAMES)
    ms = (C.c_double * n)()
    cnt = (C.c_uint32 * n)()
    ctx._check(ctx._lib.ck_kernel_times(ctx.handle, ms, cnt, n))
    return {CLASS_NAMES[i]: (ms[i], cnt[i]) for i in range(n)}


def algorithmic_bytes(lens: torch.Tensor, uniq: bool, lo: int = 1, hi: int = 1 << 62) -> int:
    sel = lens[(lens >= lo) & (lens <= hi)]
    b = (8 * ((sel + 31) // 32) + sel + 16).sum()
    if uniq:
        b = b + 40 * sel.numel()
    return int(b.item())
```

include/circkit_b200.h:

```cpp
#ifndef CIRCKIT_B200_H
#define CIRCKIT_B200_H

#include <stddef.h>
#include <stdint.h>

#ifdef __cplusplus
extern "C" {
#endif

#define CK_OK 0
#define CK_ERR_CUDA (-1)
#define CK_ERR_ARG (-2)
#define CK_ERR_STATE (-3)
#define CK_ERR_TOO_LONG (-4)
#define CK_ERR_TABLE_FULL (-5)

#define CK_F_NORMALIZE 1u
#define CK_F_NO_BYTES 2u
#define CK_F_ALIGNED_OUT 4u

#define CK_F_SURVIVORS 16u
#define CK_F_SINGLE_COPY 32u
#define CK_F_PACKED_IN 8u

typedef struct ck_ctx ck_ctx;

typedef struct ck_config {
    int32_t device;
    uint64_t max_batch_bytes;
    uint32_t max_batch_records;
    uint64_t table_capacity;
} ck_config;

int ck_init(const ck_config *cfg, ck_ctx **out);
void ck_destroy(ck_ctx *ctx);
const char *ck_last_error(const ck_ctx *ctx);
void *ck_alloc_pinned(ck_ctx *ctx, size_t bytes);
void ck_free_pinned(ck_ctx *ctx, void *p);

int ck_canon_submit(ck_ctx *ctx, int slot, const uint8_t *bytes, const uint64_t *offsets,
                    uint32_t n_records, uint32_t flags);
int ck_canon_wait(ck_ctx *ctx, int slot, uint8_t *out_bytes, uint32_t *out_len, uint32_t *out_start,
                  uint8_t *out_strand, uint64_t *out_hash64);

int ck_uniq_submit(ck_ctx *ctx, int slot, const uint8_t *bytes, const uint64_t *offsets,
                   uint32_t n_records, uint32_t flags, uint64_t base_index);
int ck_uniq_wait(ck_ctx *ctx, int slot, uint8_t *out_bytes, uint32_t *out_len, uint64_t *out_hash64,
                 uint64_t *out_first_index);
int ck_uniq_wait_survivors(ck_ctx *ctx, int slot, uint32_t *out_n_survivors, uint32_t *out_index, uint64_t *out_compact_offsets,
                           uint8_t *out_compact_bytes, uint32_t *out_len, uint64_t *out_hash64, uint64_t *out_first_index);
int ck_uniq_reset(ck_ctx *ctx);
int ck_uniq_grow(ck_ctx *ctx, uint64_t max_keys);
int ck_uniq_table_info(ck_ctx *ctx, uint64_t *out_keys, uint64_t *out_capacity_keys, uint64_t *out_grows);

typedef struct ck_packed_batch {
    const uint64_t *packed2;
    const uint64_t *offsets;
    const uint32_t *lens;
    const uint8_t *lane;
    const uint8_t *lane_bytes;
    const uint64_t *lane_offsets;
    uint64_t lane_bytes_total;
    uint32_t n_records;
} ck_packed_batch;
uint64_t ck_pack2_words(uint64_t total_bytes, uint32_t n_records);
int ck_pack2_host(const uint8_t *bytes, const uint64_t *offsets, uint32_t n_records, uint32_t flags, uint32_t threads,
                  uint64_t *packed2_dense, uint32_t *lens, uint8_t *lane, uint8_t *lane_bytes, uint64_t lane_bytes_capacity,
                  uint64_t *lane_offsets, uint64_t *lane_bytes_total);
int ck_canon_submit_packed(ck_ctx *ctx, int slot, const ck_packed_batch *batch, uint32_t flags);
int ck_uniq_submit_packed(ck_ctx *ctx, int slot, const ck_packed_batch *batch, uint32_t flags, uint64_t base_index);

#define CK_PEER_HANDLE_BYTES 64
int ck_peer_export(ck_ctx *ctx, uint32_t world, uint32_t rank, uint32_t max_records, void *handle_out);
int ck_peer_attach(ck_ctx *ctx, const void *all_handles);
int ck_dev_peer_first_index(ck_ctx *ctx, void *stream, const uint64_t *hash64, uint32_t n, uint64_t base_index, void *table,
                            uint64_t table_bytes, uint64_t *out_first_index);

int ck_lmsr_index(ck_ctx *ctx, const uint8_t *s, size_t n, size_t *out_index);
int ck_lmsr(ck_ctx *ctx, const uint8_t *s, size_t n, uint8_t *out);
int ck_canonicalize(ck_ctx *ctx, const uint8_t *s, size_t n, uint8_t *out);
int ck_lmsr_index_batch(ck_ctx *ctx, const uint8_t *bytes, const uint64_t *offsets, uint32_t n_records,
                        uint32_t *out_index);

#define CK_CLASS_2BIT_LE_512 (1u << 0)
#define CK_CLASS_2BIT_LE_2048 (1u << 1)
#define CK_CLASS_2BIT_LE_65536 (1u << 2)
#define CK_CLASS_2BIT_LE_425984 (1u << 3)
#define CK_CLASS_2BIT_LE_4096 (1u << 10)
#define CK_CLASS_2BIT_LE_8192 (1u << 11)
uint64_t ck_dev_workspace_bytes(uint32_t n_records, uint64_t total_bytes );
uint64_t ck_out_arena_bytes(uint64_t total_bytes, uint32_t n_records);
uint64_t ck_packed2_words(uint64_t total_bytes, uint32_t n_records, uint32_t flags );
int ck_dev_canon_packed2(ck_ctx *ctx, void *stream, const uint64_t *packed2, const uint64_t *offsets,
                         uint32_t n_records, uint32_t flags, uint32_t class_mask, uint8_t *out_bytes, uint32_t *out_start,
                         uint8_t *out_strand, uint64_t *out_hash64, void *workspace, uint64_t workspace_bytes);
int ck_dev_canon_bytes(ck_ctx *ctx, void *stream, const uint8_t *bytes, const uint64_t *offsets,
                       uint32_t n_records, uint64_t total_bytes, uint32_t flags, uint32_t class_mask,
                       uint8_t *out_bytes, uint32_t *out_len, uint32_t *out_start, uint8_t *out_strand,
                       uint64_t *out_hash64, void *workspace, uint64_t workspace_bytes);
int ck_dev_check(ck_ctx *ctx, void *stream, const void *workspace);
uint64_t ck_dev_table_bytes(uint64_t capacity_keys);
int ck_dev_table_clear(ck_ctx *ctx, void *stream, void *table, uint64_t table_bytes);
int ck_dev_table_insert(ck_ctx *ctx, void *stream, void *table, uint64_t table_bytes, const uint64_t *hash64,
                        const uint64_t *index, uint64_t base_index, uint32_t n, uint64_t *slot_scratch);
int ck_dev_table_first(ck_ctx *ctx, void *stream, void *table, uint64_t table_bytes, const uint64_t *slot_scratch,
                       uint32_t n, uint64_t *out_first_index);
int ck_dev_owner_partition(ck_ctx *ctx, void *stream, const uint64_t *hash64, uint32_t n, uint64_t base_index, uint32_t world,
                           uint64_t *send_pairs, uint32_t *pos, uint32_t *counts_dev, uint32_t *counts_host);
int ck_dev_table_insert_pairs(ck_ctx *ctx, void *stream, void *table, uint64_t table_bytes, const uint64_t *pairs, uint32_t n,
                              uint64_t *slot_scratch);
int ck_dev_owner_partition_padded(ck_ctx *ctx, void *stream, const uint64_t *hash64, uint32_t n, uint64_t base_index,
                                  uint32_t world, uint32_t bucket_capacity, uint64_t *send_pairs, uint32_t *pos,
                                  uint32_t *cursors_dev);
int ck_dev_owner_scatter_peers(ck_ctx *ctx, void *stream, const uint64_t *hash64, uint32_t n, uint64_t base_index,
                               uint32_t world, uint32_t rank, uint32_t bucket_capacity, const uint64_t *peer_recv_ptrs,
                               uint32_t *pos, uint32_t *cursors_dev);
int ck_dev_table_first_peers(ck_ctx *ctx, void *stream, void *table, uint64_t table_bytes, const uint64_t *slot_scratch,
                             uint32_t world, uint32_t rank, uint32_t bucket_capacity, const uint64_t *peer_ret_ptrs);
int ck_dev_gather_first(ck_ctx *ctx, void *stream, const uint64_t *ret, const uint32_t *pos, uint32_t n, uint64_t *out_first_index);
#define CK_MONO_SENSITIVE 1u
#define CK_MONO_FIRST_ONLY 2u
#define CK_MONO_NONE 0xffffffffu
int ck_dev_monomerize(ck_ctx *ctx, void *stream, const uint8_t *bytes, const uint64_t *offsets, const uint32_t *lens,
                      uint32_t n_records, uint32_t seed_len, uint64_t overlap_dist, double overlap_min_identity, uint32_t flags,
                      uint32_t *out_end_index);
int ck_dev_normalize(ck_ctx *ctx, void *stream, const uint8_t *bytes, const uint64_t *offsets, uint32_t n_records,
                     uint8_t *out_bytes, uint32_t *out_len);
#define CK_MONO_KEEP_ALL 4u
typedef struct ck_mono_options {
    uint32_t seed_len;
    uint32_t flags;
    uint64_t overlap_dist;
    double overlap_min_identity;
    uint64_t min_length;
    uint64_t max_length;
    uint64_t min_overlap;
    double min_overlap_percent;
} ck_mono_options;
int ck_mono_submit(ck_ctx *ctx, int slot, const uint8_t *bytes, const uint64_t *offsets, uint32_t n_records,
                   uint32_t flags , const ck_mono_options *opt);
int ck_mono_wait(ck_ctx *ctx, int slot, uint32_t *out_n_written, uint32_t *out_index, uint64_t *out_compact_offsets,
                 uint8_t *out_compact_bytes, uint32_t *out_monomer_len, uint32_t *out_full_len, uint32_t *out_end_index);

#define CK_CMD_CANONICALIZE 1
#define CK_CMD_UNIQ 2
#define CK_CMD_MONOMERIZE 3
#define CK_F_CANONICAL_BODY 64u
uint64_t ck_fasta_out_bytes(uint64_t text_bytes, uint32_t n_records);
int ck_fasta_submit(ck_ctx *ctx, int slot, const uint8_t *text, uint64_t text_bytes, uint32_t command, uint32_t flags,
                    uint64_t base_index, const ck_mono_options *mono, uint32_t *out_n_records);
int ck_fasta_wait(ck_ctx *ctx, int slot, uint8_t *out_fasta, uint64_t *out_fasta_bytes, uint32_t *out_n_written,
                  uint32_t *out_index, uint64_t *out_head, uint64_t *out_first_index, uint32_t *out_full_len,
                  uint32_t *out_monomer_len);
#define CK_DEFLATE_MAX_BYTES (64ull << 20)
#define CK_DEFLATE_DICT_BYTES 32768u
uint64_t ck_deflate_bound(uint64_t n);
int ck_deflate_submit(ck_ctx *ctx, int slot, const uint8_t *bytes, uint64_t n, const uint8_t *dict, uint32_t dict_bytes,
                      uint32_t crc_in);
int ck_deflate_wait(ck_ctx *ctx, int slot, uint8_t *out, uint64_t *out_bytes, uint32_t *crc_out);

uint64_t ck_launch_count(const ck_ctx *ctx);
int ck_kernel_timing(ck_ctx *ctx, int enable);
int ck_kernel_times(ck_ctx *ctx, double *out_ms, uint32_t *out_launches, uint32_t n_classes);

int ck_synth_offsets(ck_ctx *ctx, void *stream, uint64_t seed, uint64_t first_index, uint32_t n_records,
                     uint32_t kind, uint32_t lo, uint32_t hi, uint32_t dup_permille, uint64_t *offsets_dev,
                     uint64_t *total_out_host);
int ck_synth_packed2(ck_ctx *ctx, void *stream, uint64_t seed, uint64_t first_index, uint32_t n_records,
                     const uint64_t *offsets_dev, uint32_t dup_permille, uint32_t adversarial_permille,
                     uint64_t *packed2_dev, uint32_t flags );
int ck_dev_unpack2(ck_ctx *ctx, void *stream, const uint64_t *packed2, const uint64_t *offsets, uint32_t n_records,
                   uint8_t *ascii_out, uint32_t flags );

#ifdef __cplusplus
}
#endif
#endif
```

Measured before the change: 1.456 billion.

## Replace radix-sort work list with tiled counting sort and 128-bit table CAS

Builds the per-class record work list with a custom two-pass tiled counting sort (per-tile histogram, exclusive scan, stable warp-aggregated scatter) instead of classify plus a CUB radix sort and a separate list-starts launch. The intent is to cut sort passes and launches on the canonicalize path. The hash table insert also gains a 128-bit atom.cas variant that claims key and first index in one atomic, replacing the separate key CAS and atomicMin, when the slots are 16-byte aligned. Both paths keep fallbacks behind context flags, and they add code complexity and per-step __syncthreads in the scatter.

```diff
diff --git a/circkit_b200/_native.py b/circkit_b200/_native.py
--- a/circkit_b200/_native.py
+++ b/circkit_b200/_native.py
@@ -71,6 +71,7 @@
     "ck_dev_canon_packed2": (_i, [_vp, _vp, _vp, _vp, _u32, _u32, _u32, _vp, _vp, _vp, _vp, _vp, _u64]),
     "ck_dev_canon_bytes": (_i, [_vp, _vp, _vp, _vp, _u32, _u64, _u32, _u32, _vp, _vp, _vp, _vp, _vp, _vp, _u64]),
     "ck_dev_check": (_i, [_vp, _vp, _vp]),
+    "ck_dev_work_list": (_i, [_vp, _vp, _vp, _vp, _vp, _u32, _vp, _u64, _vp]),
     "ck_dev_table_bytes": (_u64, [_u64]),
     "ck_dev_table_clear": (_i, [_vp, _vp, _vp, _u64]),
     "ck_dev_table_insert": (_i, [_vp, _vp, _vp, _u64, _vp, _vp, _u64, _u32, _vp]),
diff --git a/circkit_b200/csrc/ck_kernels.cuh b/circkit_b200/csrc/ck_kernels.cuh
--- a/circkit_b200/csrc/ck_kernels.cuh
+++ b/circkit_b200/csrc/ck_kernels.cuh
@@ -45,16 +45,39 @@
 struct TableSlot { u64 key; u64 first; };
 #define CK_EMPTY_KEY 0xffffffffffffffffULL
 __device__ __forceinline__ u64 table_home(u64 key, u64 nslots) { return __umul64hi((key ^ (key >> 29)) * 0x9E3779B97F4A7C15ULL, nslots); }
-__device__ __forceinline__ u64 table_insert_one(TableSlot *slots, u64 nslots, u64 *side_first, u32 *overflow, u64 key, u64 idx)
-{
-    if (key == CK_EMPTY_KEY) { atomicMin(side_first, idx); return ~0ULL; }
+__device__ __forceinline__ TableSlot slot_cas(TableSlot *p, TableSlot cmp, TableSlot val)
+{
+    TableSlot old;
+    asm volatile("{\n\t.reg .b128 c, v, d;\n\t"
+                 "mov.b128 c, {%2, %3};\n\t"
+                 "mov.b128 v, {%4, %5};\n\t"
+                 "atom.global.cas.b128 d, [%6], c, v;\n\t"
+                 "mov.b128 {%0, %1}, d;\n\t}"
+                 : "=l"(old.key), "=l"(old.first)
+                 : "l"(cmp.key), "l"(cmp.first), "l"(val.key), "l"(val.first), "l"(p) : "memory");
+    return old;
+}
+template <bool WIDE>
+__device__ __forceinline__ u64 table_insert_one(TableSlot *slots, u64 nslots, u64 key, u64 idx, bool &claimed)
+{
     u64 s = table_home(key, nslots);
     for (u64 probes = 0; probes < nslots; probes++) {
-        const u64 prev = atomicCAS(&slots[s].key, CK_EMPTY_KEY, key);
-        if (prev == CK_EMPTY_KEY || prev == key) { atomicMin(&slots[s].first, idx); return s; }
+        if (WIDE) {
+            TableSlot cmp{CK_EMPTY_KEY, ~0ULL};
+            for (;;) {
+                const TableSlot prev = slot_cas(slots + s, cmp, TableSlot{key, idx});
+                if (prev.key == cmp.key && prev.first == cmp.first) { claimed = prev.key == CK_EMPTY_KEY; return s; }
+                if (prev.key != key && prev.key != CK_EMPTY_KEY) break;
+                if (prev.key == key && prev.first <= idx) { claimed = false; return s; }
+                cmp = prev;
+            }
+        } else {
+            const u64 prev = atomicCAS(&slots[s].key, CK_EMPTY_KEY, key);
+            if (prev == CK_EMPTY_KEY || prev == key) { atomicMin(&slots[s].first, idx); claimed = prev == CK_EMPTY_KEY; return s; }
+        }
         s = s + 1 == nslots ? 0 : s + 1;
     }
-    *overflow = 1;
+    claimed = false;
     return ~0ULL - 1;
 }
 
@@ -413,6 +436,21 @@
     }
 }
 
+__device__ __forceinline__ int record_class(u32 n, u32 bits)
+{
+    if (n == 0) return CLS_EMPTY;
+    if (bits == 2) return n <= cls_max_n(CLS_W2S) ? CLS_W2S : n <= cls_max_n(CLS_W2M) ? CLS_W2M
+                        : n <= cls_max_n(CLS_W2L) ? CLS_W2L : n <= cls_max_n(CLS_W2X) ? CLS_W2X
+                        : n <= cls_max_n(CLS_C2A) ? CLS_C2A : n <= cls_max_n(CLS_C2B) ? CLS_C2B : CLS_HUGE;
+    if (bits == 4 || bits == 3) return n <= cls_max_n(CLS_W4) ? CLS_W4 : n <= cls_max_n(CLS_C4) ? CLS_C4 : CLS_HUGE;
+    return n <= cls_max_n(CLS_W8) ? CLS_W8 : n <= cls_max_n(CLS_C8) ? CLS_C8 : CLS_HUGE;
+}
+__device__ __forceinline__ u32 quarter_octave(u32 n)
+{
+    const u32 msb = 31u - __clz(n | 1u);
+    return (msb << 2) | (((n << (31u - msb)) >> 29) & 3u);
+}
+
 struct ClassifyArgs {
     const u64 *offsets; const u32 *lens; const u8 *lane;
     u32 n_records;
@@ -435,13 +473,7 @@
         u32 n = 0;
         if (i < a.n_records) {
             n = a.lens ? a.lens[i] : (u32)(a.offsets[i + 1] - a.offsets[i]);
-            const u32 bits = a.lane ? a.lane[i] : 2u;
-            if (n == 0) cls = CLS_EMPTY;
-            else if (bits == 2) cls = n <= cls_max_n(CLS_W2S) ? CLS_W2S : n <= cls_max_n(CLS_W2M) ? CLS_W2M
-                                    : n <= cls_max_n(CLS_W2L) ? CLS_W2L : n <= cls_max_n(CLS_W2X) ? CLS_W2X
-                                    : n <= cls_max_n(CLS_C2A) ? CLS_C2A : n <= cls_max_n(CLS_C2B) ? CLS_C2B : CLS_HUGE;
-            else if (bits == 4 || bits == 3) cls = n <= cls_max_n(CLS_W4) ? CLS_W4 : n <= cls_max_n(CLS_C4) ? CLS_C4 : CLS_HUGE;
-            else cls = n <= cls_max_n(CLS_W8) ? CLS_W8 : n <= cls_max_n(CLS_C8) ? CLS_C8 : CLS_HUGE;
+            cls = record_class(n, a.lane ? a.lane[i] : 2u);
         }
         if (a.direct_mask) {
             const u32 m = __ballot_sync(CK_FULL, cls >= 0 && !((a.direct_mask >> cls) & 1u));
@@ -454,7 +486,7 @@
             u32 key = (cls_rank(cls) << 10) | bin;
             if (a.window_shift < 32u) {
                 const bool lane_cls = cls == CLS_W2S || cls == CLS_W2M || cls == CLS_W2L || cls == CLS_W2X;
-                const u32 q = (msb << 2) | (((n << (31u - msb)) >> 29) & 3u);
+                const u32 q = quarter_octave(n);
                 key = lane_cls ? (((i >> a.window_shift) << 5) | (q > 28u ? q - 28u : 0u)) : (key | (1u << a.top_bit));
             }
             a.keys[i] = key; a.vals[i] = i;
@@ -470,20 +502,22 @@
     __syncthreads();
     if (threadIdx.x < 16 && cnt[threadIdx.x]) atomicAdd(a.counts + threadIdx.x, cnt[threadIdx.x]);
 }
+__device__ __forceinline__ void write_list_starts(u32 *counts)
+{
+    u32 s = 0;
+    for (u32 r = 0; r < (u32)CLS_COUNT; r++) {
+        const int c = cls_of_rank(r);
+        counts[16 + c] = s; counts[48 + c] = s;
+        s += counts[c];
+    }
+    counts[12] = counts[CLS_W2S] + counts[CLS_W2M] + counts[CLS_W2L] + counts[CLS_W2X];
+    counts[28] = counts[16 + CLS_W2S];
+    counts[13] = counts[CLS_C2A] + counts[CLS_C2B];
+    counts[29] = counts[16 + CLS_C2A];
+}
 __global__ void k_list_starts(u32 *counts)
 {
-    if (threadIdx.x == 0) {
-        u32 s = 0;
-        for (u32 r = 0; r < (u32)CLS_COUNT; r++) {
-            const int c = cls_of_rank(r);
-            counts[16 + c] = s; counts[48 + c] = s;
-            s += counts[c];
-        }
-        counts[12] = counts[CLS_W2S] + counts[CLS_W2M] + counts[CLS_W2L] + counts[CLS_W2X];
-        counts[28] = counts[16 + CLS_W2S];
-        counts[13] = counts[CLS_C2A] + counts[CLS_C2B];
-        counts[29] = counts[16 + CLS_C2A];
-    }
+    if (threadIdx.x == 0) write_list_starts(counts);
 }
 
 __device__ __forceinline__ u32 p2_last_unit(u32 n) { return max((2u * n + 143u) >> 4, (n >> 4) + 5u); }
@@ -567,6 +601,7 @@
     u32 *overflow;
     u64 *keys;
 };
+template <bool WIDE>
 __global__ void __launch_bounds__(256) k_table_insert(TableArgs a)
 {
     const u32 i = blockIdx.x * blockDim.x + threadIdx.x;
@@ -575,21 +610,14 @@
     const u64 idx = a.index ? a.index[(size_t)i * a.stride] : a.base_index + i;
     if (idx == ~0ULL) { a.slot_of[i] = ~0ULL - 1; return; }
     if (key == CK_EMPTY_KEY) { atomicMin(a.side_first, idx); a.slot_of[i] = ~0ULL; return; }
-    u64 s = table_home(key, a.nslots);
-    for (u64 probes = 0; probes < a.nslots; probes++) {
-        u64 prev = atomicCAS(&a.slots[s].key, CK_EMPTY_KEY, key);
-        if (prev == CK_EMPTY_KEY || prev == key) {
-            atomicMin(&a.slots[s].first, idx);
-            a.slot_of[i] = s;
-            if (a.keys && prev == CK_EMPTY_KEY) {
-                const u32 m = __activemask();
-                if ((threadIdx.x & 31) == (u32)(__ffs(m) - 1)) atomicAdd(a.keys, (u64)__popc(m));
-            }
-            return;
-        }
-        s = s + 1 == a.nslots ? 0 : s + 1;
-    }
-    *a.overflow = 1; a.slot_of[i] = ~0ULL - 1;
+    bool claimed;
+    const u64 s = table_insert_one<WIDE>(a.slots, a.nslots, key, idx, claimed);
+    a.slot_of[i] = s;
+    if (s == ~0ULL - 1) { *a.overflow = 1; return; }
+    if (a.keys && claimed) {
+        const u32 m = __activemask();
+        if ((threadIdx.x & 31) == (u32)(__ffs(m) - 1)) atomicAdd(a.keys, (u64)__popc(m));
+    }
 }
 __global__ void __launch_bounds__(256) k_table_first(TableArgs a)
 {
@@ -840,6 +868,7 @@
     u32 world, rank, cap;
     PeerBlockPtrs ret;
 };
+template <bool WIDE>
 __global__ void __launch_bounds__(256) k_table_insert_regions(RegionArgs a)
 {
     const u32 s = blockIdx.y;
@@ -850,13 +879,8 @@
         const ulonglong2 pr = pairs[k];
         const u64 key = pr.x, idx = pr.y;
         if (key == CK_EMPTY_KEY) { atomicMin(a.side_first, idx); slot_of[k] = ~0ULL; continue; }
-        u64 sl = table_home(key, a.nslots);
-        u64 found = ~0ULL - 1;
-        for (u64 probes = 0; probes < a.nslots; probes++) {
-            const u64 prev = atomicCAS(&a.slots[sl].key, CK_EMPTY_KEY, key);
-            if (prev == CK_EMPTY_KEY || prev == key) { atomicMin(&a.slots[sl].first, idx); found = sl; break; }
-            sl = sl + 1 == a.nslots ? 0 : sl + 1;
-        }
+        bool claimed;
+        const u64 found = table_insert_one<WIDE>(a.slots, a.nslots, key, idx, claimed);
         if (found == ~0ULL - 1) *a.overflow = 1;
         slot_of[k] = found;
     }
diff --git a/circkit_b200/csrc/ck_lib.cu b/circkit_b200/csrc/ck_lib.cu
--- a/circkit_b200/csrc/ck_lib.cu
+++ b/circkit_b200/csrc/ck_lib.cu
@@ -14,6 +14,7 @@
 
 #include "../../include/circkit_b200.h"
 #include "ck_kernels.cuh"
+#include "ck_worklist.cuh"
 #include "ck_warp2.cuh"
 #include "ck_lane2.cuh"
 #include "ck_stream2.cuh"
@@ -158,8 +159,10 @@
     bool l4_kernel = true;
     bool seg_kernel = true;
     int lane_kernel = 3;
+    bool table_cas64 = false;
+    bool list_cub = false;
     bool timing = false;
-    std::vector<cudaEvent_t> ev_pairs[CLS_COUNT + 7];
+    std::vector<cudaEvent_t> ev_pairs[CLS_COUNT + 8];
 };
 
 namespace {
@@ -302,6 +305,52 @@
 
 u64 lists_bytes_for(u64 n) { return ((16 * (n + 4) + 24 * (n + 4) + 255) & ~255ull) + (1ull << 20); }
 
+void list_windows(u32 n, u32 &window_shift, u32 &top_bit)
+{
+    window_shift = 16;
+    u32 wbits = 0;
+    while ((((u64)n - 1) >> window_shift) >> wbits) wbits++;
+    top_bit = std::max(14u, 5u + wbits);
+}
+
+int work_list(ck_ctx *ctx, cudaStream_t st, const CanonIO &io, u32 window_shift, u32 top_bit, const u32 *&sorted, u32 *&retry)
+{
+    const u64 stride = ((u64)io.n + 4) & ~3ull;
+    u32 *k0 = io.lists, *k1 = k0 + stride, *v0 = k1 + stride, *v1 = v0 + stride;
+    void *tmp = v1 + stride;
+    const size_t tmp_bytes = (size_t)(io.lists_bytes - 16 * stride);
+    if (window_shift < 32 && !ctx->list_cub) {
+        const u32 tile_shift = window_shift - CK_WL_TILE_SHIFT;
+        const u32 n_tiles = (u32)(((((u64)io.n - 1) >> window_shift) + 1) << tile_shift);
+        const u64 cells = (u64)n_tiles * CK_WL_BUCKETS, padded = (cells + 63) & ~63ull;
+        u32 *tile_counts = reinterpret_cast<u32 *>(tmp), *tile_base = tile_counts + padded;
+        size_t need = 0;
+        cub::DeviceScan::ExclusiveSum(nullptr, need, tile_counts, tile_base, (int)cells, st);
+        if (8 * padded + need > tmp_bytes) return fail(ctx, CK_ERR_ARG, "sort workspace too small");
+        const WorkListArgs wa{io.offsets, io.lens, io.lane, io.n, tile_shift, n_tiles, io.counts, tile_counts, tile_base, v0,
+                            reinterpret_cast<u16 *>(k0)};
+        k_wl_count<<<n_tiles, CK_WL_THREADS, 0, st>>>(wa);
+        CK_CUDA(ctx, cub::DeviceScan::ExclusiveSum(tile_base + padded, need, tile_counts, tile_base, (int)cells, st));
+        k_wl_scatter<<<n_tiles, CK_WL_THREADS, 0, st>>>(wa);
+        ctx->launches += 3;
+        sorted = v0;
+        retry = v1;
+        return CK_OK;
+    }
+    ClassifyArgs ca{io.offsets, io.lens, io.lane, io.n, k0, v0, io.counts, 0u, window_shift, top_bit};
+    k_classify<<<std::min<u32>((io.n + 255) / 256, 16u * (u32)ctx->num_sms), 256, 0, st>>>(ca);
+    cub::DoubleBuffer<u32> keys(k0, k1), vals(v0, v1);
+    size_t need = 0;
+    cub::DeviceRadixSort::SortPairs(nullptr, need, keys, vals, (int)io.n, 0, (int)top_bit + 1, st);
+    if (need > tmp_bytes) return fail(ctx, CK_ERR_ARG, "sort workspace too small");
+    CK_CUDA(ctx, cub::DeviceRadixSort::SortPairs(tmp, need, keys, vals, (int)io.n, 0, (int)top_bit + 1, st));
+    k_list_starts<<<1, 32, 0, st>>>(io.counts);
+    ctx->launches += 3;
+    sorted = vals.Current();
+    retry = vals.Alternate();
+    return CK_OK;
+}
+
 int run_canon(ck_ctx *ctx, cudaStream_t st, ExecScratch &scr, const CanonIO &io, u32 class_mask)
 {
     if (io.n == 0) return CK_OK;
@@ -312,16 +361,11 @@
     if (class_mask && (class_mask & (class_mask - 1)) == 0)
         for (int c = 0; c < CLS_COUNT; c++) if (class_mask == (1u << c)) only = c;
     const u64 stride = ((u64)io.n + 4) & ~3ull;
-    u32 *k0 = io.lists, *k1 = k0 + stride, *v0 = k1 + stride, *v1 = v0 + stride;
+    u32 *k0 = io.lists, *v0 = k0 + 2 * stride;
     if (io.lists_bytes < 16 * stride) return fail(ctx, CK_ERR_ARG, "sort workspace too small");
     const bool fastv = io.packed2 && !(io.mode & 1u) && (!io.out || (io.mode & 2u)) && io.out_start && io.out_strand;
     u32 window_shift = 32, top_bit = 13;
-    if (fastv && only < 0) {
-        window_shift = 16;
-        u32 wbits = 0;
-        while ((((u64)io.n - 1) >> window_shift) >> wbits) wbits++;
-        top_bit = std::max(14u, 5u + wbits);
-    }
+    if (fastv && only < 0) list_windows(io.n, window_shift, top_bit);
     const bool l4_run = fastv && only < 0 && ctx->l4_kernel && io.p4 && io.lane && io.bytes && (!class_mask || (class_mask & (1u << CLS_W4)));
     if (l4_run) {
         cudaEvent_t e0 = nullptr, e1 = nullptr;
@@ -330,29 +374,8 @@
         if (ctx->timing) { CK_CUDA(ctx, cudaEventRecord(e1, st)); ctx->ev_pairs[CLS_COUNT + 5].push_back(e0); ctx->ev_pairs[CLS_COUNT + 5].push_back(e1); }
         ctx->launches++;
     }
-    const int sort_bits = (int)top_bit + 1;
     const bool lane_checks = fastv && only >= 0 && io.lane == nullptr &&
                              (only == CLS_W2S || only == CLS_W2M || only == CLS_W2L || only == CLS_W2X);
-    if (!lane_checks) {
-        ClassifyArgs ca{io.offsets, io.lens, io.lane, io.n, k0, v0, io.counts, only >= 0 ? (1u << only) : 0u, window_shift, top_bit};
-        k_classify<<<std::min<u32>((io.n + 255) / 256, 16u * (u32)ctx->num_sms), 256, 0, st>>>(ca);
-        ctx->launches++;
-    }
-    const u32 *sorted = nullptr;
-    u32 *retry = v0;
-    if (only < 0) {
-        cub::DoubleBuffer<u32> keys(k0, k1), vals(v0, v1);
-        void *tmp = v1 + stride;
-        size_t tmp_bytes = (size_t)(io.lists_bytes - 16 * stride), need = 0;
-        cub::DeviceRadixSort::SortPairs(nullptr, need, keys, vals, (int)io.n, 0, sort_bits, st);
-        if (need > tmp_bytes) return fail(ctx, CK_ERR_ARG, "sort workspace too small");
-        CK_CUDA(ctx, cub::DeviceRadixSort::SortPairs(tmp, need, keys, vals, (int)io.n, 0, sort_bits, st));
-        sorted = vals.Current();
-        retry = vals.Alternate();
-        k_list_starts<<<1, 32, 0, st>>>(io.counts);
-        ctx->launches += 2;
-    }
-    const u32 lane_classes = (1u << CLS_W2S) | (1u << CLS_W2M) | (1u << CLS_W2L) | (1u << CLS_W2X);
     auto timed = [&](int slot, cudaEvent_t &e0, cudaEvent_t &e1, bool begin, cudaStream_t on) -> cudaError_t {
         if (!ctx->timing) return cudaSuccess;
         if (begin) {
@@ -363,6 +386,20 @@
         ctx->ev_pairs[slot].push_back(e0); ctx->ev_pairs[slot].push_back(e1);
         return cudaEventRecord(e1, on);
     };
+    const u32 *sorted = nullptr;
+    u32 *retry = v0;
+    if (only >= 0 && !lane_checks) {
+        ClassifyArgs ca{io.offsets, io.lens, io.lane, io.n, k0, v0, io.counts, 1u << only, window_shift, top_bit};
+        k_classify<<<std::min<u32>((io.n + 255) / 256, 16u * (u32)ctx->num_sms), 256, 0, st>>>(ca);
+        ctx->launches++;
+    }
+    if (only < 0) {
+        cudaEvent_t e0 = nullptr, e1 = nullptr;
+        CK_CUDA(ctx, timed(CLS_COUNT + 7, e0, e1, true, st));
+        if ((rc = work_list(ctx, st, io, window_shift, top_bit, sorted, retry))) return rc;
+        CK_CUDA(ctx, timed(CLS_COUNT + 7, e0, e1, false, st));
+    }
+    const u32 lane_classes = (1u << CLS_W2S) | (1u << CLS_W2M) | (1u << CLS_W2L) | (1u << CLS_W2X);
     auto base_args = [&](int c) {
         CanonArgs a{};
         a.packed2 = io.packed2; a.p2_dbl = io.dbl; a.bytes = io.bytes; a.offsets = io.offsets; a.lens = io.lens;
@@ -496,12 +533,15 @@
 
 u64 table_slots_for(u64 keys) { return std::max<u64>(1024, keys + keys / 2 + 16); }
 
+bool table_wide(const ck_ctx *ctx, const TableSlot *slots) { return !ctx->table_cas64 && ((uintptr_t)slots & 15u) == 0; }
+
 int table_insert(ck_ctx *ctx, cudaStream_t st, TableSlot *slots, u64 nslots, u64 *side, u32 *overflow,
                  const u64 *hash, const u64 *index, u64 base, u32 n, u64 *slot_of, u32 stride = 1, u64 *keys = nullptr)
 {
     if (!n) return CK_OK;
     TableArgs t{slots, nslots, side, hash, index, stride, base, n, slot_of, nullptr, overflow, keys};
-    k_table_insert<<<(n + 255) / 256, 256, 0, st>>>(t);
+    if (table_wide(ctx, slots)) k_table_insert<true><<<(n + 255) / 256, 256, 0, st>>>(t);
+    else k_table_insert<false><<<(n + 255) / 256, 256, 0, st>>>(t);
     ctx->launches++;
     CK_CUDA(ctx, cudaGetLastError());
     return CK_OK;
@@ -593,7 +633,8 @@
     ra.recv = P.recv(P.rank, slot); ra.counts = P.counts(P.rank, slot); ra.slot_of = P.slot_of[slot];
     ra.world = P.world; ra.rank = P.rank; ra.cap = P.cap;
     const u32 gx = std::max<u32>(1u, std::min<u32>((P.cap + 255) / 256, (8u * (u32)ctx->num_sms + P.world - 1) / P.world));
-    k_table_insert_regions<<<dim3(gx, P.world), 256, 0, st>>>(ra);
+    if (table_wide(ctx, table)) k_table_insert_regions<true><<<dim3(gx, P.world), 256, 0, st>>>(ra);
+    else k_table_insert_regions<false><<<dim3(gx, P.world), 256, 0, st>>>(ra);
     if (insert_done) CK_CUDA(ctx, cudaEventRecord(insert_done, st));
     if (wait_before_query) CK_CUDA(ctx, cudaStreamWaitEvent(st, wait_before_query, 0));
     k_table_first_regions<<<dim3(gx, P.world), 256, 0, st>>>(ra);
@@ -903,6 +944,8 @@
     if (const char *sk = getenv("CK_SEG_KERNEL")) ctx->seg_kernel = atoi(sk) != 0;
     if (const char *lk = getenv("CK_L4_KERNEL")) ctx->l4_kernel = atoi(lk) != 0;
     if (const char *lk = getenv("CK_LANE_KERNEL")) ctx->lane_kernel = atoi(lk) == 2 ? 2 : 3;
+    if (const char *ls = getenv("CK_LIST_SORT")) ctx->list_cub = strcmp(ls, "cub") == 0;
+    if (const char *tc = getenv("CK_TABLE_CAS")) ctx->table_cas64 = atoi(tc) == 64;
 #define CK_INIT(call)                                                                          \
     do {                                                                                       \
         cudaError_t e__ = (call);                                                              \
@@ -1684,6 +1727,26 @@
     io.out_hash = U(out_hash64); io.counts = counts; io.lists = lists; io.lists_bytes = lists_bytes_for(n_records);
     return run_canon(ctx, st, ctx->dev_scr, io, class_mask);
 }
+int ck_dev_work_list(ck_ctx *ctx, void *stream, const uint64_t *offsets, const uint32_t *lens, const uint8_t *lane_bits,
+                     uint32_t n_records, void *workspace, uint64_t workspace_bytes, uint32_t *out_list)
+{
+    if (!ctx) return CK_ERR_ARG;
+    if (!offsets || !out_list) return fail(ctx, CK_ERR_ARG, "null argument");
+    if (workspace_bytes < ck_dev_workspace_bytes(n_records, 0)) return fail(ctx, CK_ERR_ARG, "workspace too small");
+    if (!n_records) return CK_OK;
+    cudaStream_t st = (cudaStream_t)stream;
+    CanonIO io{};
+    io.offsets = U(offsets); io.lens = lens; io.lane = lane_bits; io.n = n_records;
+    io.counts = (u32 *)workspace; io.lists = (u32 *)((u8 *)workspace + 256); io.lists_bytes = lists_bytes_for(n_records);
+    CK_CUDA(ctx, cudaMemsetAsync(io.counts, 0, 64 * sizeof(u32), st));
+    u32 window_shift, top_bit;
+    list_windows(n_records, window_shift, top_bit);
+    const u32 *sorted = nullptr; u32 *retry = nullptr;
+    const int rc = work_list(ctx, st, io, window_shift, top_bit, sorted, retry);
+    if (rc) return rc;
+    CK_CUDA(ctx, cudaMemcpyAsync(out_list, sorted, (size_t)n_records * 4, cudaMemcpyDeviceToDevice, st));
+    return CK_OK;
+}
 int ck_dev_check(ck_ctx *ctx, void *stream, const void *workspace)
 {
     if (!ctx) return CK_ERR_ARG;
@@ -1859,7 +1922,7 @@
     if (!ctx || !out_ms || !out_launches) return ctx ? fail(ctx, CK_ERR_ARG, "null argument") : CK_ERR_ARG;
     CK_CUDA(ctx, cudaDeviceSynchronize());
     for (u32 c = 0; c < n_classes; c++) { out_ms[c] = 0; out_launches[c] = 0; }
-    for (u32 c = 0; c < (u32)CLS_COUNT + 7; c++) {
+    for (u32 c = 0; c < (u32)CLS_COUNT + 8; c++) {
         std::vector<cudaEvent_t> &v = ctx->ev_pairs[c];
         for (size_t k = 0; k + 1 < v.size(); k += 2) {
             float ms = 0;
diff --git a/circkit_b200/csrc/ck_worklist.cuh b/circkit_b200/csrc/ck_worklist.cuh
--- /dev/null
+++ b/circkit_b200/csrc/ck_worklist.cuh
@@ -0,0 +1,145 @@
+#pragma once
+#include "ck_kernels.cuh"
+
+namespace ck {
+
+constexpr u32 CK_WL_TILE_SHIFT = 14, CK_WL_TILE = 1u << CK_WL_TILE_SHIFT;
+constexpr u32 CK_WL_THREADS = 256, CK_WL_WARPS = CK_WL_THREADS / 32;
+constexpr u32 CK_WL_BATCH = 8;
+static_assert(CK_WL_TILE % (CK_WL_BATCH * CK_WL_THREADS) == 0 && CK_WL_BATCH % 2 == 0, "tile = whole batches, even batch");
+constexpr u32 CK_WL_LANE_BUCKETS = 32;
+constexpr u32 CK_WL_BUCKETS = CK_WL_LANE_BUCKETS + 8u * 128u;
+static_assert(cls_rank(CLS_W2S) < 4 && cls_rank(CLS_W2M) < 4 && cls_rank(CLS_W2L) < 4 && cls_rank(CLS_W2X) < 4,
+              "the lane-kernel classes lead the list");
+
+struct WorkListArgs {
+    const u64 *offsets; const u32 *lens; const u8 *lane;
+    u32 n_records;
+    u32 tile_shift;
+    u32 n_tiles;
+    u32 *counts;
+    u32 *tile_counts;
+    const u32 *tile_base;
+    u32 *list;
+    u16 *bucket;
+};
+
+constexpr u64 CK_WL_RANKS = 0x32BA98765410ull;
+__host__ __device__ constexpr bool wl_ranks_match(int c) { return c == CLS_COUNT || (((CK_WL_RANKS >> (4 * c)) & 15u) == cls_rank(c) && wl_ranks_match(c + 1)); }
+static_assert(wl_ranks_match(0), "CK_WL_RANKS = cls_rank");
+__device__ __forceinline__ u32 wl_bucket(int cls, u32 n)
+{
+    const u32 q = quarter_octave(n), rank = (u32)(CK_WL_RANKS >> (4 * cls)) & 15u;
+    if (rank < 4u) return q > 28u ? q - 28u : 0u;
+    return CK_WL_LANE_BUCKETS + ((rank - 4u) << 7) + q;
+}
+__device__ __forceinline__ u32 wl_slot(const WorkListArgs &a, u32 t, u32 b)
+{
+    if (b < CK_WL_LANE_BUCKETS) {
+        const u32 w = t >> a.tile_shift;
+        return ((w * CK_WL_LANE_BUCKETS + b) << a.tile_shift) + (t & ((1u << a.tile_shift) - 1u));
+    }
+    return CK_WL_LANE_BUCKETS * a.n_tiles + (b - CK_WL_LANE_BUCKETS) * a.n_tiles + t;
+}
+__device__ __forceinline__ void wl_load(const WorkListArgs &a, u64 i, u32 &n, u32 &bits)
+{
+    n = 0; bits = 0;
+    if (i >= a.n_records) return;
+    n = a.lens ? a.lens[i] : (u32)(a.offsets[i + 1] - a.offsets[i]);
+    bits = a.lane ? a.lane[i] : 2u;
+}
+__device__ __forceinline__ void wl_batch(const WorkListArgs &a, u64 i, int (&cls)[CK_WL_BATCH], u32 (&b)[CK_WL_BATCH])
+{
+    u32 n[CK_WL_BATCH], bits[CK_WL_BATCH];
+#pragma unroll
+    for (u32 j = 0; j < CK_WL_BATCH; j++) wl_load(a, i + j * CK_WL_THREADS, n[j], bits[j]);
+#pragma unroll
+    for (u32 j = 0; j < CK_WL_BATCH; j++) {
+        cls[j] = bits[j] ? record_class(n[j], bits[j]) : -1;
+        b[j] = bits[j] ? wl_bucket(cls[j], n[j]) : 0xffffffffu;
+    }
+}
+
+__global__ void __launch_bounds__(CK_WL_THREADS, 6) k_wl_count(WorkListArgs a)
+{
+    __shared__ u32 hist[CK_WL_BUCKETS];
+    __shared__ u32 cnt[16];
+    for (u32 b = threadIdx.x; b < CK_WL_BUCKETS; b += CK_WL_THREADS) hist[b] = 0;
+    if (threadIdx.x < 16) cnt[threadIdx.x] = 0;
+    __syncthreads();
+    const u32 lane = lane_id();
+    const u64 i0 = (u64)blockIdx.x << CK_WL_TILE_SHIFT;
+    u32 cc[3] = {0, 0, 0};
+    static_assert(CK_WL_TILE / CK_WL_THREADS < 256 && CLS_COUNT <= 12, "class counters fit 3 x 4 bytes");
+    for (u32 k0 = threadIdx.x; k0 < CK_WL_TILE; k0 += CK_WL_BATCH * CK_WL_THREADS) {
+        int cls[CK_WL_BATCH];
+        u32 b[CK_WL_BATCH];
+        wl_batch(a, i0 + k0, cls, b);
+#pragma unroll
+        for (u32 j = 0; j < CK_WL_BATCH; j++) {
+            const u32 pb = __match_any_sync(CK_FULL, b[j]);
+            if (cls[j] >= 0 && lane == (u32)(__ffs(pb) - 1)) atomicAdd(hist + b[j], __popc(pb));
+            if (cls[j] >= 0) a.bucket[i0 + k0 + j * CK_WL_THREADS] = (u16)b[j];
+            const u32 inc = cls[j] >= 0 ? 1u << (8 * (cls[j] & 3)) : 0u, w = (u32)cls[j] >> 2;
+            cc[0] += w == 0 ? inc : 0u; cc[1] += w == 1 ? inc : 0u; cc[2] += w == 2 ? inc : 0u;
+        }
+    }
+#pragma unroll
+    for (int c = 0; c < CLS_COUNT; c++) {
+        const u32 v = __reduce_add_sync(CK_FULL, (cc[c >> 2] >> (8 * (c & 3))) & 255u);
+        if (lane == 0 && v) atomicAdd(cnt + c, v);
+    }
+    __syncthreads();
+    for (u32 b = threadIdx.x; b < CK_WL_BUCKETS; b += CK_WL_THREADS) a.tile_counts[wl_slot(a, blockIdx.x, b)] = hist[b];
+    if (threadIdx.x < 16 && cnt[threadIdx.x]) atomicAdd(a.counts + threadIdx.x, cnt[threadIdx.x]);
+}
+
+__global__ void __launch_bounds__(CK_WL_THREADS, 6) k_wl_scatter(WorkListArgs a)
+{
+    __shared__ u32 cur[CK_WL_BUCKETS];
+    __shared__ __align__(16) u8 wc[2][CK_WL_BUCKETS][CK_WL_WARPS];
+    static_assert(CK_WL_WARPS % 4 == 0, "a row of wc is whole words");
+    const u32 lane = lane_id(), warp = threadIdx.x >> 5;
+    for (u32 b = threadIdx.x; b < CK_WL_BUCKETS; b += CK_WL_THREADS) cur[b] = a.tile_base[wl_slot(a, blockIdx.x, b)];
+    u32 *wcw = reinterpret_cast<u32 *>(&wc[0][0][0]);
+    for (u32 k = threadIdx.x; k < sizeof(wc) / 4; k += CK_WL_THREADS) wcw[k] = 0;
+    if (blockIdx.x == 0 && threadIdx.x == 0) write_list_starts(a.counts);
+    __syncthreads();
+    const u64 i0 = (u64)blockIdx.x << CK_WL_TILE_SHIFT;
+    if (i0 >= a.n_records) return;
+    for (u32 k0 = threadIdx.x; k0 < CK_WL_TILE; k0 += CK_WL_BATCH * CK_WL_THREADS) {
+        u32 bk[CK_WL_BATCH];
+#pragma unroll
+        for (u32 j = 0; j < CK_WL_BATCH; j++) {
+            const u64 i = i0 + k0 + j * CK_WL_THREADS;
+            bk[j] = i < a.n_records ? a.bucket[i] : 0xffffffffu;
+        }
+#pragma unroll
+        for (u32 j = 0; j < CK_WL_BATCH; j++) {
+            const u32 p = j & 1u, b = bk[j];
+            const u64 i = i0 + k0 + j * CK_WL_THREADS;
+            const bool valid = i < a.n_records;
+            const u32 peers = __match_any_sync(CK_FULL, b);
+            const u32 leader = (u32)__ffs(peers) - 1u, mine = __popc(peers);
+            const bool lead = valid && lane == leader;
+            if (lead) wc[p][b][warp] = (u8)mine;
+            __syncthreads();
+            u32 base = 0;
+            if (lead) {
+                const u32 *row = reinterpret_cast<const u32 *>(wc[p][b]);
+                base = cur[b];
+#pragma unroll
+                for (u32 q = 0; q < CK_WL_WARPS / 4; q++) {
+                    const u32 keep = warp >= 4 * q + 4 ? 0xffffffffu : warp <= 4 * q ? 0u : (1u << (8 * (warp - 4 * q))) - 1u;
+                    base = __dp4a(row[q] & keep, 0x01010101u, base);
+                }
+            }
+            base = __shfl_sync(CK_FULL, base, leader) + __popc(peers & ((1u << lane) - 1u));
+            if (valid) a.list[base] = (u32)i;
+            __syncthreads();
+            if (lead) { wc[p][b][warp] = 0; atomicAdd(cur + b, mine); }
+        }
+    }
+}
+
+}
diff --git a/circkit_b200/device.py b/circkit_b200/device.py
--- a/circkit_b200/device.py
+++ b/circkit_b200/device.py
@@ -9,7 +9,7 @@
 
 CLASS_NAMES = ["2bit_le_512", "2bit_le_2048", "2bit_le_65536", "2bit_le_425984", "4bit_le_2048", "4bit_le_212992",
                "byte_le_1024", "byte_le_106496", "huge", "empty", "2bit_le_4096", "2bit_le_8192", "2bit_lane_128_8192",
-               "table_insert", "table_first", "2bit_seg_8193_425984", "4bit_lane_129_2048", "pack4", "prepare"]
+               "table_insert", "table_first", "2bit_seg_8193_425984", "4bit_lane_129_2048", "pack4", "prepare", "worklist"]
 BYTE_CLASSES = ("4bit_le_2048", "4bit_le_212992", "byte_le_1024", "byte_le_106496")
 CLASS_RANGE = {"2bit_le_512": (1, 512), "2bit_le_2048": (513, 2048), "2bit_le_4096": (2049, 4096), "2bit_le_8192": (4097, 8192),
                "2bit_le_65536": (8193, 65536), "2bit_le_425984": (65537, 425984), "2bit_lane_128_8192": (1, 8192), "2bit_seg_8193_425984": (8193, 425984)}
@@ -101,6 +101,14 @@
     ctx._check(ctx._lib.ck_dev_canon_bytes(ctx.handle, _stream(), _p(raw), _p(offsets), n, total, flags, class_mask,
                                            _p(outs.out), _p(lens_out), _p(outs.start), _p(outs.strand), _p(outs.hash),
                                            _p(ws.buf), ws.bytes))
+
+
+def work_list(ctx: Context, offsets: torch.Tensor, n: int, ws: Workspace, lens: torch.Tensor = None,
+              lane_bits: torch.Tensor = None):
+    out = torch.empty(n, dtype=torch.int32, device=offsets.device)
+    ctx._check(ctx._lib.ck_dev_work_list(ctx.handle, _stream(), _p(offsets), _p(lens), _p(lane_bits), n,
+                                         _p(ws.buf), ws.bytes, _p(out)))
+    return out, ws.buf[:256].view(torch.int32).clone()
 
 
 def check(ctx: Context, ws: Workspace):
diff --git a/include/circkit_b200.h b/include/circkit_b200.h
--- a/include/circkit_b200.h
+++ b/include/circkit_b200.h
@@ -99,6 +99,8 @@
                        uint8_t *out_bytes, uint32_t *out_len, uint32_t *out_start, uint8_t *out_strand,
                        uint64_t *out_hash64, void *workspace, uint64_t workspace_bytes);
 int ck_dev_check(ck_ctx *ctx, void *stream, const void *workspace);
+int ck_dev_work_list(ck_ctx *ctx, void *stream, const uint64_t *offsets, const uint32_t *lens, const uint8_t *lane_bits,
+                     uint32_t n_records, void *workspace, uint64_t workspace_bytes, uint32_t *out_list);
 uint64_t ck_dev_table_bytes(uint64_t capacity_keys);
 int ck_dev_table_clear(ck_ctx *ctx, void *stream, void *table, uint64_t table_bytes);
 int ck_dev_table_insert(ck_ctx *ctx, void *stream, void *table, uint64_t table_bytes, const uint64_t *hash64,
```

Measured after the change: 1.500 billion, median of 6. +3.0%, better.
